# osqp/osqp-python

Measured on AMD Instinct MI355X. Metric: ADMM iterations/sec, n=100000 m=200000 nnz(A)=1000000 sparse QP (indirect PCG), higher is better.
Workload: dtype f64

## Files before the change

### osqp-python_amd/csrc/backend.h

```cpp
#pragma once
#include <cstddef>
#include <cstdint>
#include <stdexcept>

namespace osqp_hip {

struct DeviceError : std::runtime_error { using std::runtime_error::runtime_error; };

#ifndef OSQP_HIP_KBLOCK
#define OSQP_HIP_KBLOCK 256
#define OSQP_HIP_KGRID 1024
#endif
constexpr int kBlock = OSQP_HIP_KBLOCK;
constexpr int kGrid = OSQP_HIP_KGRID;
constexpr int kChunk = 8 * kBlock;
constexpr int kLongRow = 128;
constexpr int kMaxRowsPerBlock = 1024;
constexpr int kPartSlots = 40;
constexpr int kMaxCg = 1024;
constexpr int kWinCap = 1472;
constexpr int kF1Win = 512;
constexpr int kF1MaxD = 4;
constexpr int kF1PChunk = 256;
constexpr int kF1MaxOwn = 512;
constexpr int kF1MaxRows = 512;
constexpr int kF1Chunk = 1024;
constexpr int kF1StreamBytes = kF1Chunk * 12;

struct DevCsr {
  int nrows = 0, ncols = 0, nnz = 0, nblk = 0;
  int *rowptr = nullptr, *col = nullptr;
  int *blkdesc = nullptr;
  int *runinfo = nullptr;
  double *val = nullptr;
  int *blkwin = nullptr;
  unsigned short *lcol = nullptr;
  int split = 0;
  int nwin = 0;
  int single = 0;
};

struct DevF1 {
  int on = 0;
  int D = 0;
  int *blk = nullptr;
  unsigned char *stream = nullptr;
  unsigned short *cptr = nullptr;
  int *prp = nullptr, *pcol = nullptr, *psrc = nullptr;
  double *pval = nullptr;
  int pnnz = 0;
  double *va = nullptr; size_t ns = 0;
  unsigned vbytes = 0, o_rho = 0, o_pval = 0, o_pcol = 0, o_prp = 0, o_rowptr = 0, o_cptr = 0, nsb = 0;
  int mix = 0;
  int wt = 0;
  int *fcol = nullptr, *fq = nullptr;
  int *sp_ptr = nullptr;
  int *spk = nullptr;
  double *spill = nullptr; size_t nsp = 0;
};
constexpr int kF1MaxFar = 128;

constexpr int kKfMaxFill = 8;
struct DevKf {
  int on = 0;
  DevCsr K;
  int *tptr = nullptr;
  int *trow = nullptr, *ta = nullptr, *tb = nullptr;
  int nterm = 0;
  double *rec = nullptr;
};

constexpr int kWbMaxRows = 128;
constexpr int kWbLargeMax = 16384;
inline size_t wb_inverse_work(int n) { return (size_t)n * 64 * 3 + 2 * 64 * 64 + 8; }
constexpr int kWbxCols = 64;
constexpr int kWbxMaxN = 16384;
struct DevWbx {
  int on = 0, G = 0, nsc = 0;
  int slots = 0;
  double *tile2 = nullptr;
  double *tile = nullptr;
  double *partG = nullptr, *partZ = nullptr;
  double *ls0 = nullptr, *ls1 = nullptr;
  int one = 0;
  double *sinvp = nullptr;
  double *lz0 = nullptr, *lz1 = nullptr;
  int *sc_ptr = nullptr, *sc_row = nullptr, *sc_src = nullptr;
  double *sc_val = nullptr;
  double *bjj = nullptr;
};
struct DevWb {
  int on = 0, r = 0;
  int large = 0;
  int ct = 0;
  int probe = 0;
  double exact_tol = 1e-6;
  int log = 0;
  int *colmap = nullptr;
  double *W = nullptr;
  double *pv = nullptr;
  int *info = nullptr;
  int *dbg = nullptr;
  int exact = 0;
  DevWbx x;
  DevCsr AL, ALT;
  int *al_src = nullptr, *alt_src = nullptr;
  unsigned char *islong = nullptr;
  int *rows = nullptr;
  double *WT = nullptr;
  double *S = nullptr, *Sinv = nullptr;
  static constexpr int kCache = 4;
  double rho_key = 0.0;
  double *cache_buf[kCache] = {nullptr, nullptr, nullptr, nullptr}; double cache_rho[kCache] = {0, 0, 0, 0}; int cache_used = 0, cache_next = 0;
  int cache_hits = 0, cache_on = 1;
  double *g = nullptr, *h = nullptr;
  double *Dinv0 = nullptr;
  int vendor = 0;
  double *gjwork = nullptr;
  int dual = 0, cd = 0;
  int *kind = nullptr;
  int *dcol = nullptr;
  int *srow = nullptr, *ssrc = nullptr; double *sval = nullptr;
  int *sg_ptr = nullptr, *sg_col = nullptr;
  double *wv = nullptr, *den = nullptr, *beta = nullptr, *wbeta = nullptr, *rt = nullptr;
  double *uz = nullptr;
  int fused = 0;
  DevCsr Bd, Bn, As;
  double *cc = nullptr;
  int *lidx = nullptr;
  double *sig = nullptr;
  int dense = 0, grb = 0;
  int thin = 0;
  double *Ad = nullptr, *ud = nullptr, *ccd = nullptr, *gp = nullptr;
  int *bq_ptr = nullptr, *bq_idx = nullptr, *bq_col = nullptr;
};

enum ResId {
  R_PRI_U = 0, R_AX_U, R_Z_U, R_PRI_S, R_AX_S, R_Z_S, R_DY_U, R_DY_S, R_PINF_LHS, R_SUPP,
  R_DUA_U, R_PX_U, R_ATY_U, R_DUA_S, R_PX_S, R_ATY_S, R_DX_U, R_DX_S, R_XPX, R_QX, R_QDX,
  R_QN_S, R_QN_U,
  R_ATDY_U, R_ATDY_S, R_PDX_U, R_PDX_S, R_ADX_VIOL,
  R_COUNT
};
enum FlagId { F_DONE = 0, F_ITERS, F_STAT_SUM, F_STAT_MAX, F_STAT_UNCONV, F_STAT_SUMSQ, F_STAT_N, F_STAT_STAG, F_COUNT };
enum ScalId { S_TOL_REL = 0, S_TOL_ABS, S_TOL_NOW, S_RN0 , S_RN0H , S_HIST = 8  };

struct Ctl;
struct Dev {
  int n = 0, m = 0, device = 0;
  Ctl *ctl = nullptr;
  double sigma = 0, alpha = 0;
  double rho_eq_factor = 1e3;
  DevCsr A, B;
  int *Bdiag = nullptr;
  double *Praw = nullptr, *Araw = nullptr;
  int nzP = 0, nzA = 0;
  int *Pi = nullptr, *Pj = nullptr, *Pm1 = nullptr, *Pm2 = nullptr;
  int *Ai = nullptr, *Aj = nullptr, *AmA = nullptr, *AmB = nullptr;
  double *cs = nullptr;
  double *q = nullptr, *l = nullptr, *u = nullptr, *D = nullptr, *Dinv = nullptr, *E = nullptr, *Einv = nullptr;
  double *rho = nullptr, *rho_inv = nullptr;
  int *ctype = nullptr;
  double *qraw = nullptr, *lraw = nullptr, *uraw = nullptr;
  int *cnt = nullptr;
  int eq_from_cnt = 0;
  double rho_eq_mixed = 10.0;
  double *x = nullptr, *z = nullptr, *y = nullptr, *dx = nullptr, *dy = nullptr;
  double *xs = nullptr;
  double *xg = nullptr, *xsp = nullptr, *ztg = nullptr;
  int wt = 0;
  double theta = 0.9;
  double *zt = nullptr;
  double *t0 = nullptr;
  double *v = nullptr;
  double *r = nullptr, *uu = nullptr, *p = nullptr, *s = nullptr, *w = nullptr, *t = nullptr, *Minv = nullptr;
  double *uu2 = nullptr, *ms = nullptr;
  int fused = 0;
  int batch_wave_ran = -1;
  DevF1 f1;
  DevKf kf;
  DevWb wb;
  double *part = nullptr;
  double *res = nullptr;
  double *scal = nullptr;
  int *flags = nullptr;
  int *slot = nullptr;
  void *stream = nullptr;
  void *bside = nullptr, *bev0 = nullptr, *bev1 = nullptr;
  void *impl = nullptr;
};

constexpr int kBatchNB = 8;
constexpr int kBatchDirectMaxBw = 64 - kBatchNB;

constexpr int kBatchRec = 12;
struct BatchParams {
  int n, m, nbatch;
  DevCsr A, B;
  const double *D, *Dinv, *E, *Einv;
  double c, cinv, sigma, alpha, rho0, eq_factor, eps_abs, eps_rel, eps_pinf, eps_dinf, cg_frac, rho_tol;
  int max_iter, check, rho_interval, cg_max, unscaled, scaling, precond, rho_is_vec, warm;
  const double *q, *l, *u;
  const double *q0, *l0, *u0;
  double *x, *y;
  double *rec;
  int *iters_out = nullptr;
  const int *order = nullptr;
  double *zs = nullptr;
  int variant = 0;
  int polish = 0, refine = 0;
  double delta = 1e-6;
  int bw = -1;
// ... 152 lines not shown
```

### osqp-python_amd/csrc/engine.cpp

```cpp


#include "engine_internal.hpp"

#include <atomic>
#include <cstdarg>

namespace osqp_hip {

const BatchEnv &batch_env() {
  static const BatchEnv e = [] {
    auto num = [](const char *name, int dflt) { const char *v = std::getenv(name); return v ? std::atoi(v) : dflt; };
    return BatchEnv{num("OSQP_HIP_WAVE_SPLIT", -1), num("OSQP_HIP_WAVE_CUS", -1), num("OSQP_HIP_BATCH_WIDE_ROUNDS", 1 << 20)};
  }();
  return e;
}
namespace {
thread_local OSQPHipPolicy g_default_policy;
thread_local bool g_default_policy_set = false;

void policy_from_env(OSQPHipPolicy &p, bool runtime_only) {
  if (!runtime_only) { if (g_default_policy_set) p = g_default_policy; else Engine::default_policy(&p); }
  auto on = [](const char *name, OSQPInt &v) { if (const char *e = std::getenv(name)) v = e[0] != '0'; };
  auto num = [](const char *name, OSQPInt &v) { if (const char *e = std::getenv(name)) v = std::atoi(e); };
  auto real = [](const char *name, OSQPFloat &v) { if (const char *e = std::getenv(name)) v = std::atof(e); };
  on("OSQP_HIP_SMALL_DIRECT", p.small_direct); num("OSQP_HIP_DEVICE_DRIVEN", p.device_driven); on("OSQP_HIP_BATCH_REORDER", p.batch_reorder);
  num("OSQP_HIP_BATCH_WAVE", p.batch_wave);
  num("OSQP_HIP_RHO_WINDOW", p.rho_window); real("OSQP_HIP_RHO_WINDOW_TOL", p.rho_window_tol); on("OSQP_HIP_RHO_PERSIST", p.rho_persist);
  if (const char *e = std::getenv("OSQP_HIP_RHO_TOL_EXP")) { const double v = std::atof(e); p.rho_tol_exp = v > 0 && v <= 1 ? v : 0.5; }
  real("OSQP_HIP_BUDGET_TOLERATE", p.budget_tolerate); real("OSQP_HIP_BUDGET_SIGMA", p.budget_sigma); num("OSQP_HIP_BUDGET_SLACK", p.budget_slack);
  if (std::getenv("OSQP_HIP_BUDGET_FULL")) p.budget_full = 1;
  on("OSQP_HIP_CG_ESCALATE", p.cg_escalate); on("OSQP_HIP_STALL", p.stall);
  real("OSQP_HIP_POLISH_DELTA_FLOOR", p.polish_delta_floor); real("OSQP_HIP_POLISH_PCG_TOL", p.polish_pcg_tol);
  on("OSQP_HIP_SLOT_POLL", p.slot_poll); num("OSQP_HIP_POLL_LOW", p.poll_low); real("OSQP_HIP_POLL_FIRST", p.poll_first);
  real("OSQP_HIP_POLL_FRAC", p.poll_frac); real("OSQP_HIP_POLL_WAIT", p.poll_wait);
  num("OSQP_HIP_FINISH_PAIRS", p.finish_pairs); num("OSQP_HIP_POLL_SLEEP_US", p.poll_sleep_us);
  if (std::getenv("OSQP_HIP_SLOT_LOG")) p.slot_log = 1;
  if (std::getenv("OSQP_HIP_BATCH_TIMING")) p.batch_timing = 1;
  if (std::getenv("OSQP_HIP_WB_LOG")) p.woodbury_log = 1;
  if (const char *e = std::getenv("OSQP_HIP_BATCH_VARIANT")) {
    static const char *names[] = {"", "direct", "direct256", "w64", "w256", "generic"};
    p.batch_variant = 0;
    for (int k = 1; k <= 5; k++) if (!std::strcmp(e, names[k])) p.batch_variant = k;
  }
  if (runtime_only) return;
  num("OSQP_HIP_WOODBURY_FUSED", p.woodbury_fused); real("OSQP_HIP_WOODBURY_DIRECT_TOL", p.woodbury_direct_tol);
  on("OSQP_HIP_WOODBURY", p.woodbury); on("OSQP_HIP_WOODBURY_DIRECT", p.woodbury_direct); on("OSQP_HIP_WOODBURY_LARGE", p.woodbury_large);
  num("OSQP_HIP_REORDER", p.reorder); on("OSQP_HIP_WOODBURY_CACHE", p.woodbury_cache); on("OSQP_HIP_KFORM", p.kform); on("OSQP_HIP_WOODBURY_DUAL", p.woodbury_dual); on("OSQP_HIP_WOODBURY_VENDOR", p.woodbury_vendor);
  on("OSQP_HIP_GRAPH", p.graph); on("OSQP_HIP_SLOTS", p.slots); on("OSQP_HIP_PCG_FUSED", p.pcg_fused); num("OSQP_HIP_F1", p.f1); on("OSQP_HIP_WINDOW", p.window);
  real("OSQP_HIP_EXTRAP", p.extrap);
  if (const char *e = std::getenv("OSQP_HIP_RHO_EQ_FACTOR")) { const double v = std::atof(e); if (v >= 1.0) p.rho_eq_factor = v; }
  if (std::getenv("OSQP_HIP_SETUP_TIMING")) p.setup_timing = 1;
}
}

void Engine::default_policy(OSQPHipPolicy *p) {
  if (!p) return;
  *p = OSQPHipPolicy();
  p->graph = p->slots = p->pcg_fused = p->f1 = p->window = p->device_driven = p->small_direct = p->batch_reorder = 1; p->batch_variant = 0;
  p->extrap = 0.9; p->rho_eq_factor = 0.0;
  p->rho_window = 10; p->rho_window_tol = 0.1; p->rho_persist = 1; p->rho_tol_exp = 0.5;
  p->budget_tolerate = 0.0; p->budget_sigma = 3.0; p->budget_slack = 0; p->budget_full = 0; p->cg_escalate = 1; p->stall = 1;
  p->polish_delta_floor = 1e-3; p->polish_pcg_tol = 1e-15; p->woodbury = 1; p->woodbury_direct = 1; p->woodbury_large = 1; p->woodbury_cache = 1;
  p->slot_poll = 1; p->poll_low = 6; p->poll_first = 0.8; p->poll_frac = 0.75; p->poll_wait = 0.7;
  p->finish_pairs = 12; p->poll_sleep_us = 30;
  p->reorder = 1; p->kform = 0; p->woodbury_dual = 1; p->woodbury_vendor = 0; p->woodbury_fused = 1; p->woodbury_direct_tol = 1e-6; p->debug_fail_refactor = 0; p->batch_wave = 0;
}
void Engine::set_default_policy(const OSQPHipPolicy *p) {
  g_default_policy_set = p != nullptr;
  if (p) g_default_policy = *p;
}
int Engine::get_policy(OSQPHipPolicy *p) const { if (!p) return OSQP_DATA_VALIDATION_ERROR; *p = pol_; return OSQP_NO_ERROR; }
int Engine::set_policy(const OSQPHipPolicy *p) {
  if (!p) return OSQP_DATA_VALIDATION_ERROR;
  if (!(p->extrap >= 0 && p->extrap <= 2) || p->rho_window < 0 || !(p->rho_window_tol > 0) || !(p->rho_tol_exp > 0 && p->rho_tol_exp <= 1) ||
      !(p->budget_sigma >= 0) || p->finish_pairs < 1 || p->batch_variant < 0 || p->batch_variant > 5 || p->batch_wave < -1 || p->batch_wave > 1 ||
      !(p->rho_eq_factor == 0 || p->rho_eq_factor >= 1) || p->reorder < 0 || p->reorder > 2 || !(p->woodbury_direct_tol > 0 && p->woodbury_direct_tol < 1) || !(p->polish_delta_floor > 0) || !(p->polish_pcg_tol > 0 && p->polish_pcg_tol < 1))
    return OSQP_SETTINGS_VALIDATION_ERROR;
  const OSQPHipPolicy old = pol_;
  pol_ = *p; pol_explicit_ = true;
  pol_.slots = old.slots; pol_.pcg_fused = old.pcg_fused; pol_.f1 = old.f1; pol_.window = old.window; pol_.woodbury = old.woodbury; pol_.woodbury_direct = old.woodbury_direct; pol_.woodbury_large = old.woodbury_large; pol_.reorder = old.reorder; pol_.woodbury_cache = old.woodbury_cache; pol_.woodbury_fused = old.woodbury_fused; pol_.woodbury_direct_tol = old.woodbury_direct_tol; pol_.kform = old.kform; pol_.woodbury_dual = old.woodbury_dual; pol_.woodbury_vendor = old.woodbury_vendor;
  if (pol_.graph != old.graph) { use_graph_ = pol_.graph != 0; if (dev_ready_) { be::activate(d_); be::sync(d_); drop_graphs(); } }
  if (dev_ready_) d_.theta = pol_.extrap;
  if (dev_ready_ && d_.wb.dbg && pol_.debug_fail_refactor != old.debug_fail_refactor) { be::activate(d_); const int v = pol_.debug_fail_refactor; be::h2d(d_, d_.wb.dbg, &v, sizeof(int)); }
  if (dev_ready_ && pol_.rho_eq_factor >= 1.0 && pol_.rho_eq_factor != old.rho_eq_factor) return set_rho_eq_factor(pol_.rho_eq_factor);
  return OSQP_NO_ERROR;
}

namespace {
std::atomic<osqp_hip_print_fn> g_print_fn{nullptr};
std::atomic<void *> g_print_user{nullptr};
}
void Engine::set_default_print(osqp_hip_print_fn fn, void *user) { g_print_user.store(user); g_print_fn.store(fn); }
void Engine::say(const char *fmt, ...) const {
  char buf[1024];
  va_list ap;
  va_start(ap, fmt);
  std::vsnprintf(buf, sizeof(buf), fmt, ap);
  va_end(ap);
  if (print_fn_) print_fn_(buf, print_user_);
  else { std::fputs(buf, stdout); std::fflush(stdout); }
}
void Engine::print_summary_line(int iter, double obj, double pri, double dua, double rho, double t0) const {
  say("%4d  %11.4e   %8.2e   %8.2e   %8.2e  %8.2es\n", iter, obj, pri, dua, rho, (first_run_ ? info.setup_time : info.update_time) + (now_s() - t0));
}
void Engine::print_log(const Ctl &c, double t0) {
  if (!settings.verbose) return;
  if (c.nlog - log_printed_ > kCtlLog) log_printed_ = c.nlog - kCtlLog;
  for (; log_printed_ < c.nlog; log_printed_++) {
    const double *e = c.log[log_printed_ % kCtlLog];
    print_summary_line((int)e[0], e[1], e[2], e[3], e[4], t0);
  }
}

Engine::Engine() {
  print_fn_ = g_print_fn.load(); print_user_ = g_print_user.load();
  pub.settings = &settings; pub.solution = &solution; pub.info = &info; pub.work = reinterpret_cast<OSQPWorkspace *>(this);
  policy_from_env(pol_, false);
  use_graph_ = pol_.graph != 0; use_slots_ = pol_.slots != 0;
  if (pol_.rho_eq_factor >= 1.0) { eq_factor_mixed_ = pol_.rho_eq_factor; eq_factor_env_ = true; }
}
Engine::~Engine() { free_all(); }

void Engine::drop_graphs() {
  for (auto &kv : graphs_) be::graph_free(d_, kv.second);
  graphs_.clear();
  for (auto &kv : sgraphs_) be::graph_free(d_, kv.second);
  sgraphs_.clear();
}

void Engine::sync_graph_scalars() {
  const double sig[7] = {d_.theta, d_.alpha, d_.sigma, d_.rho_eq_factor, d_.rho_eq_mixed, (double)d_.eq_from_cnt, (double)reinterpret_cast<uintptr_t>(d_.wb.Sinv)};
  if (std::memcmp(sig, graph_sig_, sizeof(sig)) == 0) return;
  if (!graphs_.empty() || !sgraphs_.empty()) { be::sync(d_); drop_graphs(); }
  std::memcpy(graph_sig_, sig, sizeof(sig));
}

void Engine::free_all() {
  if (!dev_ready_) return;
  try { be::activate(d_); be::ext_wait(d_); be::sync(d_); } catch (const DeviceError &) {}
  drop_graphs();
  if (bbuf_) { be::dfree(d_, bbuf_); bbuf_ = nullptr; bbuf_cap_ = 0; }
  if (bmat_) { be::dfree(d_, bmat_); bmat_ = nullptr; bmat_cap_ = 0; }
  if (d_batch_order_) { be::dfree(d_, d_batch_order_); d_batch_order_ = nullptr; batch_order_cap_ = 0; }
  if (d_batch_iters_) { be::dfree(d_, d_batch_iters_); d_batch_iters_ = nullptr; d_batch_iters_n_ = 0; }
  batch_order_.clear();
  if (ckpt_) { be::dfree(d_, ckpt_); ckpt_ = nullptr; }
  free_batch_direct(); free_batch_spectral(); free_batch_wave();
  if (d_.f1.va) {
    d_.Minv = d_.xs = d_.p = d_.r = d_.s = d_.rho = d_.f1.pval = nullptr; d_.f1.pcol = d_.f1.prp = nullptr; d_.f1.cptr = nullptr;
  }
  if (d_.wb.cache_buf[0]) d_.wb.Sinv = d_.wb.cache_buf[0];
  void *ptrs[] = {d_.A.rowptr, d_.A.col, d_.A.blkdesc, d_.A.val, d_.B.rowptr, d_.B.col, d_.B.blkdesc, d_.B.val, d_.Bdiag, d_.A.runinfo, d_.B.runinfo, d_.A.blkwin, d_.B.blkwin, d_.A.lcol, d_.B.lcol, d_.qraw, d_.lraw, d_.uraw, d_.cnt,
                  d_.q, d_.l, d_.u, d_.D, d_.Dinv, d_.E, d_.Einv, d_.rho, d_.rho_inv, d_.ctype, d_.x, d_.z, d_.y, d_.dx,
                  d_.dy, d_.xs, d_.xg, d_.xsp, d_.ztg, d_.zt, d_.t0, d_.v, d_.r, d_.uu, d_.p, d_.s, d_.w, d_.t, d_.Minv, d_.uu2, d_.ms, d_.part, d_.res,
                  d_.scal, d_.flags, d_.slot, d_.Praw, d_.Araw, d_.cs, d_.Pi, d_.Pj, d_.Pm1, d_.Pm2, d_.Ai, d_.Aj, d_.AmA, d_.AmB,
                  d_.wb.AL.rowptr, d_.wb.AL.col, d_.wb.AL.blkdesc, d_.wb.AL.runinfo, d_.wb.AL.val, d_.wb.ALT.rowptr, d_.wb.ALT.col, d_.wb.ALT.blkdesc, d_.wb.ALT.runinfo, d_.wb.ALT.val,
                  d_.wb.al_src, d_.wb.alt_src, d_.wb.islong, d_.wb.rows, d_.wb.WT, d_.wb.S, d_.wb.Sinv, d_.wb.g, d_.wb.h, d_.wb.Dinv0, d_.wb.colmap, d_.wb.W, d_.wb.pv, d_.wb.info, d_.wb.dbg, d_.wb.x.tile, d_.wb.x.tile2, d_.wb.x.partG, d_.wb.x.partZ, d_.wb.x.ls0, d_.wb.x.ls1, d_.wb.x.lz0, d_.wb.x.lz1, d_.wb.x.sinvp, d_.wb.x.sc_ptr, d_.wb.x.sc_row, d_.wb.x.sc_src, d_.wb.x.sc_val, d_.wb.x.bjj,
                  d_.ctl, d_.f1.blk, d_.f1.stream, d_.f1.cptr, d_.f1.prp, d_.f1.pcol, d_.f1.psrc, d_.f1.pval, d_.f1.va, d_.f1.fcol, d_.f1.fq, d_.f1.sp_ptr, d_.f1.spk, d_.f1.spill, d_pc_, d_pr_,
                  d_.wb.gjwork, d_.wb.cc, d_.wb.sig, d_.wb.lidx, d_.wb.Ad, d_.wb.ud, d_.wb.ccd, d_.wb.gp, d_.wb.bq_ptr, d_.wb.bq_idx, d_.wb.bq_col, d_.wb.Bd.blkdesc, d_.wb.Bn.blkdesc, d_.wb.As.blkdesc, d_.wb.kind, d_.wb.dcol, d_.wb.srow, d_.wb.ssrc, d_.wb.sval, d_.wb.sg_ptr, d_.wb.sg_col, d_.wb.wv, d_.wb.den, d_.wb.beta, d_.wb.wbeta, d_.wb.rt, d_.wb.uz,
                  d_.kf.K.rowptr, d_.kf.K.col, d_.kf.K.blkdesc, d_.kf.K.runinfo, d_.kf.K.val, d_.kf.tptr, d_.kf.trow, d_.kf.ta, d_.kf.tb, d_.kf.rec};
  for (void *p : ptrs) if (p) be::dfree(d_, p);
  be::destroy(d_);
  d_ = Dev(); d_pc_ = d_pr_ = nullptr;
  dev_ready_ = false;
}

int Engine::validate_settings(const OSQPSettings *s, bool at_setup) {
  if (!s) return OSQP_SETTINGS_VALIDATION_ERROR;
  bool ok = s->device >= 0 && s->scaling >= 0 && s->rho > 0 && s->sigma > 0 && s->alpha > 0 && s->alpha < 2 &&
            s->cg_max_iter > 0 && s->cg_tol_reduction > 0 && s->cg_tol_fraction > 0 && s->cg_tol_fraction < 1 &&
            s->adaptive_rho_interval >= 0 && s->adaptive_rho_fraction > 0 && s->adaptive_rho_tolerance >= 1 &&
            s->max_iter > 0 && s->eps_abs >= 0 && s->eps_rel >= 0 && (s->eps_abs > 0 || s->eps_rel > 0) &&
            s->eps_prim_inf > 0 && s->eps_dual_inf > 0 && s->check_termination >= 0 && s->time_limit > 0 &&
            s->delta > 0 && s->polish_refine_iter >= 0 &&
            (s->cg_precond == OSQP_NO_PRECONDITIONER || s->cg_precond == OSQP_DIAGONAL_PRECONDITIONER);
  for (int flag : {s->verbose, s->warm_starting, s->polishing, s->rho_is_vec, s->adaptive_rho, s->scaled_termination, s->check_dualgap})
    ok = ok && (flag == 0 || flag == 1);
  if (!ok) return OSQP_SETTINGS_VALIDATION_ERROR;
  if (at_setup && s->linsys_solver != OSQP_INDIRECT_SOLVER) return OSQP_LINSYS_SOLVER_INIT_ERROR;
  return OSQP_NO_ERROR;
}

int Engine::auto_rho_interval() const {
  if (settings.adaptive_rho_interval > 0) return settings.adaptive_rho_interval;
  return settings.check_termination > 0 ? 2 * settings.check_termination : 50;
}

void Engine::compute_scaling(std::vector<double> &Px, std::vector<double> &Ax, std::vector<double> &qs) {
  D_.assign(n, 1.0); E_.assign(m, 1.0); c_ = 1.0;
  std::vector<double> dt(n), et(m), nP(n);
  auto p_col_norms = [&](std::vector<double> &out) {
    std::fill(out.begin(), out.end(), 0.0);
    for (int j = 0; j < n; j++)
      for (int k = P_.p[j]; k < P_.p[j + 1]; k++) {
        double a = std::fabs(Px[k]); int i = P_.i[k];
        out[j] = std::max(out[j], a); out[i] = std::max(out[i], a);
      }
  };
  for (int it = 0; it < settings.scaling; it++) {
    p_col_norms(dt);
    std::fill(et.begin(), et.end(), 0.0);
    for (int j = 0; j < n; j++)
      for (int k = A_.p[j]; k < A_.p[j + 1]; k++) {
        double a = std::fabs(Ax[k]);
        dt[j] = std::max(dt[j], a); et[A_.i[k]] = std::max(et[A_.i[k]], a);
      }
    for (int j = 0; j < n; j++) dt[j] = 1.0 / std::sqrt(limit_scaling(dt[j]));
    for (int i = 0; i < m; i++) et[i] = 1.0 / std::sqrt(limit_scaling(et[i]));
    for (int j = 0; j < n; j++) {
      for (int k = P_.p[j]; k < P_.p[j + 1]; k++) Px[k] *= dt[P_.i[k]] * dt[j];
      for (int k = A_.p[j]; k < A_.p[j + 1]; k++) Ax[k] *= et[A_.i[k]] * dt[j];
      qs[j] *= dt[j]; D_[j] *= dt[j];
    }
    for (int i = 0; i < m; i++) E_[i] *= et[i];
    p_col_norms(nP);
    double mean = 0; for (int j = 0; j < n; j++) mean += nP[j];
    mean /= std::max(n, 1);
    double nq = 0; for (int j = 0; j < n; j++) nq = std::max(nq, std::fabs(qs[j]));
    double ct = 1.0 / limit_scaling(std::max(limit_scaling(nq), mean));
    for (auto &v : Px) v *= ct;
    for (auto &v : qs) v *= ct;
    c_ *= ct;
  }
  Dinv_.resize(n); Einv_.resize(m);
  for (int j = 0; j < n; j++) Dinv_[j] = 1.0 / D_[j];
  for (int i = 0; i < m; i++) Einv_[i] = 1.0 / E_[i];
  cinv_ = 1.0 / c_;
}

void Engine::scale_matrix_values(std::vector<double> &Px, std::vector<double> &Ax) const {
  Px.resize(P_.nnz()); Ax.resize(A_.nnz());
  for (int j = 0; j < n; j++) {
    for (int k = P_.p[j]; k < P_.p[j + 1]; k++) Px[k] = c_ * D_[P_.i[k]] * D_[j] * P_.x[k];
    for (int k = A_.p[j]; k < A_.p[j + 1]; k++) Ax[k] = E_[A_.i[k]] * D_[j] * A_.x[k];
  }
}

void Engine::classify_constraints(const std::vector<double> &ls, const std::vector<double> &us) {
  const std::vector<int> before = ctype_;
  ctype_.resize(m);
  int n_ineq = 0;
  for (int i = 0; i < m; i++) {
    int t;
    if (ls[i] < -OSQP_INFTY * kMinScaling && us[i] > OSQP_INFTY * kMinScaling) t = -1;
    else if (us[i] - ls[i] < kRhoTol) t = 1;
    else t = 0;
    if (!settings.rho_is_vec) t = 0;
    ctype_[i] = t;
    n_ineq += (t == 0);
  }
  d_.rho_eq_factor = (n_ineq == 0) ? 1e3 : mixed_eq_factor();
  d_.eq_from_cnt = 0;
  if (before != ctype_) for (int k = 0; k < DevWb::kCache; k++) d_.wb.cache_rho[k] = -1.0;
}

void Engine::device_scale_vectors(bool q, bool bounds) {
  if (q) be::scale_q(d_, c_);
  if (bounds) {
    d_.rho_eq_mixed = mixed_eq_factor(); d_.eq_from_cnt = 1;
    be::scale_bounds(d_, settings.rho_is_vec);
    scaled_stale_ = true;
  }
}

void Engine::ensure_host_vectors() {
  if (raw_stale_) {
    be::d2h(d_, q0_.data(), d_.qraw, sizeof(double) * n);
    if (m > 0) { be::d2h(d_, l0_.data(), d_.lraw, sizeof(double) * m); be::d2h(d_, u0_.data(), d_.uraw, sizeof(double) * m); }
    raw_stale_ = false;
  }
  if (scaled_stale_) {
    ls_.resize(m); us_.resize(m);
    for (int i = 0; i < m; i++) { ls_[i] = E_[i] * l0_[i]; us_[i] = E_[i] * u0_[i]; }
    const int keep = d_.eq_from_cnt; const double keepf = d_.rho_eq_factor;
    classify_constraints(ls_, us_);
    d_.eq_from_cnt = keep; if (keep) d_.rho_eq_factor = keepf;
    scaled_stale_ = false;
  }
}

double Engine::mixed_eq_factor() const {
  constexpr int kSmallEqN = 256;
  return (!eq_factor_set_ && !eq_factor_env_ && n <= kSmallEqN) ? 1e3 : eq_factor_mixed_;
}

int Engine::set_rho_eq_factor(double f) {
  if (!dev_ready_) return OSQP_WORKSPACE_NOT_INIT_ERROR;
  if (!(f >= 1.0)) return OSQP_SETTINGS_VALIDATION_ERROR;
  be::activate(d_);
  eq_factor_mixed_ = f; eq_factor_set_ = true;
  ensure_host_vectors();
  upload_bounds_and_types();
  be::set_rho(d_, rho_bar_);
  be::precond(d_, settings.cg_precond == OSQP_DIAGONAL_PRECONDITIONER);
  return OSQP_NO_ERROR;
}

void Engine::upload_bounds_and_types() {
  std::vector<double> ls(m), us(m);
  for (int i = 0; i < m; i++) { ls[i] = E_[i] * l0_[i]; us[i] = E_[i] * u0_[i]; }
  apply_scaled_bounds(ls, us);
}
// ... 674 lines not shown
```

### osqp-python_amd/csrc/engine_setup.cpp

```cpp
#include "engine_internal.hpp"

namespace osqp_hip {

bool Engine::compute_reorder(const std::vector<int> &Arp, const std::vector<int> &Arj, const std::vector<int> &Brp, const std::vector<int> &Bj) {
  std::vector<int> cstamp(n, 0), rstamp(m, 0), comp_done(n, 0), order, sweep, best;
  order.reserve(n);
  int stamp = 0;
  size_t widest = 0;
  auto bfs = [&](int start, std::vector<int> &out) {
    out.clear(); stamp++;
    out.push_back(start); cstamp[start] = stamp;
    size_t level_end = 1;
    for (size_t h = 0; h < out.size(); h++) {
      if (h == level_end) { widest = std::max(widest, out.size() - level_end); level_end = out.size(); }
      const int j = out[h];
      for (int k = A_.p[j]; k < A_.p[j + 1]; k++) {
        const int i = A_.i[k];
        if (rstamp[i] == stamp) continue;
        rstamp[i] = stamp;
        for (int e = Arp[i]; e < Arp[i + 1]; e++) { const int c = Arj[e]; if (cstamp[c] != stamp) { cstamp[c] = stamp; out.push_back(c); } }
      }
      for (int k = Brp[j]; k < Brp[j + 1] && Bj[k] < n; k++) { const int c = Bj[k]; if (cstamp[c] != stamp) { cstamp[c] = stamp; out.push_back(c); } }
    }
  };
// ... 89 lines not shown
  if (!be::device_assembly() || m == 0 || nb < kGrid / 4) return fail("too few row blocks", nb);
  std::vector<int> a0(nb), wl(nb), lo0(nb), hi0(nb), nfar(nb, 0), cs(nb + 1);
  std::vector<int> sc, dcols;
  int D = 0;
  const int npass = allow_mix ? 3 : 1;
  for (int pass = 0; pass < npass; pass++) {
  bool pass_failed = false;
  const int far_cost = pass == 2 ? 1 : 4;
  pl.mix = 0; std::fill(nfar.begin(), nfar.end(), 0);
  for (int b = 0; b < nb; b++) {
    const int r0 = rb[b], r1 = rb[b + 1], k0 = Arp[r0], k1 = Arp[r1];
    if (k1 == k0 || r1 - r0 > kF1MaxRows || k1 - k0 > kF1Chunk || (r1 - r0 == 1 && k1 - k0 > kLongRow)) return fail("block shape", b);
    int lo = INT32_MAX, hi = -1;
    for (int k = k0; k < k1; k++) { lo = std::min(lo, Arj[k]); hi = std::max(hi, Arj[k]); }
    if (hi - lo + 1 > kF1Win || pass >= 1) {
      if (!allow_mix) return fail("no window (strict)", b);
      sc.assign(Arj.begin() + k0, Arj.begin() + k1);
      std::sort(sc.begin(), sc.end());
      bool found = false;
      {
        const int kFarCost = far_cost;
        std::vector<int> &dc = dcols; dc.assign(sc.begin(), sc.end());
        dc.erase(std::unique(dc.begin(), dc.end()), dc.end());
        const int U = (int)dc.size();
        int bi = 0, bj = 0, ci = 0; long cur = 0, best = 0;
        for (int t = 1; t < U; t++) {
          cur += kFarCost + 1 - (dc[t] - dc[t - 1]);
          if (cur < 0) { cur = 0; ci = t; }
          else if (cur > best) { best = cur; bi = ci; bj = t; }
        }
        const int far = U - (bj - bi + 1);
        const long inside = std::upper_bound(sc.begin(), sc.end(), dc[bj]) - std::lower_bound(sc.begin(), sc.end(), dc[bi]);
        if (far <= kF1MaxFar && 2 * inside >= (long)sc.size() && dc[bj] - dc[bi] + 1 <= (far ? kF1Win - kF1MaxFar : kF1Win)) { found = true; lo = dc[bi]; hi = dc[bj]; nfar[b] = far; }
      }
      if (!found && hi - lo + 1 <= kF1Win) found = true;
      if (!found) {
        const int width = kF1Win - kF1MaxFar;
        int best = -1, bi = 0, bj = 0;
        for (int i = 0, j = 0; i < (int)sc.size(); i++) {
          while (j < (int)sc.size() && sc[j] - sc[i] < width) j++;
          if (j - i > best) { best = j - i; bi = i; bj = j; }
        }
        int far = 0;
        for (int i = 0; i < (int)sc.size(); i++) if ((i < bi || i >= bj) && (i == 0 || sc[i] != sc[i - 1])) far++;
        if (far <= kF1MaxFar) { found = true; lo = sc[bi]; hi = sc[bj - 1]; nfar[b] = far; }
      }
      if (!found) { if (pass + 1 < npass) { pass_failed = true; break; } return fail("too many far columns", b); }
      if (nfar[b]) pl.mix = 1;
    }
    lo0[b] = lo; hi0[b] = hi;
  }
  if (pass_failed) continue;
  cs[0] = 0;
  for (int g = 1; g < nb; g++) {
    const int ideal = (int)((long)rb[g] * n / m);
    const int lo = std::max(cs[g - 1], std::min(lo0[g], n)), up = hi0[g - 1] + 1;
    cs[g] = lo <= up ? std::min(std::max(ideal, lo), up) : lo;
    cs[g] = std::min(std::max(cs[g], cs[g - 1]), n);
  }
  cs[nb] = n;
  for (int b = 0; b < nb; b++) {
    int lo = lo0[b], hi = hi0[b];
    if (cs[b + 1] > cs[b]) { lo = std::min(lo, cs[b]); hi = std::max(hi, cs[b + 1] - 1); }
    if (hi - lo + 1 > (nfar[b] ? kF1Win - kF1MaxFar : kF1Win)) { if (pass + 1 < npass) { pass_failed = true; break; } return fail("window + own columns too wide", b); }
    a0[b] = lo; wl[b] = hi - lo + 1;
  }
  if (pass_failed) continue;
  D = 0;
  for (int t = 1; t <= kF1MaxD && !D; t++) {
    bool ok = true;
    for (int g = 0; g + t < nb && ok; g++) ok = a0[g] + wl[g] <= a0[g + t];
    if (ok) D = t;
  }
  if (D) break;
  }
  if (!D) return fail("windows of blocks g and g + 4 overlap", -1);
  std::vector<int> &prp = pl.prp; prp.assign(n + 1, 0);
  for (int j = 0; j < n; j++) { int c = 0; for (int k = Brp[j]; k < Brp[j + 1] && Bj[k] < n; k++) c++; prp[j + 1] = prp[j] + c; }
  const int pnnz = prp[n];
  std::vector<int> &pcol = pl.pcol, &psrc = pl.psrc; pcol.assign(std::max(pnnz, 1), 0); psrc.assign(std::max(pnnz, 1), 0);
  for (int j = 0; j < n; j++) for (int k = Brp[j], o = prp[j]; k < Brp[j + 1] && Bj[k] < n; k++, o++) { pcol[o] = Bj[k]; psrc[o] = k; }
  std::vector<int> &blk = pl.blk; blk.assign(16 * (size_t)nb, 0);
  std::vector<unsigned int> &ent = pl.ent; ent.assign(Arj.size(), 0u);
  std::vector<unsigned short> &cptr = pl.cptr; cptr.clear();
  if (pl.mix) { pl.fcol.assign((size_t)nb * kF1MaxFar, -1); pl.fq.assign((size_t)nb * kF1MaxFar, 0); }
  size_t nsp = 0;
  std::vector<int> order, tpos, fc, slot;
  for (int b = 0; b < nb; b++) {
    if (cs[b + 1] - cs[b] > kF1MaxOwn || prp[cs[b + 1]] - prp[cs[b]] > kF1PChunk) return fail("own columns", b);
    const int r0 = rb[b], r1 = rb[b + 1], k0 = Arp[r0], k1 = Arp[r1], cnt = k1 - k0;
    int *w = &blk[16 * (size_t)b];
    w[0] = r0; w[1] = r1; w[2] = k0; w[3] = k1;
    w[4] = b < D ? 0 : a0[b]; w[5] = b + D < nb ? a0[b + D] : n; w[6] = cs[b]; w[7] = cs[b + 1];
    w[8] = (int)cptr.size(); w[9] = prp[cs[b]]; w[10] = prp[cs[b + 1]]; w[11] = 0;
    fc.clear();
    if (nfar[b]) {
      for (int k = k0; k < k1; k++) if (Arj[k] < a0[b] || Arj[k] >= a0[b] + wl[b]) fc.push_back(Arj[k]);
      std::sort(fc.begin(), fc.end()); fc.erase(std::unique(fc.begin(), fc.end()), fc.end());
    }
    const int nfc = (int)fc.size();
    w[11] = nfc;
    int g0 = a0[b], g1 = a0[b] + wl[b];
    for (int k = prp[cs[b]]; k < prp[cs[b + 1]]; k++) { g0 = std::min(g0, pcol[k]); g1 = std::max(g1, pcol[k] + 1); }
    if (g1 - g0 > (nfc ? kF1Win - kF1MaxFar : kF1Win) || 4 * (g1 - g0) > 5 * wl[b]) { g0 = a0[b]; g1 = a0[b] + wl[b]; }
    w[12] = g0; w[13] = g1 - g0; w[14] = a0[b]; w[15] = wl[b];
    slot.resize(cnt);
    for (int e = 0; e < cnt; e++) {
      const int c = Arj[k0 + e];
      if (c >= a0[b] && c < a0[b] + wl[b]) slot[e] = c - a0[b];
      else slot[e] = wl[b] + (int)(std::lower_bound(fc.begin(), fc.end(), c) - fc.begin());
    }
    order.resize(cnt);
    for (int e = 0; e < cnt; e++) order[e] = e;
    std::stable_sort(order.begin(), order.end(), [&](int x, int y) { return slot[x] < slot[y]; });
    tpos.resize(cnt);
    for (int t = 0; t < cnt; t++) tpos[order[t]] = t;
    for (int r = r0; r < r1; r++)
      for (int k = Arp[r]; k < Arp[r + 1]; k++) {
        const int sl = slot[k - k0];
        const unsigned gs = sl < wl[b] ? (unsigned)(Arj[k] - g0) : (unsigned)(kF1Win - kF1MaxFar + sl - wl[b]);
        ent[k] = gs | ((unsigned)(r - r0) << 9) | ((unsigned)tpos[k - k0] << 18);
      }
    const size_t base = cptr.size();
    cptr.resize(base + wl[b] + nfc + 1, 0);
    for (int e = 0; e < cnt; e++) cptr[base + slot[e] + 1]++;
    for (int c = 0; c < wl[b] + nfc; c++) cptr[base + c + 1] = (unsigned short)(cptr[base + c + 1] + cptr[base + c]);
    if (pl.mix) { std::copy(fc.begin(), fc.end(), pl.fcol.begin() + (size_t)b * kF1MaxFar); nsp += (size_t)nfc; }
  }
  if (pol_.f1 == 3 && !pl.mix) { pl.mix = 1; pl.fcol.assign((size_t)nb * kF1MaxFar, -1); pl.fq.assign((size_t)nb * kF1MaxFar, 0); }
  if (pl.mix && nsp >= (size_t)1 << 25) return fail("too many spill slots", -1);
  if (pl.mix) {
    pl.nsp = nsp;
    pl.sp_ptr.assign((size_t)n + 1, 0);
    for (int c : pl.fcol) if (c >= 0) pl.sp_ptr[c + 1]++;
    for (int j = 0; j < n; j++) pl.sp_ptr[j + 1] += pl.sp_ptr[j];
    std::vector<int> cur(pl.sp_ptr.begin(), pl.sp_ptr.end() - 1);
    for (size_t i = 0; i < pl.fcol.size(); i++) if (pl.fcol[i] >= 0) pl.fq[i] = cur[pl.fcol[i]]++;
    for (int j = 0; j < n; j++) if (pl.sp_ptr[j + 1] - pl.sp_ptr[j] > 63) return fail("a column is far for more than 63 row blocks", -1);
  }
  pl.D = D; pl.pnnz = pnnz; pl.ok = true;
  if (pol_.setup_timing) {
    double swl = 0, sgl = 0, sown = 0; int mwl = 0;
    for (int b = 0; b < nb; b++) { swl += wl[b]; sgl += blk[16 * (size_t)b + 13]; sown += cs[b + 1] - cs[b]; mwl = std::max(mwl, wl[b]); }
    std::fprintf(stderr, "[osqp_hip] F1 plan: %d row blocks, D = %d, scatter window %.1f columns on average (max %d), gather window %.1f, own columns %.1f, far columns %.2f per block\n",
                 nb, D, swl / nb, mwl, sgl / nb, sown / nb, (double)pl.nsp / nb);
  }
  return true;
}

void Engine::upload_f1(const F1Plan &pl, const std::vector<int> &Arp) {
  d_.f1 = DevF1();
  if (!pl.ok) return;
  const size_t ns = ((size_t)n + 31) / 32 * 32;
  size_t at = 8 * (7 + 3 * (size_t)pl.D) * ns;
  auto region = [&at](size_t bytes) { const size_t o = at; at += (std::max<size_t>(bytes, 1) + 255) / 256 * 256; return o; };
  const size_t o_rho = region(8 * (size_t)m), o_pval = region(8 * (size_t)pl.pnnz), o_pcol = region(sizeof(int) * pl.pcol.size()),
               o_prp = region(sizeof(int) * pl.prp.size()), o_rowptr = region(sizeof(int) * Arp.size()), o_cptr = region(sizeof(unsigned short) * pl.cptr.size());
  if (at >= ((size_t)1 << 31)) return;
  auto up_i = [&](const std::vector<int> &h) { int *p = dev_vec<int>(d_, h.size()); if (!h.empty()) be::h2d(d_, p, h.data(), sizeof(int) * h.size()); return p; };
  DevF1 &f = d_.f1;
  f.D = pl.D; f.pnnz = pl.pnnz;
  f.ns = ns; f.nsb = (unsigned)(8 * ns);
  f.va = dev_vec<double>(d_, at / 8); f.vbytes = (unsigned)at;
  unsigned char *ab = reinterpret_cast<unsigned char *>(f.va);
  f.o_rho = (unsigned)o_rho; f.o_pval = (unsigned)o_pval; f.o_pcol = (unsigned)o_pcol; f.o_prp = (unsigned)o_prp; f.o_rowptr = (unsigned)o_rowptr; f.o_cptr = (unsigned)o_cptr;
  f.pval = reinterpret_cast<double *>(ab + o_pval); f.pcol = reinterpret_cast<int *>(ab + o_pcol); f.prp = reinterpret_cast<int *>(ab + o_prp);
  f.cptr = reinterpret_cast<unsigned short *>(ab + o_cptr);
  auto put = [&](size_t o, const void *h, size_t bytes) { if (bytes) be::h2d(d_, ab + o, h, bytes); };
  put(o_pcol, pl.pcol.data(), sizeof(int) * pl.pcol.size()); put(o_prp, pl.prp.data(), sizeof(int) * pl.prp.size());
  put(o_rowptr, Arp.data(), sizeof(int) * Arp.size()); put(o_cptr, pl.cptr.data(), sizeof(unsigned short) * pl.cptr.size());
  f.blk = up_i(pl.blk); f.psrc = up_i(pl.psrc);
  {
    const size_t nb = pl.blk.size() / 16;
    std::vector<unsigned char> hs(nb * (size_t)kF1StreamBytes, 0);
    for (size_t b = 0; b < nb; b++) {
      const int k0 = pl.blk[16 * b + 2], cnt = pl.blk[16 * b + 3] - k0;
      std::memcpy(hs.data() + b * (size_t)kF1StreamBytes + sizeof(double) * kF1Chunk, pl.ent.data() + k0, sizeof(unsigned int) * (size_t)cnt);
    }
    f.stream = dev_vec<unsigned char>(d_, hs.size()); be::h2d(d_, f.stream, hs.data(), hs.size());
  }
  if (pl.mix) {
    std::vector<int> spk((size_t)n), fc2(2 * pl.fcol.size(), 0);
    for (int j = 0; j < n; j++) spk[j] = (pl.sp_ptr[j] << 6) | (pl.sp_ptr[j + 1] - pl.sp_ptr[j]);
    for (size_t i = 0; i < pl.fcol.size(); i++) if (pl.fcol[i] >= 0) { fc2[2 * i] = pl.fcol[i]; fc2[2 * i + 1] = spk[pl.fcol[i]]; }
    f.mix = 1; f.fcol = up_i(fc2); f.fq = up_i(pl.fq); f.sp_ptr = up_i(pl.sp_ptr); f.spk = up_i(spk);
    f.nsp = pl.nsp; f.spill = dev_vec<double>(d_, 3 * (f.nsp + 2));
  }
  {
    const double mb = ((double)(pl.blk.size() / 16) * kF1StreamBytes + 8.0 * (7 + 3 * (double)pl.D) * (double)f.ns + 8.0 * 10 * (double)m) / (1024.0 * 1024.0);
    const char *e = std::getenv("OSQP_HIP_F1_WT");
    f.wt = e ? (e[0] != '0') : (mb <= 380.0);
  }
  f.on = 1;
}

void Engine::prepare_kf(const std::vector<int> &Arp, const std::vector<int> &Arj, const std::vector<int> &Brp, const std::vector<int> &Bj) {
  d_.kf = DevKf();
  if (!pol_.kform || !be::kf_supported() || !be::device_assembly() || m == 0) return;
  const double t0 = now_s();
  const long nzA = Arp[m];
  long nprod = 0;
  for (int i = 0; i < m; i++) { const long len = Arp[i + 1] - Arp[i]; nprod += len * len; if (nprod > (long)kKfMaxFill * nzA + n) break; }
  long npt = 0;
  for (int j = 0; j < n; j++) for (int k = Brp[j]; k < Brp[j + 1] && Bj[k] < n; k++) npt++;
  if (nprod > (long)kKfMaxFill * nzA + n || nprod + npt >= (1L << 30)) {
    if (pol_.setup_timing) std::fprintf(stderr, "[osqp_hip] K form: fill too large (sum of squared row lengths > %d nnz(A))\n", kKfMaxFill);
    return;
  }
  std::vector<int> Krp(n + 1, 0), Kj, tptr, trow, ta, tb;
  Kj.reserve((size_t)(nprod + npt)); trow.reserve((size_t)(nprod + npt)); ta.reserve((size_t)(nprod + npt)); tb.reserve((size_t)(nprod + npt));
  tptr.reserve((size_t)(nprod + npt) + 1);
  std::vector<int> mark(n, -1), slot(n, 0), cols, cnt, order, newslot, start;
  struct Term { int s, row, a, b; };
  std::vector<Term> terms;
  for (int j = 0; j < n; j++) {
    cols.clear(); cnt.clear(); terms.clear();
    auto add = [&](int c, int row, int a, int b) {
      if (mark[c] != j) { mark[c] = j; slot[c] = (int)cols.size(); cols.push_back(c); cnt.push_back(0); }
      cnt[slot[c]]++; terms.push_back(Term{slot[c], row, a, b});
    };
    for (int k = Brp[j]; k < Brp[j + 1] && Bj[k] < n; k++) add(Bj[k], -1, k, 0);
    for (int k = A_.p[j]; k < A_.p[j + 1]; k++) {
      const int i = A_.i[k], pa = AmapA_[k];
      for (int e = Arp[i]; e < Arp[i + 1]; e++) add(Arj[e], i, pa, e);
    }
    const int nc = (int)cols.size();
    order.resize(nc);
    for (int q = 0; q < nc; q++) order[q] = q;
    std::sort(order.begin(), order.end(), [&](int x, int y) { return cols[x] < cols[y]; });
    newslot.resize(nc); start.resize(nc + 1);
    start[0] = 0;
    for (int q = 0; q < nc; q++) { newslot[order[q]] = q; start[q + 1] = start[q] + cnt[order[q]]; }
    const size_t tbase = trow.size();
    for (int q = 0; q < nc; q++) { Kj.push_back(cols[order[q]]); tptr.push_back((int)tbase + start[q]); }
    trow.resize(tbase + terms.size()); ta.resize(tbase + terms.size()); tb.resize(tbase + terms.size());
    for (const Term &t : terms) { const size_t o = tbase + (size_t)start[newslot[t.s]]++; trow[o] = t.row; ta[o] = t.a; tb[o] = t.b; }
    Krp[j + 1] = (int)Kj.size();
  }
  tptr.push_back((int)trow.size());
  const int nzK = (int)Kj.size();
  std::vector<int> rb = build_row_blocks(Krp, n), runs;
  auto up_i = [&](const std::vector<int> &h) { int *p = dev_vec<int>(d_, h.size()); if (!h.empty()) be::h2d(d_, p, h.data(), sizeof(int) * h.size()); return p; };
  DevKf &f = d_.kf;
  DevCsr &K = f.K;
  K.nrows = n; K.ncols = n; K.nnz = nzK; K.nblk = (int)rb.size() - 1; K.split = n; K.nwin = 0;
  K.single = (int)rb.size() - 1 <= kGrid;
  for (size_t b = 0; b + 1 < rb.size(); b++) if (rb[b + 1] - rb[b] > kBlock) K.single = 0;
  K.rowptr = up_i(Krp); K.col = up_i(Kj); K.blkdesc = up_i(block_descs(rb, Krp, Kj, runs)); K.runinfo = up_i(runs);
  K.val = dev_vec<double>(d_, nzK);
  f.tptr = up_i(tptr); f.trow = up_i(trow); f.ta = up_i(ta); f.tb = up_i(tb); f.nterm = (int)trow.size();
  f.rec = dev_vec<double>(d_, 8 * (size_t)n);
  f.on = 1;
  if (pol_.setup_timing) std::fprintf(stderr, "[osqp_hip] K form: nnz(K) = %d (%.1f per row), %d terms, %d row blocks, %.1f ms\n", nzK, (double)nzK / n, f.nterm, K.nblk, 1e3 * (now_s() - t0));
}

void Engine::prepare_wb(const std::vector<int> &Arp, const std::vector<int> &Arj) {
  d_.wb = DevWb();
  if (!pol_.woodbury || !be::wb_supported() || settings.cg_precond != OSQP_DIAGONAL_PRECONDITIONER || m == 0) return;
  std::vector<int> rows;
  for (int i = 0; i < m; i++) if (Arp[i + 1] - Arp[i] > kLongRow) rows.push_back(i);
  const int r = (int)rows.size();
  if (r < 1) return;
  bool large = false, dual = false;
  std::vector<int> colmap, cntL;
  int ct = 0, cd = 0;
  if (r > kWbMaxRows) {
    if (r > kWbLargeMax || !pol_.woodbury_large || !be::wb_large_supported()) return;
    size_t nz_long = 0;
    for (int i : rows) nz_long += (size_t)(Arp[i + 1] - Arp[i]);
    if (2 * nz_long < (size_t)Arp[m]) return;
    colmap.assign(n, -1);
    for (int i : rows) for (int k = Arp[i]; k < Arp[i + 1]; k++) colmap[Arj[k]] = 0;
    for (int j = 0; j < n; j++) if (colmap[j] == 0) colmap[j] = ct++;
    cntL.assign(n, 0);
    for (int i : rows) for (int k = Arp[i]; k < Arp[i + 1]; k++) cntL[Arj[k]]++;
    for (int j = 0; j < n; j++) cd += cntL[j] >= 2;
    dual = pol_.woodbury_dual != 0 && cd >= 1 && 4 * (long)cd <= 3 * (long)r;
    const double order = dual ? cd : r, width = dual ? cd : ct;
    if (8.0 * ((double)r * width + 2.0 * order * order) > 24.0 * 1024 * 1024 * 1024) return;
    large = true;
  }
  std::vector<unsigned char> islong(m, 0);
  std::vector<int> lrp(r + 1, 0), lcol, lsrc;
  for (int a = 0; a < r; a++) {
    const int i = rows[a]; islong[i] = 1;
    for (int k = Arp[i]; k < Arp[i + 1]; k++) { lcol.push_back(Arj[k]); lsrc.push_back(k); }
    lrp[a + 1] = (int)lcol.size();
  }
  std::vector<int> trp(n + 1, 0), tcol(lcol.size()), tsrc(lcol.size());
  for (int c : lcol) trp[c + 1]++;
  for (int j = 0; j < n; j++) trp[j + 1] += trp[j];
  { std::vector<int> cur(trp.begin(), trp.end() - 1);
    for (int a = 0; a < r; a++) for (int k = lrp[a]; k < lrp[a + 1]; k++) { const int pos = cur[lcol[k]]++; tcol[pos] = a; tsrc[pos] = lsrc[k]; } }
  auto up_i = [&](const std::vector<int> &h) { int *p = dev_vec<int>(d_, h.size()); if (!h.empty()) be::h2d(d_, p, h.data(), sizeof(int) * h.size()); return p; };
  auto up_csr = [&](DevCsr &M, int nr, int nc, const std::vector<int> &rp, const std::vector<int> &cj) {
    std::vector<int> rb;
    if (&M == &d_.wb.AL) { for (int a = 0; a <= nr; a++) rb.push_back(a); }
    else rb = build_row_blocks(rp, nr);
    std::vector<int> runs;
    M.nrows = nr; M.ncols = nc; M.nnz = (int)cj.size(); M.nblk = (int)rb.size() - 1; M.split = nc; M.single = 0; M.nwin = 0;
    M.rowptr = up_i(rp); M.col = up_i(cj); M.blkdesc = up_i(block_descs(rb, rp, cj, runs)); M.runinfo = up_i(runs);
    M.val = dev_vec<double>(d_, cj.size());
  };
  DevWb &w = d_.wb;
  w.r = r;
  up_csr(w.AL, r, n, lrp, lcol); up_csr(w.ALT, n, r, trp, tcol);
  w.al_src = up_i(lsrc); w.alt_src = up_i(tsrc); w.rows = up_i(rows);
  w.islong = dev_vec<unsigned char>(d_, m); be::h2d(d_, w.islong, islong.data(), m);
  const size_t ord = dual ? (size_t)cd : (size_t)r;
  w.S = dev_vec<double>(d_, ord * ord); w.Sinv = dev_vec<double>(d_, ord * ord);
  w.g = dev_vec<double>(d_, r); w.h = dev_vec<double>(d_, r); w.Dinv0 = dev_vec<double>(d_, n);
  if (large && dual) {
    std::vector<int> kind(n, 0), dcol, srow(n, 0), ssrc(n, 0), sg_ptr(r + 1, 0), sg_col;
    for (int j = 0; j < n; j++) { colmap[j] = -1; if (cntL[j] >= 2) { kind[j] = 1; colmap[j] = (int)dcol.size(); dcol.push_back(j); } else if (cntL[j] == 1) kind[j] = 2; }
    for (int a = 0; a < r; a++) {
      for (int k = lrp[a]; k < lrp[a + 1]; k++) if (kind[lcol[k]] == 2) { srow[lcol[k]] = a; ssrc[lcol[k]] = lsrc[k]; sg_col.push_back(lcol[k]); }
      sg_ptr[a + 1] = (int)sg_col.size();
    }
// ... 157 lines not shown
    for (int j = 0; j < n; j++) Brp[j + 1] += Brp[j];
    nzB = Brp[n];
    Bj.assign(nzB, 0); std::vector<int> &bdiag = bdiag_; bdiag.assign(n, 0);
    Pmap1_.assign(nzP, -1); Pmap2_.assign(nzP, -1); AmapB_.resize(nzA);
    {
      std::vector<int> cur(Brp.begin(), Brp.end() - 1);
      for (int j = 0; j < n; j++) {
        for (int k = P_.p[j]; k < P_.p[j + 1]; k++) {
          int i = P_.i[k];
          if (i == j) continue;
          int p1 = cur[j]++; Bj[p1] = i; Pmap1_[k] = p1;
        }
        bdiag[j] = cur[j]++; Bj[bdiag[j]] = j;
        for (int k = P_.p[j]; k < P_.p[j + 1]; k++)
          if (P_.i[k] == j) Pmap1_[k] = bdiag[j];
        for (int k = P_.p[j]; k < P_.p[j + 1]; k++) {
          int i = P_.i[k];
          if (i == j) continue;
          int p2 = cur[i]++; Bj[p2] = j; Pmap2_[k] = p2;
        }
      }
      for (int j = 0; j < n; j++)
        for (int k = A_.p[j]; k < A_.p[j + 1]; k++) { int pos = cur[j]++; Bj[pos] = n + A_.i[k]; AmapB_[k] = pos; }
    }
  };
  build_structure();
  lap("CSR(A), B structure, maps");
  std::vector<int> rbA = build_row_blocks(Arp, m), rbB = build_row_blocks(Brp, n);
  lap("row blocks");
  bool has_long = false;
  for (int i = 0; i < m && !has_long; i++) has_long = Arp[i + 1] - Arp[i] > kLongRow;
  const bool want_f1 = pol_.pcg_fused && use_slots_ && pol_.window != 0 && pol_.f1 && !has_long;
  F1Plan plan;
  auto try_plan = [&]() {
    if (!want_f1) return false;
    if (plan_f1(rbA, Arp, Arj, Brp, Bj, plan)) return true;
    if ((long)nzA > (long)kGrid * kF1Chunk) {
      std::vector<int> rbF = build_row_blocks(Arp, m, kF1Chunk);
      if (plan_f1(rbF, Arp, Arj, Brp, Bj, plan)) { rbA.swap(rbF); return true; }
    } else {
      std::vector<int> rbF = build_row_blocks_target(Arp, m, kF1Chunk - 24);
      if ((int)rbF.size() - 1 >= kGrid / 4 && plan_f1(rbF, Arp, Arj, Brp, Bj, plan)) { rbA.swap(rbF); return true; }
    }
    return false;
  };
  bool f1ok = try_plan();
  clear_reorder(); reorder_ms_ = 0;
  const int reorder = no_reorder_ ? 0 : pol_.reorder;
  if (m > 0 && (reorder == 2 || (reorder == 1 && want_f1 && !f1ok && be::device_assembly() && (int)rbA.size() - 1 >= kGrid / 4 && !be::batch_lds_bytes(n, m)))) {
    const double tr = now_s();
    if (compute_reorder(Arp, Arj, Brp, Bj) || reorder == 2) {
      if (pc_.empty()) {
        pc_.resize(n); ipc_.resize(n); pr_.resize(m); ipr_.resize(m);
        for (int j = 0; j < n; j++) pc_[j] = ipc_[j] = j;
        for (int i = 0; i < m; i++) pr_[i] = ipr_[i] = i;
      }
      HostCsc P0 = P_, A0 = A_; std::vector<double> q00 = q0_, l00 = l0_, u00 = u0_;
      apply_reorder();
      build_structure();
      rbA = build_row_blocks(Arp, m); rbB = build_row_blocks(Brp, n);
      f1ok = try_plan();
      if (!f1ok && reorder != 2) {
        P_ = std::move(P0); A_ = std::move(A0); q0_ = std::move(q00); l0_ = std::move(l00); u0_ = std::move(u00);
        clear_reorder();
        build_structure();
        rbA = build_row_blocks(Arp, m); rbB = build_row_blocks(Brp, n);
        f1ok = try_plan();
      }
    }
    reorder_ms_ = 1e3 * (now_s() - tr);
    lap("reordering");
  }
  if (!dev_asm) { Px = P_.x; Ax = A_.x; qs = q0_; compute_scaling(Px, Ax, qs); lap("Ruiz scaling (host)"); }
  Arp_ = Arp; Arj_ = Arj; Brp_ = Brp; Bj_ = Bj;
  d_.fused = pol_.pcg_fused ? 1 : 0;
  prepare_wb(Arp, Arj);
  if (d_.wb.on) d_.fused = 0;
  d_.f1 = DevF1();
  if (d_.fused && f1ok) upload_f1(plan, Arp);
  if (d_.fused && !d_.f1.on && use_slots_) prepare_kf(Arp, Arj, Brp, Bj);
  if (reordered_) {
    d_pc_ = dev_vec<int>(d_, n); d_pr_ = dev_vec<int>(d_, m);
    be::h2d(d_, d_pc_, pc_.data(), sizeof(int) * n); be::h2d(d_, d_pr_, pr_.data(), sizeof(int) * m);
  }
  lap("F1 / Woodbury plans");
  auto descs = [](const std::vector<int> &rb, const std::vector<int> &rp, const std::vector<int> &cj, std::vector<int> &runs) {
    std::vector<int> d; d.reserve(4 * rb.size());
    runs.clear();
    for (size_t b = 0; b + 1 < rb.size(); b++) {
      const int r0 = rb[b], r1 = rb[b + 1], k0 = rp[r0], k1 = rp[r1];
      int end_row = r1;
      if (r1 - r0 == 1 && k1 - k0 > kLongRow) {
        end_row = -(1 + (int)runs.size());
        for (int base = k0; base < k1; base += kChunk) {
          const int end = std::min(k1, base + kChunk);
          bool run = true;
          for (int k = base + 1; k < end && run; k++) run = cj[k] == cj[k - 1] + 1;
          runs.push_back(run ? cj[base] : -1);
        }
      }
      d.push_back(r0); d.push_back(end_row); d.push_back(k0); d.push_back(k1);
    }
    return d;
  };

  const bool win_on = pol_.window != 0;
  auto windows = [win_on](const std::vector<int> &rb, const std::vector<int> &rp, const std::vector<int> &cj, int split,
                    std::vector<int> &win, std::vector<unsigned short> &lcol) {
    const size_t nb = rb.size() - 1;
    win.assign(4 * nb, 0); lcol.assign(std::max<size_t>(cj.size(), 1), 0);
    int nwin = 0;
    for (size_t b = 0; b < nb; b++) {
      const int r0 = rb[b], r1 = rb[b + 1], k0 = rp[r0], k1 = rp[r1];
      win[4 * b + 1] = -1;
      if (!win_on || (r1 - r0 == 1 && k1 - k0 > kLongRow) || k1 == k0) continue;
      int lo0 = INT32_MAX, hi0 = -1, lo1 = INT32_MAX, hi1 = -1;
      for (int k = k0; k < k1; k++) {
        const int c = cj[k];
        if (c < split) { lo0 = std::min(lo0, c); hi0 = std::max(hi0, c); } else { lo1 = std::min(lo1, c - split); hi1 = std::max(hi1, c - split); }
      }
      const long len0 = hi0 >= 0 ? (long)hi0 - lo0 + 1 : 0, len1 = hi1 >= 0 ? (long)hi1 - lo1 + 1 : 0;
      if (len0 + len1 > kWinCap) continue;
      if (len0 == 0) lo0 = 0;
      if (len1 == 0) lo1 = 0;
      win[4 * b] = lo0; win[4 * b + 1] = (int)len0; win[4 * b + 2] = lo1; win[4 * b + 3] = (int)len1;
      for (int k = k0; k < k1; k++) {
        const int c = cj[k];
        lcol[k] = (unsigned short)(c < split ? c - lo0 : len0 + (c - split - lo1));
      }
      nwin++;
    }
    return nwin;
  };
  auto up_i = [&](const std::vector<int> &h) { int *p = dev_vec<int>(d_, h.size()); be::h2d(d_, p, h.data(), sizeof(int) * h.size()); return p; };
  auto up_win = [&](DevCsr &M, const std::vector<int> &rb, const std::vector<int> &rp, const std::vector<int> &cj, int split) {
    std::vector<int> win; std::vector<unsigned short> lcol;
    M.split = split;
    M.single = (int)rb.size() - 1 <= kGrid;
    for (size_t b = 0; b + 1 < rb.size(); b++) if (rb[b + 1] - rb[b] > kBlock) M.single = 0;
    M.nwin = windows(rb, rp, cj, split, win, lcol);
    M.blkwin = up_i(win);
    M.lcol = dev_vec<unsigned short>(d_, lcol.size());
    be::h2d(d_, M.lcol, lcol.data(), sizeof(unsigned short) * lcol.size());
  };
  d_.A.nrows = m; d_.A.ncols = n; d_.A.nnz = nzA; d_.A.nblk = (int)rbA.size() - 1;
  d_.A.rowptr = up_i(Arp); d_.A.col = up_i(Arj); { std::vector<int> runs; d_.A.blkdesc = up_i(descs(rbA, Arp, Arj, runs)); d_.A.runinfo = up_i(runs); } d_.A.val = dev_vec<double>(d_, nzA);
  d_.B.nrows = n; d_.B.ncols = n + m; d_.B.nnz = nzB; d_.B.nblk = (int)rbB.size() - 1;
  d_.B.rowptr = up_i(Brp); d_.B.col = up_i(Bj); { std::vector<int> runs; d_.B.blkdesc = up_i(descs(rbB, Brp, Bj, runs)); d_.B.runinfo = up_i(runs); } d_.B.val = dev_vec<double>(d_, nzB);
  d_.Bdiag = up_i(bdiag_);
  up_win(d_.A, rbA, Arp, Arj, n); up_win(d_.B, rbB, Brp, Bj, n);
  build_wbf_views(rbA, rbB, Arp, Arj, Brp, Bj);
  lap("upload structure");
  auto dv = [&](size_t cnt) { return dev_vec<double>(d_, cnt); };
  d_.q = dv(n); d_.l = dv(m); d_.u = dv(m); d_.D = dv(n); d_.Dinv = dv(n); d_.E = dv(m); d_.Einv = dv(m);
  d_.rho = d_.f1.on ? reinterpret_cast<double *>(reinterpret_cast<unsigned char *>(d_.f1.va) + d_.f1.o_rho) : dv(m); d_.rho_inv = dv(m); d_.ctype = dev_vec<int>(d_, m);
  d_.x = dv(n); d_.z = dv(m); d_.y = dv(m); d_.dx = dv(n); d_.dy = dv(m); d_.zt = dv(m); d_.t0 = dv(m); d_.v = dv(m);
  d_.xg = dv(n); d_.xsp = dv(n); d_.ztg = dv(m);
  d_.theta = pol_.extrap;
  {
    const double mb = (12.0 * ((double)d_.A.nnz + (double)d_.B.nnz) + 8.0 * (14.0 * n + 12.0 * m)) / (1024.0 * 1024.0);
    const char *ev = std::getenv("OSQP_HIP_WT");
    d_.wt = ev ? (ev[0] != '0') : (mb <= 160.0);
  }
  d_.uu = dv(n); d_.w = dv(n); d_.t = dv(m); d_.uu2 = dv(n); d_.ms = dv(2 * (size_t)n);
  if (d_.f1.on) { const size_t ns = d_.f1.ns; double *va = d_.f1.va; d_.Minv = va; d_.xs = va + ns; d_.p = va + 2 * ns; d_.r = va + 3 * ns; d_.s = va + 5 * ns; }
  else { d_.r = dv(n); d_.p = dv(n); d_.s = dv(n); d_.Minv = dv(n); d_.xs = dv(n); }
  d_.part = dv((size_t)kPartSlots * kGrid); d_.res = dv(R_COUNT); d_.scal = dv(S_HIST + 3 * (kMaxCg + 1)); d_.flags = dev_vec<int>(d_, F_COUNT); d_.slot = dev_vec<int>(d_, be::kSlotInts);
  d_.ctl = be::device_assembly() ? static_cast<Ctl *>(be::alloc(d_, sizeof(Ctl))) : nullptr;
  if (dev_asm) {
    std::vector<int> Pj(nzP), Aj(nzA);
    for (int j = 0; j < n; j++) { for (int k = P_.p[j]; k < P_.p[j + 1]; k++) Pj[k] = j; for (int k = A_.p[j]; k < A_.p[j + 1]; k++) Aj[k] = j; }
    d_.nzP = nzP; d_.nzA = nzA;
    d_.Praw = dv(nzP); d_.Araw = dv(nzA); d_.cs = dv(2);
    d_.Pi = up_i(P_.i); d_.Pj = up_i(Pj); d_.Pm1 = up_i(Pmap1_); d_.Pm2 = up_i(Pmap2_);
    d_.Ai = up_i(A_.i); d_.Aj = up_i(Aj); d_.AmA = up_i(AmapA_); d_.AmB = up_i(AmapB_);
    be::h2d(d_, d_.Praw, P_.x.data(), sizeof(double) * nzP); be::h2d(d_, d_.Araw, A_.x.data(), sizeof(double) * nzA);
    be::h2d(d_, d_.q, q0_.data(), sizeof(double) * n);
    be::assemble(d_, 0, 1.0, 0);
    c_ = be::ruiz(d_, settings.scaling);
    cinv_ = 1.0 / c_;
    be::f1_refresh(d_); be::wb_refresh(d_); be::wbx_refresh(d_);
    D_.resize(n); E_.resize(m); Dinv_.resize(n); Einv_.resize(m);
    be::d2h(d_, D_.data(), d_.D, sizeof(double) * n); be::d2h(d_, Dinv_.data(), d_.Dinv, sizeof(double) * n);
    if (m > 0) { be::d2h(d_, E_.data(), d_.E, sizeof(double) * m); be::d2h(d_, Einv_.data(), d_.Einv, sizeof(double) * m); }
    lap("assembly + Ruiz scaling (device)");
  } else {
    Aval_.assign(nzA, 0.0); Bval_.assign(nzB, 0.0);
    fill_matrix_values(Px, Ax);
    be::h2d(d_, d_.D, D_.data(), sizeof(double) * n); be::h2d(d_, d_.Dinv, Dinv_.data(), sizeof(double) * n);
    be::h2d(d_, d_.E, E_.data(), sizeof(double) * m); be::h2d(d_, d_.Einv, Einv_.data(), sizeof(double) * m);
    lap("matrix values (host-scaled)");
  }
  d_.qraw = dv(n); d_.lraw = dv(m); d_.uraw = dv(m); d_.cnt = dev_vec<int>(d_, 2);
  raw_stale_ = scaled_stale_ = false;
  if (be::device_vec_updates()) {
    be::copy_in(d_, d_.qraw, q0_.data(), sizeof(double) * n, 0);
    be::copy_in(d_, d_.lraw, l0_.data(), sizeof(double) * m, 0); be::copy_in(d_, d_.uraw, u0_.data(), sizeof(double) * m, 0);
    device_scale_vectors(true, true);
  } else {
    upload_q();
    upload_bounds_and_types();
  }
  be::set_rho(d_, rho_bar_);
  try { be::precond(d_, settings.cg_precond == OSQP_DIAGONAL_PRECONDITIONER); }
  catch (const DeviceError &err) {
    if (!(d_.wb.on && d_.wb.large)) throw;
    std::fprintf(stderr, "osqp_hip: large-rank Woodbury correction switched off for this handle (%s)\n", err.what());
    d_.wb.on = 0;
    be::precond(d_, settings.cg_precond == OSQP_DIAGONAL_PRECONDITIONER);
  }
  be::init_iterates(d_, 1);

  sol_x_.assign(n, kNaN); sol_y_.assign(m, kNaN); sol_pc_.assign(m, kNaN); sol_dc_.assign(n, kNaN);
  solution.x = sol_x_.data(); solution.y = sol_y_.data(); solution.prim_inf_cert = sol_pc_.data(); solution.dual_inf_cert = sol_dc_.data();
  std::memset(&info, 0, sizeof(info));
  set_status(OSQP_UNSOLVED);
  cg_budget_ = 0; have_tol_ = false; first_run_ = true; slot_pred_[0] = slot_pred_[1] = 6.0; slot_pred_[2] = 14.0;
  stats_ = OSQPHipStats(); stats_.nnzA = nzA; stats_.nnzB = nzB;
  be::sync(d_);
  lap("vectors, rho, preconditioner");
  info.setup_time = now_s() - t0;
  if (settings.verbose) print_setup_header();
  return OSQP_NO_ERROR;
}

void Engine::print_setup_header() const {
  say("-----------------------------------------------------------------\n");
  say("           OSQP v%s  -  Operator Splitting QP Solver\n", "1.0.0-hip");
  say("        ADMM engine for AMD MI355X (%s), C ABI of osqp v1\n", be::name());
  say("-----------------------------------------------------------------\n");
  say("problem:  variables n = %d, constraints m = %d\n", n, m);
  say("          nnz(P) + nnz(A) = %d\n", P_.nnz() + A_.nnz());
  say("settings: linear system solver = indirect (reduced-KKT PCG, %s),\n", settings.cg_precond == OSQP_DIAGONAL_PRECONDITIONER ? "diagonal preconditioner" : "no preconditioner");
  say("          eps_abs = %.2e, eps_rel = %.2e,\n", settings.eps_abs, settings.eps_rel);
  say("          eps_prim_inf = %.2e, eps_dual_inf = %.2e,\n", settings.eps_prim_inf, settings.eps_dual_inf);
  say("          rho = %.2e %s\n", settings.rho, settings.adaptive_rho ? "(adaptive)" : "");
  say("          sigma = %.2e, alpha = %.2f, max_iter = %d\n", settings.sigma, settings.alpha, settings.max_iter);
  say("          check_termination: %s (interval %d), cg_max_iter = %d\n", settings.check_termination ? "on" : "off", settings.check_termination, settings.cg_max_iter);
  say("          scaling: %s, scaled_termination: %s\n", settings.scaling ? "on" : "off", settings.scaled_termination ? "on" : "off");
  say("          warm_start: %s, polish: %s\n\n", settings.warm_starting ? "on" : "off", settings.polishing ? "on" : "off");
}

}
```

### osqp-python_amd/csrc/pcg_hip.hip

```cpp
#include "hip_common.h"

namespace osqp_hip {
namespace be {

namespace {

struct GKb {
  const double *xg, *v, *t0; int n;
  __device__ __forceinline__ void operator()(int c, double a, double (&pr)[2]) const {
    if (c < n) { pr[0] = 0.0; pr[1] = a * xg[c]; }
    else { pr[0] = a * v[c - n]; pr[1] = a * t0[c - n]; }
  }
};
struct EKb {
  const double *x, *q, *Minv; double *r, *uu; double sigma; const double *xg; double *xs; double g = 0, rn = 0, bn = 0; double px = 0, pq = 0, pm = 0, pg = 0; int wt = 0;
  __device__ __forceinline__ void prefetch(int j) { px = x[j]; pq = q[j]; pm = Minv[j]; pg = xg[j]; }
  __device__ __forceinline__ void operator()(int j, const double (&s)[2]) {
    const double rhs = sigma * px - pq + s[0];
    const double rr = rhs - s[1], u = pm * rr;
    stw(wt, r + j, rr); stw(wt, uu + j, u); stw(wt, xs + j, pg);
    g += rr * u; rn = nanmax(rn, fabs(rr)); bn = nanmax(bn, fabs(rhs));
  }
};
__global__ __launch_bounds__(kBlock) void k_kb(Dev d) {
// ... 384 lines not shown
    double DL = dl_first;
    if (!d.B.single) { __syncthreads(); DL += block_sum(e.dl, lds.k2f.red); }
    put_partial(d.part, SL_DELTA, DL);
    st.ph = P_K1F;
  }
  slot_write(W, st);
}

template <class L>
__device__ __forceinline__ void slot_ka(const Dev &d, L &lds, int used, int conv, const FirstDesc &fd, int admm, int target, int seq, int rn_slot = -1) {
  double theta = d.theta, rn_last = 0.0, bn_last = 0.0;
  if (!conv) { theta = cutoff_theta(d, rn_slot >= 0 ? rn_slot : (used & 1), lds.red, rn_last, bn_last, admm); __syncthreads(); }
  GVec g{d.xs};
  EKa e{d.l, d.u, d.rho, d.rho_inv, d.z, d.y, d.zt, d.t0, d.v, d.dy, d.alpha, d.ztg, theta}; e.wt = d.wt;
  process_rows_fd<1>(d.A, g, e, lds, NoPre(), fd);
  const int stride = gridDim.x * kBlock;
  for (int j = blockIdx.x * kBlock + threadIdx.x; j < d.n; j += stride) {
    const double xt = d.xs[j], xo = d.x[j], xn = d.alpha * xt + (1.0 - d.alpha) * xo;
    stw(d.wt, d.dx + j, xn - xo); stw(d.wt, d.x + j, xn);
    stw(d.wt, d.xg + j, xt + theta * (xt - d.xsp[j])); stw(d.wt, d.xsp + j, xt);
  }
  if (blockIdx.x == 0) {
    if (!conv) {
      const double rn = rn_last, bn = bn_last;
      conv = !(rn > fmax(d.scal[S_TOL_REL] * bn, d.scal[S_TOL_ABS])) ? 2 : 0;
      if (!conv && threadIdx.x == 0 && rn > 0.1 * d.scal[S_RN0]) d.flags[F_STAT_STAG] += 1;
    }
    if (threadIdx.x == 0) {
      d.flags[F_STAT_SUM] += used; d.flags[F_STAT_SUMSQ] += used * used; d.flags[F_STAT_N] += 1;
      if (used > d.flags[F_STAT_MAX]) d.flags[F_STAT_MAX] = used;
      if (!conv) d.flags[F_STAT_UNCONV] += 1;
      if (d.ctl && admm + 1 >= target) { d.ctl->seq_end = seq + 1; d.ctl->chunk_done = 1; }
    }
  }
}

__global__ __launch_bounds__(kBlock) void k_slot_a(Dev d) {
  __shared__ union { StreamLdsW<1, double> k1; StreamLdsW<1, double> k1f; } lds;
  const FirstDesc fd = first_desc<true>(d.A);
  SlotState st = slot_read(d.slot + SR_WORDS);
  int *W = d.slot;
  if (st.ph == P_K1) {
    GVec g{d.uu};
    EK1 e{d.rho, d.t};
    if (process_rows_fd<1>(d.A, g, e, lds.k1, PreK1{d, 0, 0, lds.k1.red, st.admm & 1}, fd)) { st.ph = P_K2F; st.k = 0; }
    else {
      __syncthreads();
      slot_ka(d, lds.k1, 0, 1, fd, st.admm, st.target, st.seq);
      st.ph = P_KB; st.admm += 1;
    }
  } else if (st.ph == P_K1F) {
    const int k = st.k, i = k + 1;
    const int nchunk = (d.n + kBlock - 1) / kBlock, per = (nchunk + 7) >> 3;
    const int xcd = blockIdx.x & 7, slot0 = blockIdx.x >> 3;
    const bool has_vec = slot0 < per && xcd * per + slot0 < nchunk;
    if (!wg_has_rows(d.A) && !has_vec && blockIdx.x != 0) {
      put_partial(d.part, SL_GAMMA0 + (i & 1), 0.0); put_partial(d.part, SL_RN0 + (i & 1), 0.0);
    } else {
      double g = 0, rn = 0;
      GMs gr{d.ms};
      EK1F e{d.rho, d.t}; e.wt = d.wt;
      process_rows_fd<1>(d.A, gr, e, lds.k1f, PreK1F{d, k, has_vec, &e, lds.k1f.red, &g, &rn}, fd);
      __syncthreads();
      block_sum_max(g, rn, lds.k1f.red);
      put_partial(d.part, SL_GAMMA0 + (i & 1), g); put_partial(d.part, SL_RN0 + (i & 1), rn);
    }
    if (i >= st.cap) { st.ph = P_KA; st.used = i; st.conv = 0; }
    else { st.ph = P_K2F; st.k = i; }
  } else if (st.ph == P_KA) {
    slot_ka(d, lds.k1, st.used, st.conv, fd, st.admm, st.target, st.seq);
    st.ph = P_KB; st.admm += 1;
  }
  slot_write(W, st);
}


struct F1Lds {
  double win[kF1Win];
  double prod[kF1Chunk];
  double tvec[kF1MaxRows];
  double uown[kF1MaxOwn];
  double puown[kF1MaxOwn];
  double pprod[kF1PChunk];
  double red[3 * kWaves];
};
struct F1Stream { double val[kF1Chunk]; unsigned int ent[kF1Chunk]; };
static_assert(sizeof(F1Stream) == kF1StreamBytes, "LDS image and global layout of a block's stream must agree");
static_assert(kF1StreamBytes % (kWaves * 1024) == 0, "every wave issues whole 1 KB pieces");
template <bool NT>
__device__ __forceinline__ void lds_dma16(const void *gsrc, unsigned lds_base) {
#if defined(__HIP_DEVICE_COMPILE__)
  unsigned keep;
  if constexpr (NT) asm volatile("s_mov_b32 %0, m0\n\ts_mov_b32 m0, %2\n\ts_nop 0\n\tglobal_load_lds_dwordx4 %1, off nt\n\ts_mov_b32 m0, %0" : "=&s"(keep) : "v"(gsrc), "s"(lds_base) : "memory");
  else asm volatile("s_mov_b32 %0, m0\n\ts_mov_b32 m0, %2\n\ts_nop 0\n\tglobal_load_lds_dwordx4 %1, off\n\ts_mov_b32 m0, %0" : "=&s"(keep) : "v"(gsrc), "s"(lds_base) : "memory");
#else
  (void)gsrc; (void)lds_base;
#endif
}
__device__ __forceinline__ unsigned lds_offset_of(const void *p) {
#if defined(__HIP_DEVICE_COMPILE__)
  return (unsigned)(unsigned long long)(__attribute__((address_space(3))) const void *)p;
#else
  (void)p; return 0u;
#endif
}
template <bool NT>
__device__ __forceinline__ void f1_stream_issue(const unsigned char *stream, int b, F1Stream &S) {
  constexpr int kPieces = kF1StreamBytes / (kWaves * 1024);
  const int wave = __builtin_amdgcn_readfirstlane((int)(threadIdx.x >> 6));
  const unsigned char *g = stream + (size_t)b * kF1StreamBytes + (size_t)wave * (kPieces * 1024) + (threadIdx.x & 63) * 16;
  const unsigned l0 = lds_offset_of(&S) + (unsigned)wave * (kPieces * 1024);
#pragma unroll
  for (int q = 0; q < kPieces; q++) lds_dma16<NT>(g + q * 1024, __builtin_amdgcn_readfirstlane(l0 + q * 1024));
}
__device__ __forceinline__ void f1_stream_wait() {
#if defined(__HIP_DEVICE_COMPILE__)
  asm volatile("s_waitcnt vmcnt(0)" ::: "memory");
#endif
}
struct F1Scal { double alpha, beta; int general; };
template <int D>
__device__ __forceinline__ double f1_w(const double (&rp)[D]) {
  double w = rp[0];
#pragma unroll
  for (int q = 1; q < D; q++) w += rp[q];
  return w;
}
__device__ __forceinline__ void f1_upd(const F1Scal &sc, double minv, double r, double w, double sp, double &sn, double &rn, double &un) {
  sn = fma(sc.beta, sc.general ? sp : 0.0, w);
  rn = fma(-sc.alpha, sn, r);
  un = minv * rn;
}
template <int kB>
__device__ __forceinline__ double f1_segsum(const double *seg, int a, int z) {
  double v[kB];
#pragma unroll
  for (int q = 0; q < kB; q++) v[q] = a + q < z ? seg[a + q] : 0.0;
  double acc = 0.0;
#pragma unroll
  for (int q = 0; q < kB; q++) acc += v[q];
  for (int k = a + kB; k < z; k++) acc += seg[k];
  return acc;
}
struct F1Fold { PartRegs a, b, c; };
__device__ __forceinline__ F1Fold f1_fold_issue(const double *part, const int par, const int probe) {
  F1Fold f;
#pragma unroll
  for (int q = 0; q < kPart; q++) { f.a.v[q] = 0.0; f.b.v[q] = 0.0; f.c.v[q] = 0.0; }
  if (probe == 1) return f;
  const int prev = par ^ 1;
  f.a = partial_load(part + (SL_GAMMA0 + prev) * kGrid); f.b = partial_load(part + (SL_DELTA + prev) * kGrid); f.c = partial_load(part + (SL_RN0 + prev) * kGrid);
  return f;
}
__device__ __forceinline__ bool f1_fold_finish(const Dev &d, const int k, const int admm_par, const int probe, const F1Fold &f, double *red, F1Scal &sc) {
  double *gam = gptr(d.scal) + S_HIST, *alp = gptr(d.scal) + S_HIST + kMaxCg + 1;
  const int tid = threadIdx.x;
  sc = F1Scal{0.0, 0.0, k >= 2};
  if (probe == 1) { sc.alpha = 1e-3; sc.beta = k >= 2 ? 0.5 : 0.0; return true; }
  if (k == 0) return true;
  double tol = gptr(d.scal)[S_TOL_NOW];
  const double glast = k >= 2 ? gam[k - 2] : 1.0, alast = k >= 2 ? alp[k - 2] : 1.0;
  double gamma = partial_fold_sum(f.a), rn = partial_fold_max(f.c), delta = partial_fold_sum(f.b);
  block_sum_max_sum(gamma, rn, delta, red);
  if (k == 1 && probe == 0) {
    const double bn = block_max(partial_fold_max(partial_load(gptr(d.part) + SL_BN * kGrid)), red);
    tol = fmax(gptr(d.scal)[S_TOL_REL] * bn, gptr(d.scal)[S_TOL_ABS]);
    if (blockIdx.x == 0 && tid == 0) { gptr(d.scal)[S_TOL_NOW] = tol; gptr(d.scal)[S_RN0] = rn; gptr(d.scal)[S_RN0H + admm_par] = rn; }
    if (!(rn > tol)) return false;
  }
  if (probe) {
    if (rn < -1.0) gptr(d.res)[R_COUNT - 1] = gamma + delta + tol + glast + alast;
    sc.alpha = 1e-3; sc.beta = k >= 2 ? 0.5 : 0.0;
    return true;
  }
  if (k >= 2 && !(rn > tol)) return false;
  sc.beta = k >= 2 ? gamma / glast : 0.0;
  sc.alpha = k >= 2 ? gamma / (delta - sc.beta * gamma / alast) : gamma / delta;
  if (blockIdx.x == 0 && tid == 0) { gam[k - 1] = gamma; alp[k - 1] = sc.alpha; }
  return true;
}
__device__ __forceinline__ int4 sload_int4(const int *base, size_t idx) {
#if defined(__HIP_DEVICE_COMPILE__)
  typedef int __attribute__((ext_vector_type(4))) v4i;
  typedef const v4i __attribute__((address_space(4))) *cptr;
  const v4i v = ((cptr)(unsigned long long)base)[idx];
  return make_int4(v.x, v.y, v.z, v.w);
#else
  return reinterpret_cast<const int4 *>(base)[idx];
#endif
}
struct F1Rec { int4 ds, fa, fb, fc; };
__device__ __forceinline__ F1Rec f1_record(const DevF1 &f, int b) {
  return F1Rec{sload_int4(f.blk, 4 * (size_t)b), sload_int4(f.blk, 4 * (size_t)b + 1), sload_int4(f.blk, 4 * (size_t)b + 2), sload_int4(f.blk, 4 * (size_t)b + 3)};
}
struct F1Spill { double v0, v1; };
__device__ __forceinline__ F1Spill f1_spill_take(const double *sp, int word) {
  const int q0 = word >> 6, cnt = word & 63;
  F1Spill t{0.0, 0.0};
  if (cnt > 0) t.v0 = sp[q0];
  if (cnt > 1) t.v1 = sp[q0 + 1];
  return t;
}
__device__ __forceinline__ double f1_spill_sum(const double *sp, int word, const F1Spill &t) {
  const int q0 = word >> 6, cnt = word & 63;
  double a = 0.0;
  if (cnt > 0) a += t.v0;
  if (cnt > 1) a += t.v1;
  for (int q = q0 + 2; q < q0 + cnt; q++) a += sp[q];
  return a;
}
__device__ __forceinline__ double f1_spill_sum(const double *sp, const int *spk, int c) {
  const int word = spk[c];
  return f1_spill_sum(sp, word, f1_spill_take(sp, word));
}
template <bool WT>
__device__ __forceinline__ void gst_(double *p, double v) {
  if constexpr (WT) __hip_atomic_store(p, v, __ATOMIC_RELAXED, __HIP_MEMORY_SCOPE_AGENT); else *p = v;
}
#define gst gst_<WT>
struct F1Arena {
#if defined(__HIP_DEVICE_COMPILE__)
  __amdgpu_buffer_rsrc_t r;
  __device__ __forceinline__ F1Arena(const double *va, unsigned bytes) : r(__builtin_amdgcn_make_buffer_rsrc(const_cast<double *>(va), 0, (int)bytes, 0x00020000)) {}
  __device__ __forceinline__ double d(unsigned vo, unsigned so) const { return __builtin_bit_cast(double, __builtin_amdgcn_raw_buffer_load_b64(r, vo, so, 0)); }
  __device__ __forceinline__ int i(unsigned vo, unsigned so) const { return (int)__builtin_amdgcn_raw_buffer_load_b32(r, vo, so, 0); }
  __device__ __forceinline__ int h(unsigned vo, unsigned so) const { return (int)__builtin_amdgcn_raw_buffer_load_b16(r, vo, so, 0); }
#else
  const unsigned char *b;
  __device__ F1Arena(const double *va, unsigned) : b(reinterpret_cast<const unsigned char *>(va)) {}
  __device__ double d(unsigned vo, unsigned so) const { return *reinterpret_cast<const double *>(b + vo + so); }
  __device__ int i(unsigned vo, unsigned so) const { return *reinterpret_cast<const int *>(b + vo + so); }
  __device__ int h(unsigned vo, unsigned so) const { return *reinterpret_cast<const unsigned short *>(b + vo + so); }
#endif
};
template <int D, bool FIRST, bool MIX, bool WT>
__device__ __forceinline__ void f1_body(const Dev &d, const int k, const bool vec_only, const F1Scal sc, F1Lds &L, F1Stream &S, const F1Rec &rec0, const int par) {
  const DevF1 &f = d.f1;
  const int n = d.n, tid = threadIdx.x;
  const int cur = (k + 1) & 1, nxt = k & 1;
  KT(1);
  const size_t ns = f.ns;
  const F1Arena ar(f.va, f.vbytes);
  const unsigned nsb = f.nsb;
  const unsigned oxs = nsb, op = 2 * nsb;
  const unsigned orr = (3 + cur) * nsb;
  const unsigned osp = (5 + cur) * nsb;
  const unsigned orep = (7 + cur * D) * nsb;
  [[maybe_unused]] const unsigned orepV = (7 + 2 * D) * nsb;
  double *xs_w = gptr(f.va) + ns, *p_w = gptr(f.va) + 2 * ns;
  double *rnxt = gptr(f.va) + (3 + nxt) * ns;
  double *snew = gptr(f.va) + (5 + nxt) * ns;
  double *repnxt = gptr(f.va) + (7 + (size_t)nxt * D) * ns;
  [[maybe_unused]] const double *spcur = MIX ? gptr(f.spill) + (size_t)cur * (f.nsp + 2) : nullptr, *spV = MIX ? gptr(f.spill) + 2 * (f.nsp + 2) : nullptr;
  [[maybe_unused]] double *spnxt = MIX ? gptr(f.spill) + (size_t)nxt * (f.nsp + 2) : nullptr;
  [[maybe_unused]] const int *spk = MIX ? gptr(f.spk) : nullptr;
  double g_acc = 0.0, rn_acc = 0.0, dl_acc = 0.0, bn_acc = 0.0;
  auto own_update = [&](int j, double mi, double r, double w, double sp, double pp, double x) -> double {
    double sn, rn, un;
    f1_upd(sc, mi, r, w, sp, sn, rn, un);
    const double pn = fma(sc.beta, sc.general ? pp : 0.0, mi * r);
    gst(xs_w + j, fma(sc.alpha, pn, x)); gst(p_w + j, pn); gst(snew + j, sn); gst(rnxt + j, rn);
    g_acc += rn * un; rn_acc = nanmax(rn_acc, fabs(rn));
    return un;
  };
  const int xcd = blockIdx.x & 7, slot0 = blockIdx.x >> 3, slots = gridDim.x >> 3;
  const int per = (d.A.nblk + 7) >> 3;
  constexpr int CW = kF1Win / kBlock, CE = kF1Chunk / kBlock;
  constexpr int kFB = kF1Win - kF1MaxFar;
  static_assert(kFB >= (CW - 1) * kBlock, "the far slots belong to the lanes' last window element");
  static_assert(kF1PChunk == kBlock, "one (P + sigma I) entry per lane");
  for (int sl = slot0; sl < per; sl += slots) {
    const int b = __builtin_amdgcn_readfirstlane(xcd * per + sl);
    if (b >= d.A.nblk) break;
    [[maybe_unused]] int2 fcl = make_int2(0, 0); [[maybe_unused]] int fql = 0;
    if constexpr (MIX) { if (tid >= kFB - (CW - 1) * kBlock) { const size_t i = (size_t)b * kF1MaxFar + (tid - (kFB - (CW - 1) * kBlock)); fcl = reinterpret_cast<const int2 *>(gptr(f.fcol))[i]; fql = gptr(f.fq)[i]; } }
    const F1Rec rec = sl == slot0 ? rec0 : f1_record(f, b);
    const int4 ds = rec.ds, fa = rec.fa, fb = rec.fb, fc = rec.fc;
    const int r0 = ds.x, nrows = ds.y - ds.x, k0 = ds.z, cnt = ds.w - ds.z;
    const int cov0 = fa.x, cov1 = fa.y, cs0 = fa.z, nown = fa.w - fa.z;
    const int cpo = fb.x, pk0 = fb.y, pcnt = fb.z - fb.y;
    const int g0 = fc.x, gl = vec_only ? 0 : fc.y, a0 = fc.z, wl = fc.w;
    const int nfc = MIX && !vec_only ? fb.w : 0;
    const int nw = nfc ? CW : (gl + kBlock - 1) / kBlock, nu = (cnt + kBlock - 1) / kBlock, ns2 = nfc ? CW : (wl + kBlock - 1) / kBlock;
    KT(2);
    const bool hasp = !vec_only && tid < pcnt;
    const int pe = min(pk0 + max(0, min(tid, pcnt - 1)), f.pnnz - 1);
    const double pv = ar.d(8u * pe, f.o_pval); const int pc = ar.i(4u * pe, f.o_pcol);
    double wm[CW], wr[CW], wsv[CW], wq[CW][D], wpp[CW], wx[CW];
    bool wown[CW];
    [[maybe_unused]] int wsw[CW]; [[maybe_unused]] F1Spill wst[CW];
#pragma unroll
    for (int u = 0; u < CW; u++) {
      wown[u] = false;
      if (u < nw) {
        const int e = tid + u * kBlock;
        int c = g0 + min(e, gl - 1);
        if constexpr (MIX) { const bool isfar = u == CW - 1 && e >= kFB && e - kFB < nfc; if (isfar) c = fcl.x; wsw[u] = isfar ? fcl.y : spk[c]; }
        wown[u] = e < gl && c >= cs0 && c - cs0 < nown;
        wm[u] = ar.d(8u * c, 0);
#pragma unroll
        for (int q = 0; q < D; q++) wq[u][q] = ar.d(8u * c, orep + q * nsb);
        const int co = wown[u] ? c : g0;
        if (!FIRST) {
          wr[u] = ar.d(8u * c, orr);
          wsv[u] = ar.d(8u * c, osp);
          wx[u] = ar.d(8u * co, oxs); wpp[u] = ar.d(8u * co, op);
        } else { wx[u] = ar.d(8u * co, oxs); wpp[u] = gptr(d.xg)[co]; }
      }
    }
    if constexpr (MIX) {
#pragma unroll
      for (int u = 0; u < CW; u++) { if (u < nw) wst[u] = f1_spill_take(spcur, wsw[u]); }
    }
    int cp0[CW], cp1[CW];
    const int prow = r0 + min(tid, nrows - 1);
    const int rp0 = ar.i(4u * prow, f.o_rowptr), rp1 = ar.i(4u * prow, f.o_rowptr + 4); const double rrho = ar.d(8u * prow, f.o_rho);
#pragma unroll
    for (int u = 0; u < CW; u++) {
      if (u < ns2) {
        int c = min(tid + u * kBlock, wl - 1);
        if constexpr (MIX) { const int cf = tid + u * kBlock - kFB; if (u == CW - 1 && cf >= 0 && cf < nfc) c = wl + cf; }
        cp0[u] = ar.h(2u * (cpo + c), f.o_cptr); cp1[u] = ar.h(2u * (cpo + c), f.o_cptr + 2);
      }
    }
    const int pj = min(cs0 + max(0, min(tid, nown - 1)), n - 1);
    const int pp0 = ar.i(4u * pj, f.o_prp), pp1 = ar.i(4u * pj, f.o_prp + 4);
    const int pcl = pc - g0;
    const bool esc = hasp && !(pcl >= 0 && pcl < gl);
    KT(3);
#pragma unroll
    for (int u = 0; u < CW; u++) {
      if (u < nw) {
        int e = min(tid + u * kBlock, gl - 1);
        if constexpr (MIX) { const int ef = tid + u * kBlock; if (u == CW - 1 && ef >= kFB && ef - kFB < nfc) e = ef; }
        double un;
        double w = f1_w<D>(wq[u]);
        if constexpr (MIX) w += f1_spill_sum(spcur, wsw[u], wst[u]);
        if constexpr (FIRST) {
          const double r0 = w;
          un = wm[u] * r0;
          if (wown[u]) {
            const int j = g0 + e;
            gst(rnxt + j, r0); gst(gptr(d.xsp) + j, wx[u]); gst(xs_w + j, wpp[u]);
            g_acc += r0 * un; rn_acc = nanmax(rn_acc, fabs(r0));
          }
        } else {
          if (wown[u]) un = own_update(g0 + e, wm[u], wr[u], w, wsv[u], wpp[u], wx[u]);
          else { double sn, rn; f1_upd(sc, wm[u], wr[u], w, wsv[u], sn, rn, un); }
        }
        if (wown[u]) L.uown[g0 + e - cs0] = un;
        L.win[e] = un;
      }
    }
    for (int jj = tid; jj < nown; jj += kBlock) {
      const int j = cs0 + jj;
      if (j >= g0 && j - g0 < gl) continue;
      const double mi = ar.d(8u * j, 0);
      double rp[D];
#pragma unroll
      for (int q = 0; q < D; q++) rp[q] = ar.d(8u * j, orep + q * nsb);
      double un;
      double wj = f1_w<D>(rp);
      if constexpr (MIX) wj += f1_spill_sum(spcur, spk, j);
      if constexpr (FIRST) {
        const double r0 = wj;
        un = mi * r0;
        gst(rnxt + j, r0); gst(gptr(d.xsp) + j, ar.d(8u * j, oxs)); gst(xs_w + j, gptr(d.xg)[j]);
        g_acc += r0 * un; rn_acc = nanmax(rn_acc, fabs(r0));
      } else un = own_update(j, mi, ar.d(8u * j, orr), wj, ar.d(8u * j, osp), ar.d(8u * j, op), ar.d(8u * j, oxs));
      if (!vec_only) L.uown[jj] = un;
    }
    if (vec_only) continue;
    KT(4);
    f1_stream_wait();
#if defined(__HIP_DEVICE_COMPILE__)
    asm volatile("" :: "v"(rp0), "v"(rp1), "v"(rrho), "v"(pp0), "v"(pp1), "v"(pv), "v"(pc));
#pragma unroll
    for (int u = 0; u < CW; u++) { if (u < ns2) asm volatile("" :: "v"(cp0[u]), "v"(cp1[u])); }
    if constexpr (MIX) asm volatile("" :: "v"(fql));
#endif
    __syncthreads();
    [[maybe_unused]] double bv[D];
    [[maybe_unused]] int bsw = 0; [[maybe_unused]] F1Spill bst{0.0, 0.0};
    if constexpr (FIRST) {
      const int j = cs0 + max(0, min(tid, nown - 1));
#pragma unroll
      for (int q = 0; q < D; q++) bv[q] = ar.d(8u * j, orepV + q * nsb);
      if constexpr (MIX) bsw = spk[j];
    }
    double vw[CE]; unsigned int en[CE];
#pragma unroll
    for (int u = 0; u < CE; u++) { if (u < nu) { const int e = min(tid + u * kBlock, cnt - 1); vw[u] = S.val[e]; en[u] = S.ent[e]; } }
#pragma unroll
    for (int u = 0; u < CE; u++) { if (u < nu) L.prod[tid + u * kBlock] = vw[u] * L.win[en[u] & 0x1ffu]; }
    if (hasp) {
      double uv;
      if (!esc) uv = L.win[pcl];
      else {
        double eq[D];
#pragma unroll
        for (int q = 0; q < D; q++) eq[q] = ar.d(8u * pc, orep + q * nsb);
        const double em = ar.d(8u * pc, 0);
        double ew = f1_w<D>(eq);
        if constexpr (MIX) ew += f1_spill_sum(spcur, spk, pc);
        if constexpr (FIRST) uv = em * ew;
        else { double sn, rn; f1_upd(sc, em, ar.d(8u * pc, orr), ew, ar.d(8u * pc, osp), sn, rn, uv); }
      }
      L.pprod[tid] = pv * uv;
    }
    KT(5);
    __syncthreads();
    if (sl + slots < per) {
      const int bn = __builtin_amdgcn_readfirstlane(xcd * per + sl + slots);
      if (bn < d.A.nblk) f1_stream_issue<!WT>(f.stream, bn, S);
    }
    if (tid < nrows) {
      const double au = f1_segsum<6>(L.prod, rp0 - k0, rp1 - k0), t = rrho * au;
      L.tvec[tid] = t; dl_acc += t * au;
    }
    for (int row = tid + kBlock; row < nrows; row += kBlock) {
      const int q0 = ar.i(4u * (r0 + row), f.o_rowptr), q1 = ar.i(4u * (r0 + row), f.o_rowptr + 4);
      const double au = f1_segsum<6>(L.prod, q0 - k0, q1 - k0), t = ar.d(8u * (r0 + row), f.o_rho) * au;
      L.tvec[row] = t; dl_acc += t * au;
    }
    KT(6);
    __syncthreads();
#pragma unroll
    for (int u = 0; u < CE; u++) { if (u < nu) L.prod[en[u] >> 18] = vw[u] * L.tvec[(en[u] >> 9) & 0x1ffu]; }
    if (tid < nown) {
      const double pu = f1_segsum<4>(L.pprod, pp0 - pk0, pp1 - pk0);
      L.puown[tid] = pu; dl_acc += L.uown[tid] * pu;
    }
    for (int jj = tid + kBlock; jj < nown; jj += kBlock) {
      const int q0 = ar.i(4u * (cs0 + jj), f.o_prp), q1 = ar.i(4u * (cs0 + jj), f.o_prp + 4);
      const double pu = f1_segsum<4>(L.pprod, q0 - pk0, q1 - pk0);
      L.puown[jj] = pu; dl_acc += L.uown[jj] * pu;
    }
    KT(7);
    __syncthreads();
    double *rout = repnxt + (size_t)(b % D) * ns;
#pragma unroll
    for (int u = 0; u < CW; u++) {
      if (u < ns2) {
        const int c = tid + u * kBlock;
        if (c < wl) {
          double v = f1_segsum<8>(L.prod, cp0[u], cp1[u]);
          const int jo = a0 + c - cs0;
          if (jo >= 0 && jo < nown) v += L.puown[jo];
          gst(rout + a0 + c, v);
        } else if constexpr (MIX) {
          if (u == CW - 1 && c >= kFB && c - kFB < nfc) gst(spnxt + fql, f1_segsum<8>(L.prod, cp0[u], cp1[u]));
        }
      }
    }
    for (int j = cov0 + tid; j < a0; j += kBlock) gst(rout + j, 0.0);
    for (int j = a0 + wl + tid; j < cov1; j += kBlock) gst(rout + j, 0.0);
    if constexpr (FIRST) {
      if (tid < nown) bn_acc = nanmax(bn_acc, fabs(MIX ? f1_w<D>(bv) + f1_spill_sum(spV, bsw, f1_spill_take(spV, bsw)) : f1_w<D>(bv)));
      for (int jj = tid + kBlock; jj < nown; jj += kBlock) {
        double rv[D];
#pragma unroll
        for (int q = 0; q < D; q++) rv[q] = ar.d(8u * (cs0 + jj), orepV + q * nsb);
        bn_acc = nanmax(bn_acc, fabs(MIX ? f1_w<D>(rv) + f1_spill_sum(spV, spk, cs0 + jj) : f1_w<D>(rv)));
      }
    }
    KT(8);
    if (sl + slots < per) __syncthreads();
  }
  if (vec_only) f1_stream_wait();
  __syncthreads();
  block_sum_max_sum(g_acc, rn_acc, dl_acc, L.red);
  put_partial(gptr(d.part), SL_GAMMA0 + par, g_acc); put_partial(gptr(d.part), SL_RN0 + par, rn_acc);
  if constexpr (FIRST) {
    bn_acc = block_max(bn_acc, L.red);
    put_partial(gptr(d.part), SL_BN, bn_acc);
  }
  if (!vec_only) put_partial(gptr(d.part), SL_DELTA + par, dl_acc);
  KT(9);
}
__device__ __forceinline__ F1Rec f1_first_record(const int *blk, int nblk) {
  const int b0 = __builtin_amdgcn_readfirstlane((int)(blockIdx.x & 7) * ((nblk + 7) >> 3) + (int)(blockIdx.x >> 3));
  const size_t b = (size_t)min(b0, nblk - 1);
  return F1Rec{sload_int4(blk, 4 * b), sload_int4(blk, 4 * b + 1), sload_int4(blk, 4 * b + 2), sload_int4(blk, 4 * b + 3)};
}
template <int D, bool MIX, bool WT>
__device__ __forceinline__ bool f1_iteration(const Dev &d, const int k, const int cap, const int admm_par, const int probe, F1Lds &L, F1Stream &S, const F1Rec &rec0, const F1Fold &fold, const int par) {
  KT(0);
  F1Scal sc;
  if (!f1_fold_finish(d, k, admm_par, probe, fold, L.red, sc)) return false;
  const bool vec_only = !probe && k >= cap;
  if (k == 0) f1_body<D, true, MIX, WT>(d, k, vec_only, sc, L, S, rec0, par);
  else f1_body<D, false, MIX, WT>(d, k, vec_only, sc, L, S, rec0, par);
  return true;
}
template <bool NT>
__device__ __forceinline__ void f1_stream_first(const unsigned char *stream, int nblk, F1Stream &S) {
  const int per = (nblk + 7) >> 3, slot0 = (int)(blockIdx.x >> 3);
  const int b0 = __builtin_amdgcn_readfirstlane((int)(blockIdx.x & 7) * per + slot0);
  if (slot0 < per && b0 < nblk) f1_stream_issue<NT>(stream, b0, S);
}

template <int D, bool SCATTER_ONLY, bool MIX, bool WT>
__device__ __forceinline__ void f1_ka_body(const Dev &d, F1Lds &L, F1Stream &S, const F1Rec &rec0, const double theta) {
  const DevF1 &f = d.f1;
  const int tid = threadIdx.x;
  const double *va = gptr(f.va); const size_t ns = f.ns;
  const double *xs_r = va + ns;
  double *repR = gptr(f.va) + (7 + (size_t)1 * D) * ns, *repV = gptr(f.va) + (7 + (size_t)2 * D) * ns;
  [[maybe_unused]] double *spR = MIX ? gptr(f.spill) + (f.nsp + 2) : nullptr, *spVw = MIX ? gptr(f.spill) + 2 * (f.nsp + 2) : nullptr;
  const double alpha = d.alpha, sigma = d.sigma;
  const int xcd = blockIdx.x & 7, slot0 = blockIdx.x >> 3, slots = gridDim.x >> 3;
  const int per = (d.A.nblk + 7) >> 3;
  constexpr int CW = kF1Win / kBlock, CE = kF1Chunk / kBlock;
  constexpr int kFB = kF1Win - kF1MaxFar;
  for (int sl = slot0; sl < per; sl += slots) {
    const int b = __builtin_amdgcn_readfirstlane(xcd * per + sl);
    if (b >= d.A.nblk) break;
    [[maybe_unused]] int fcl = 0, fql = 0;
    if constexpr (MIX) { if (tid >= kFB - (CW - 1) * kBlock) { const size_t i = (size_t)b * kF1MaxFar + (tid - (kFB - (CW - 1) * kBlock)); fcl = gptr(f.fcol)[2 * i]; fql = gptr(f.fq)[i]; } }
    const F1Rec rec = sl == slot0 ? rec0 : f1_record(f, b);
    const int4 ds = rec.ds, fa = rec.fa, fb = rec.fb, fc = rec.fc;
    const int r0 = ds.x, nrows = ds.y - ds.x, k0 = ds.z, cnt = ds.w - ds.z;
    const int cov0 = fa.x, cov1 = fa.y, cs0 = fa.z, nown = fa.w - fa.z;
    const int cpo = fb.x, pk0 = fb.y, pcnt = fb.z - fb.y;
    const int g0 = fc.x, gl = fc.y, a0 = fc.z, wl = fc.w;
    const int nfc = MIX ? fb.w : 0;
    const int nw = nfc ? CW : (gl + kBlock - 1) / kBlock, nu = (cnt + kBlock - 1) / kBlock, ns2 = nfc ? CW : (wl + kBlock - 1) / kBlock;
    double pv = 0.0; int pc = g0;
    const bool hasp = tid < pcnt;
    { const int e = pk0 + max(0, min(tid, pcnt - 1)); pv = gptr(f.pval)[e]; pc = gptr(f.pcol)[e]; }
    const int pcl = pc - g0;
    const bool pin = pcl >= 0 && pcl < gl;
    double pxs = 0.0, pxp = 0.0;
    if (SCATTER_ONLY) pxs = gptr(d.xg)[pc];
    else { pxp = gptr(d.xsp)[pc]; if (!pin) pxs = xs_r[pc]; }
    double wx[CW], wxo[CW], wxp[CW], wq[CW];
    bool wown[CW];
#pragma unroll
    for (int u = 0; u < CW; u++) {
      wown[u] = false;
      if (u < nw) {
        const int e = tid + u * kBlock;
        int c = g0 + min(e, gl - 1);
        if constexpr (MIX) { if (u == CW - 1 && e >= kFB && e - kFB < nfc) c = fcl; }
        wown[u] = e < gl && c >= cs0 && c - cs0 < nown;
        const int co = wown[u] ? c : g0;
        if (!SCATTER_ONLY) { wx[u] = xs_r[c]; wxp[u] = gptr(d.xsp)[co]; }
        wxo[u] = gptr(d.x)[co]; wq[u] = gptr(d.q)[co];
      }
    }
    int rp0 = 0, rp1 = 0;
    double el = 0, eu = 0, erho = 0, erinv = 0, ez = 0, ey = 0, ezt = 0;
    { const int row = r0 + min(tid, nrows - 1);
      if (SCATTER_ONLY) { ez = gptr(d.v)[row]; ey = gptr(d.t0)[row]; }
      else { rp0 = gptr(d.A.rowptr)[row]; rp1 = gptr(d.A.rowptr)[row + 1]; el = gptr(d.l)[row]; eu = gptr(d.u)[row]; erho = gptr(d.rho)[row]; erinv = gptr(d.rho_inv)[row]; ez = gptr(d.z)[row]; ey = gptr(d.y)[row]; ezt = gptr(d.zt)[row]; } }
    int cp0[CW], cp1[CW];
#pragma unroll
    for (int u = 0; u < CW; u++) {
      if (u < ns2) {
        int c = min(tid + u * kBlock, wl - 1);
        if constexpr (MIX) { const int cf = tid + u * kBlock - kFB; if (u == CW - 1 && cf >= 0 && cf < nfc) c = wl + cf; }
        cp0[u] = gptr(f.cptr)[cpo + c]; cp1[u] = gptr(f.cptr)[cpo + c + 1];
      }
    }
    int pp0 = 0, pp1 = 0;
    { const int j = min(cs0 + max(0, min(tid, nown - 1)), d.n - 1); pp0 = gptr(f.prp)[j]; pp1 = gptr(f.prp)[j + 1]; }
#pragma unroll
    for (int u = 0; u < CW; u++) {
      if (u < nw) {
        int e = min(tid + u * kBlock, gl - 1);
        if constexpr (MIX) { const int ef = tid + u * kBlock; if (u == CW - 1 && ef >= kFB && ef - kFB < nfc) e = ef; }
        if (!SCATTER_ONLY) L.win[e] = wx[u];
        if (wown[u]) {
          const int j = g0 + e;
          double xn = wxo[u];
          if (!SCATTER_ONLY) {
            const double xt = wx[u];
            xn = alpha * xt + (1.0 - alpha) * wxo[u];
            gst(gptr(d.dx) + j, xn - wxo[u]); gst(gptr(d.x) + j, xn);
            gst(gptr(d.xg) + j, xt + theta * (xt - wxp[u]));
          }
          L.uown[j - cs0] = sigma * xn - wq[u];
        }
      }
    }
    f1_stream_wait();
#if defined(__HIP_DEVICE_COMPILE__)
    asm volatile("" :: "v"(rp0), "v"(rp1), "v"(el), "v"(eu), "v"(erho), "v"(erinv), "v"(ez), "v"(ey), "v"(ezt), "v"(pp0), "v"(pp1), "v"(pv), "v"(pc), "v"(pxs), "v"(pxp));
#pragma unroll
    for (int u = 0; u < CW; u++) { if (u < ns2) asm volatile("" :: "v"(cp0[u]), "v"(cp1[u])); }
    if constexpr (MIX) asm volatile("" :: "v"(fql));
#endif
    __syncthreads();
    double vw[CE]; unsigned int en[CE];
#pragma unroll
    for (int u = 0; u < CE; u++) { if (u < nu) { const int e = min(tid + u * kBlock, cnt - 1); vw[u] = S.val[e]; en[u] = S.ent[e]; } }
    if (!SCATTER_ONLY) {
#pragma unroll
      for (int u = 0; u < CE; u++) { if (u < nu) L.prod[tid + u * kBlock] = vw[u] * L.win[en[u] & 0x1ffu]; }
    }
    if (hasp) {
      double xg;
      if (SCATTER_ONLY) xg = pxs;
      else { const double xt = pin ? L.win[pcl] : pxs; xg = xt + theta * (xt - pxp); }
      L.pprod[tid] = pv * xg;
    }
    __syncthreads();
    if (sl + slots < per) {
      const int bn = __builtin_amdgcn_readfirstlane(xcd * per + sl + slots);
      if (bn < d.A.nblk) f1_stream_issue<!WT>(f.stream, bn, S);
    }
    double t0r = 0.0;
    if (tid < nrows) {
      double vi;
      if (SCATTER_ONLY) { vi = ez; t0r = ey; }
      else {
        const int i = r0 + tid;
        const double ztil = f1_segsum<6>(L.prod, rp0 - k0, rp1 - k0);
        const double zr = alpha * ztil + (1.0 - alpha) * ez;
        const double zn = fmin(fmax(zr + erinv * ey, el), eu);
        const double dyi = erho * (zr - zn), yn = ey + dyi;
        const double zg = ztil + theta * (ztil - ezt);
        vi = erho * zn - yn; t0r = erho * zg;
        gst(gptr(d.y) + i, yn); gst(gptr(d.dy) + i, dyi); gst(gptr(d.z) + i, zn); gst(gptr(d.zt) + i, ztil); gst(gptr(d.v) + i, vi); gst(gptr(d.ztg) + i, zg); gst(gptr(d.t0) + i, t0r);
      }
      L.tvec[tid] = vi;
    }
    for (int row = tid + kBlock; row < nrows; row += kBlock) {
      const int i = r0 + row;
      double vi;
      if (SCATTER_ONLY) vi = gptr(d.v)[i];
      else {
        const int q0 = gptr(d.A.rowptr)[i], q1 = gptr(d.A.rowptr)[i + 1];
        const double rho = gptr(d.rho)[i], zo = gptr(d.z)[i], yo = gptr(d.y)[i];
        const double ztil = f1_segsum<6>(L.prod, q0 - k0, q1 - k0);
        const double zr = alpha * ztil + (1.0 - alpha) * zo;
        const double zn = fmin(fmax(zr + gptr(d.rho_inv)[i] * yo, gptr(d.l)[i]), gptr(d.u)[i]);
        const double dyi = rho * (zr - zn), yn = yo + dyi;
        const double zg = ztil + theta * (ztil - gptr(d.zt)[i]);
        vi = rho * zn - yn;
        gst(gptr(d.y) + i, yn); gst(gptr(d.dy) + i, dyi); gst(gptr(d.z) + i, zn); gst(gptr(d.zt) + i, ztil); gst(gptr(d.v) + i, vi); gst(gptr(d.ztg) + i, zg); gst(gptr(d.t0) + i, rho * zg);
      }
      L.tvec[row] = vi;
    }
    if (tid < nown) L.puown[tid] = f1_segsum<4>(L.pprod, pp0 - pk0, pp1 - pk0);
    for (int jj = tid + kBlock; jj < nown; jj += kBlock) { const int q0 = gptr(f.prp)[cs0 + jj], q1 = gptr(f.prp)[cs0 + jj + 1]; L.puown[jj] = f1_segsum<4>(L.pprod, q0 - pk0, q1 - pk0); }
    __syncthreads();
#pragma unroll
    for (int u = 0; u < CE; u++) { if (u < nu) L.prod[en[u] >> 18] = vw[u] * L.tvec[(en[u] >> 9) & 0x1ffu]; }
    __syncthreads();
    double cv[CW];
#pragma unroll
    for (int u = 0; u < CW; u++) {
      cv[u] = 0.0;
      if (u < ns2) { const int c = tid + u * kBlock; if (c < wl || (MIX && u == CW - 1 && c >= kFB && c - kFB < nfc)) cv[u] = f1_segsum<8>(L.prod, cp0[u], cp1[u]); }
    }
    __syncthreads();
    if (tid < nrows) L.tvec[tid] = t0r;
    for (int row = tid + kBlock; row < nrows; row += kBlock) L.tvec[row] = gptr(d.t0)[r0 + row];
    __syncthreads();
#pragma unroll
    for (int u = 0; u < CE; u++) { if (u < nu) L.prod[en[u] >> 18] = vw[u] * L.tvec[(en[u] >> 9) & 0x1ffu]; }
    __syncthreads();
    double *routR = repR + (size_t)(b % D) * ns, *routV = repV + (size_t)(b % D) * ns;
#pragma unroll
    for (int u = 0; u < CW; u++) {
      if (u < ns2) {
        const int c = tid + u * kBlock;
        if (c < wl) {
          double tv = cv[u], tt = f1_segsum<8>(L.prod, cp0[u], cp1[u]);
          const int jo = a0 + c - cs0;
          if (jo >= 0 && jo < nown) { tv += L.uown[jo]; tt += L.puown[jo]; }
          gst(routV + a0 + c, tv); gst(routR + a0 + c, tv - tt);
        } else if constexpr (MIX) {
          if (u == CW - 1 && c >= kFB && c - kFB < nfc) { const double tv = cv[u], tt = f1_segsum<8>(L.prod, cp0[u], cp1[u]); gst(spVw + fql, tv); gst(spR + fql, tv - tt); }
        }
      }
    }
    for (int j = cov0 + tid; j < a0; j += kBlock) { gst(routV + j, 0.0); gst(routR + j, 0.0); }
    for (int j = a0 + wl + tid; j < cov1; j += kBlock) { gst(routV + j, 0.0); gst(routR + j, 0.0); }
    if (sl + slots < per) __syncthreads();
  }
}
template <int D, bool MIX, bool WT>
__device__ __forceinline__ void f1_slot_ka(const Dev &d, F1Lds &L, F1Stream &S, const F1Rec &rec0, int used, int conv, int admm, int target, int rn_slot, int seq) {
  double theta = d.theta, rn_last = 0.0, bn_last = 0.0;
  if (!conv) { theta = cutoff_theta(d, rn_slot, L.red, rn_last, bn_last, admm); __syncthreads(); }
  f1_ka_body<D, false, MIX, WT>(d, L, S, rec0, theta);
  if (blockIdx.x == 0) {
    if (!conv) {
      const double rn = rn_last, bn = bn_last;
      conv = !(rn > fmax(gptr(d.scal)[S_TOL_REL] * bn, gptr(d.scal)[S_TOL_ABS])) ? 2 : 0;
      if (!conv && threadIdx.x == 0 && rn > 0.1 * gptr(d.scal)[S_RN0]) gptr(d.flags)[F_STAT_STAG] += 1;
    }
    if (threadIdx.x == 0) {
      gptr(d.flags)[F_STAT_SUM] += used; gptr(d.flags)[F_STAT_SUMSQ] += used * used; gptr(d.flags)[F_STAT_N] += 1;
      if (used > gptr(d.flags)[F_STAT_MAX]) gptr(d.flags)[F_STAT_MAX] = used;
      if (!conv) gptr(d.flags)[F_STAT_UNCONV] += 1;
      if (d.ctl && admm + 1 >= target) { gptr(d.ctl)->seq_end = seq + 1; gptr(d.ctl)->chunk_done = 1; }
    }
  }
}
__global__ __launch_bounds__(kBlock) void k_f1_refresh(Dev d) {
  for (int k = blockIdx.x * kBlock + threadIdx.x; k < d.f1.pnnz; k += gridDim.x * kBlock) d.f1.pval[k] = d.B.val[d.f1.psrc[k]];
  for (int b = blockIdx.x; b < d.A.nblk; b += gridDim.x) {
    const int k0 = d.f1.blk[16 * (size_t)b + 2], cnt = d.f1.blk[16 * (size_t)b + 3] - k0;
    double *dst = reinterpret_cast<double *>(d.f1.stream + (size_t)b * kF1StreamBytes);
    for (int e = threadIdx.x; e < cnt; e += kBlock) dst[e] = d.A.val[k0 + e];
  }
}
template <int D, bool MIX, bool WT>
__global__ __launch_bounds__(kBlock) __attribute__((amdgpu_waves_per_eu(4, 4))) void k_f1_probe(Dev d, int k, int mode) {
  __shared__ F1Lds lds;
  __shared__ F1Stream sbuf;
  const int par = k & 1;
  f1_stream_first<!WT>(d.f1.stream, d.A.nblk, sbuf);
  const F1Fold fold = f1_fold_issue(gptr(d.part), par, mode);
  f1_iteration<D, MIX, WT>(d, k, 1 << 30, 0, mode, lds, sbuf, f1_first_record(d.f1.blk, d.A.nblk), fold, par);
}

template <int D, bool MIX, bool WT>
__global__ __launch_bounds__(kBlock) __attribute__((amdgpu_waves_per_eu(4, 4))) void k_f1_ka_probe(Dev d, int scatter_only) {
  __shared__ F1Lds lds;
  __shared__ F1Stream sbuf;
  f1_stream_first<!WT>(d.f1.stream, d.A.nblk, sbuf);
  const F1Rec rec0 = f1_first_record(d.f1.blk, d.A.nblk);
  if (scatter_only) f1_ka_body<D, true, MIX, WT>(d, lds, sbuf, rec0, d.theta); else f1_ka_body<D, false, MIX, WT>(d, lds, sbuf, rec0, d.theta);
}

struct F1DevBlock { Dev d; };
template <int D, bool MIX, bool WT>
__global__ __launch_bounds__(kBlock) __attribute__((amdgpu_waves_per_eu(4, 4))) void k_slot1(const unsigned char *__restrict__ stream, const int *__restrict__ fblk, int nblk, int par,
                                                                                             const double *__restrict__ part, const int *__restrict__ slot, const F1DevBlock *__restrict__ blk) {
  __shared__ F1Lds lds;
  __shared__ F1Stream sbuf;
  static_assert(sizeof(F1Lds) + sizeof(F1Stream) <= 160 * 1024 / 4, "four workgroups per CU");
  const Dev &d = blk->d;
  const int *R = slot + (par ? SR_WORDS : 0);
  int *W = const_cast<int *>(R) + (par ? -SR_WORDS : SR_WORDS);
  f1_stream_first<!WT>(stream, nblk, sbuf);
  const F1Fold fold = f1_fold_issue(gptr(part), par, 0);
  const F1Rec rec0 = f1_first_record(fblk, nblk);
  SlotState st = slot_read_scalar(R);
  if (st.ph == P_KB) {
    if (st.admm >= st.target) { st.ph = P_IDLE; f1_stream_wait(); slot_write(W, st); return; }
    f1_ka_body<D, true, MIX, WT>(d, lds, sbuf, rec0, 0.0);
    if (blockIdx.x == 0 && threadIdx.x == 0) { gptr(d.flags)[F_DONE] = 0; gptr(d.flags)[F_ITERS] = 0; }
    st.ph = P_F; st.k = 0;
  } else if (st.ph == P_F) {
    if (f1_iteration<D, MIX, WT>(d, st.k, st.cap, st.admm & 1, 0, lds, sbuf, rec0, fold, par)) {
      if (st.k >= st.cap) { st.ph = P_KA; st.used = st.k; st.conv = 0; }
      else st.k += 1;
    } else {
      __syncthreads();
      f1_slot_ka<D, MIX, WT>(d, lds, sbuf, rec0, st.k - 1, 1, st.admm, st.target, 0, st.seq);
      st.admm += 1; st.k = 0; st.ph = st.admm >= st.target ? P_IDLE : P_F;
    }
  } else if (st.ph == P_KA) {
    f1_slot_ka<D, MIX, WT>(d, lds, sbuf, rec0, st.used, st.conv, st.admm, st.target, par ^ 1, st.seq);
    st.admm += 1; st.k = 0; st.ph = st.admm >= st.target ? P_IDLE : P_F;
  } else f1_stream_wait();
  slot_write(W, st);
}


#undef gst
struct KfOps { double2 a, b; };
struct GKf {
  const double *rec; const F1Scal *sc;
  using Ops = KfOps;
  __device__ __forceinline__ Ops fetch(int c) const { const double2 *p = reinterpret_cast<const double2 *>(rec + 4 * (size_t)c); Ops o; o.a = p[0]; o.b = p[1]; return o; }
  __device__ __forceinline__ void prod(const Ops &o, double a, double (&pr)[1]) const { double sn, rn, un; f1_upd(*sc, o.a.x, o.a.y, o.b.x, o.b.y, sn, rn, un); pr[0] = a * un; }
  __device__ __forceinline__ void operator()(int c, double a, double (&pr)[1]) const { prod(fetch(c), a, pr); }
};
struct EKf {
  const double *recr; double *recw, *p, *xs; const F1Scal *sc;
  double g = 0, rn = 0, dl = 0;
  double2 oa = make_double2(0, 0), ob = make_double2(0, 0); double pp = 0, px = 0;
  __device__ __forceinline__ void prefetch(int j) { const double2 *q = reinterpret_cast<const double2 *>(recr + 4 * (size_t)j); oa = q[0]; ob = q[1]; pp = p[j]; px = xs[j]; }
  __device__ __forceinline__ void update(int j, double w, bool with_w) {
    double sn, rnew, un;
    f1_upd(*sc, oa.x, oa.y, ob.x, ob.y, sn, rnew, un);
    const double pn = fma(sc->beta, sc->general ? pp : 0.0, oa.x * oa.y);
    xs[j] = fma(sc->alpha, pn, px); p[j] = pn;
    double2 *o = reinterpret_cast<double2 *>(recw + 4 * (size_t)j);
    o[0] = make_double2(oa.x, rnew); o[1] = make_double2(w, sn);
    g += rnew * un; rn = nanmax(rn, fabs(rnew)); if (with_w) dl += un * w;
  }
  __device__ __forceinline__ void operator()(int j, const double (&s)[1]) { update(j, s[0], true); }
};
struct PreKf {
  [[maybe_unused]] static constexpr int kTraceBase = 0;
  const Dev &d; int k, admm_par, probe, par; double *red; F1Scal *sc;
  using Tok = F1Fold;
  __device__ __forceinline__ Tok begin() const { return f1_fold_issue(d.part, par, probe); }
  __device__ __forceinline__ bool finish(const Tok &t) const { return f1_fold_finish(d, k, admm_par, probe, t, red, *sc); }
};
template <class L>
__device__ __forceinline__ bool kf_iteration(const Dev &d, const int k, const int cap, const int admm_par, const int probe, L &lds, const int par) {
  F1Scal sc{0.0, 0.0, 0};
  const int cur = (k + 1) & 1, nxt = k & 1;
  const double *recr = d.kf.rec + (size_t)cur * 4 * (size_t)d.n;
  double *recw = d.kf.rec + (size_t)nxt * 4 * (size_t)d.n;
  const bool vec_only = !probe && k >= cap;
  EKf e{recr, recw, d.p, d.xs, &sc};
  if (vec_only) {
    const F1Fold fold = f1_fold_issue(d.part, par, probe);
    if (!f1_fold_finish(d, k, admm_par, probe, fold, lds.red, sc)) return false;
    const DevCsr &M = d.kf.K;
    const int4 *desc = reinterpret_cast<const int4 *>(M.blkdesc);
    const int xcd = blockIdx.x & 7, slot0 = blockIdx.x >> 3, slots = gridDim.x >> 3, per = (M.nblk + 7) >> 3;
    for (int sl = slot0; sl < per; sl += slots) {
      const int b = xcd * per + sl;
      if (b >= M.nblk) break;
      const int4 ds = desc[b];
      const int r1 = ds.y < 0 ? ds.x + 1 : ds.y;
      for (int j = ds.x + (int)threadIdx.x; j < r1; j += kBlock) { e.prefetch(j); e.update(j, 0.0, false); }
    }
  } else {
    GKf g{recr, &sc};
    if (!process_rows<1>(d.kf.K, g, e, lds, PreKf{d, k, admm_par, probe, par, lds.red, &sc})) return false;
  }
  __syncthreads();
  block_sum_max_sum(e.g, e.rn, e.dl, lds.red);
  put_partial(d.part, SL_GAMMA0 + par, e.g); put_partial(d.part, SL_RN0 + par, e.rn);
  if (!vec_only) put_partial(d.part, SL_DELTA + par, e.dl);
  return true;
}
struct EKbK {
  const double *x, *q, *Minv; double *rec1; double sigma; const double *xg; double *xs; double bn = 0; double px = 0, pq = 0, pm = 0, pg = 0;
  __device__ __forceinline__ void prefetch(int j) { px = x[j]; pq = q[j]; pm = Minv[j]; pg = xg[j]; }
  __device__ __forceinline__ void operator()(int j, const double (&s)[2]) {
    const double rhs = sigma * px - pq + s[0];
    const double rr = rhs - s[1];
    double2 *o = reinterpret_cast<double2 *>(rec1 + 4 * (size_t)j);
    o[0] = make_double2(pm, rr); o[1] = make_double2(0.0, 0.0);
    xs[j] = pg;
    bn = nanmax(bn, fabs(rhs));
  }
};
__global__ __launch_bounds__(kBlock) void k_kf_values(Dev d, int cond) {
  if (cond && !d.ctl->rho_flag) return;
  const DevKf &f = d.kf;
  const int stride = gridDim.x * kBlock;
  for (int e = blockIdx.x * kBlock + threadIdx.x; e < f.K.nnz; e += stride) {
    const int t0 = f.tptr[e], t1 = f.tptr[e + 1];
    double v = 0.0;
    for (int t = t0; t < t1; t++) { const int i = f.trow[t]; v += i < 0 ? d.B.val[f.ta[t]] : d.rho[i] * (d.A.val[f.ta[t]] * d.A.val[f.tb[t]]); }
    f.K.val[e] = v;
  }
}
__global__ __launch_bounds__(kBlock) void k_slotk(Dev d, int par) {
  __shared__ union { StreamLds<2> kb; StreamLds<1> f; StreamLdsW<1, double> ka; } lds;
  const int *R = d.slot + (par ? SR_WORDS : 0);
  int *W = d.slot + (par ? 0 : SR_WORDS);
  const FirstDesc fdA = first_desc<true>(d.A);
  SlotState st = slot_read(R);
  if (st.ph == P_KB) {
    if (st.admm >= st.target) { st.ph = P_IDLE; slot_write(W, st); return; }
    GKb g{d.xg, d.v, d.t0, d.n};
    EKbK e{d.x, d.q, d.Minv, d.kf.rec + 4 * (size_t)d.n, d.sigma, d.xg, d.xs};
    process_rows<2>(d.B, g, e, lds.kb);
    __syncthreads();
    const double BN = block_max(e.bn, lds.kb.red);
    put_partial(d.part, SL_BN, BN);
    if (blockIdx.x == 0 && threadIdx.x == 0) { d.flags[F_DONE] = 0; d.flags[F_ITERS] = 0; }
    st.ph = P_F; st.k = 0;
  } else if (st.ph == P_F) {
    if (kf_iteration(d, st.k, st.cap, st.admm & 1, st.conv == 2 ? 2 : 0, lds.f, par)) {
      if (st.k >= st.cap) { st.ph = P_KA; st.used = st.k; st.conv = 0; }
      else st.k += 1;
    } else {
      __syncthreads();
      slot_ka(d, lds.ka, st.k - 1, 1, fdA, st.admm, st.target, st.seq);
      st.admm += 1; st.k = 0; st.ph = P_KB;
    }
  } else if (st.ph == P_KA) {
    slot_ka(d, lds.ka, st.used, st.conv, fdA, st.admm, st.target, st.seq, par ^ 1);
    st.admm += 1; st.k = 0; st.ph = P_KB;
  }
  slot_write(W, st);
}


}

void kb_rhs(Dev &d) { LAUNCH(k_kb, d, d); }
bool pcg_fused(const Dev &d) { return d.fused != 0; }
void k1(Dev &d, int i) { if (d.fused && i > 0) LAUNCH(k_k1f, d, d, i); else LAUNCH(k_k1, d, d, i, 0); }
void k2(Dev &d, int i) { if (d.fused) LAUNCH(k_k2f, d, d, i); else LAUNCH(k_k2, d, d, 0); }
void kv(Dev &d, int i) { if (d.n >= 2 * kGrid * kBlock) LAUNCH(k_kv<2>, d, d, i, 0); else LAUNCH(k_kv<1>, d, d, i, 0); }
void ka(Dev &d, int budget) { LAUNCH(k_ka, d, d, budget); }
bool slots_supported(const Dev &d) { return (d.fused != 0 || wbx_slots(d)) && d.slot != nullptr; }
void dev_publish(Dev &d) {
  if (!d.f1.on) return;
  Impl &p = im(d);
  if (!p.dev_block) {
    HIP_CHECK(hipMalloc(&p.dev_block, sizeof(F1DevBlock)));
    HIP_CHECK(hipHostMalloc(reinterpret_cast<void **>(&p.pin_block), sizeof(F1DevBlock), hipHostMallocDefault));
    p.shadow_block = static_cast<unsigned char *>(std::calloc(1, sizeof(F1DevBlock)));
    std::memset(p.pin_block, 0, sizeof(F1DevBlock));
    p.shadow_block[0] = 1;
  }
  F1DevBlock nb;
  std::memset(static_cast<void *>(&nb), 0, sizeof(nb));
  std::memcpy(static_cast<void *>(&nb.d), static_cast<const void *>(&d), sizeof(Dev));
  if (std::memcmp(&nb, p.shadow_block, sizeof(nb)) == 0) return;
  HIP_CHECK(hipStreamSynchronize(st(d)));
  std::memcpy(p.shadow_block, &nb, sizeof(nb));
  std::memcpy(p.pin_block, &nb, sizeof(nb));
  HIP_CHECK(hipMemcpyAsync(p.dev_block, p.pin_block, sizeof(nb), hipMemcpyHostToDevice, st(d)));
}
void dev_release(Dev &d) {
  Impl &p = im(d);
  if (p.dev_block) { (void)hipFree(p.dev_block); p.dev_block = nullptr; }
  if (p.pin_block) { (void)hipHostFree(p.pin_block); p.pin_block = nullptr; }
  if (p.shadow_block) { std::free(p.shadow_block); p.shadow_block = nullptr; }
}
template <class F>
static void f1_dispatch(const Dev &d, F &&f) {
  auto with_m = [&](auto Dc, auto Mc) { if (d.f1.wt) f(Dc, Mc, std::true_type{}); else f(Dc, Mc, std::false_type{}); };
  auto with_d = [&](auto Dc) { if (d.f1.mix) with_m(Dc, std::true_type{}); else with_m(Dc, std::false_type{}); };
  switch (d.f1.D) {
    case 1: with_d(std::integral_constant<int, 1>{}); break;
    case 2: with_d(std::integral_constant<int, 2>{}); break;
    case 3: with_d(std::integral_constant<int, 3>{}); break;
    default: with_d(std::integral_constant<int, 4>{}); break;
  }
}
void slot_begin(Dev &d, int target, int cap) { HIP_CHECK(hipSetDevice(d.device)); dev_publish(d); hipLaunchKernelGGL(k_slot_init, dim3(1), dim3(1), 0, st(d), d.slot, target, cap, ++im(d).epoch); }
void slot_pair(Dev &d) {
  if (wbx_slots(d)) { wbx_slot_pair(d); return; }
  if (d.f1.on) {
    const F1DevBlock *db = static_cast<const F1DevBlock *>(im(d).dev_block);
    f1_dispatch(d, [&](auto Dc, auto Mc, auto Wc) {
      constexpr int DD = decltype(Dc)::value; constexpr bool MM = decltype(Mc)::value, WW = decltype(Wc)::value;
      hipLaunchKernelGGL((k_slot1<DD, MM, WW>), dim3(kGrid), dim3(kBlock), 0, st(d), static_cast<const unsigned char *>(d.f1.stream), static_cast<const int *>(d.f1.blk), d.A.nblk, 0, static_cast<const double *>(d.part), static_cast<const int *>(d.slot), db);
      hipLaunchKernelGGL((k_slot1<DD, MM, WW>), dim3(kGrid), dim3(kBlock), 0, st(d), static_cast<const unsigned char *>(d.f1.stream), static_cast<const int *>(d.f1.blk), d.A.nblk, 1, static_cast<const double *>(d.part), static_cast<const int *>(d.slot), db);
    });
  }
  else if (d.kf.on) { LAUNCH(k_slotk, d, d, 0); LAUNCH(k_slotk, d, d, 1); }
  else { LAUNCH(k_slot_b, d, d); LAUNCH(k_slot_a, d, d); }
}
bool kf_supported() { return true; }
void kf_values(Dev &d, int cond) { if (d.kf.on) { HIP_CHECK(hipSetDevice(d.device)); LAUNCH(k_kf_values, d, d, cond); } }
void f1_refresh(Dev &d) { if (d.f1.on) { HIP_CHECK(hipSetDevice(d.device)); LAUNCH(k_f1_refresh, d, d); } }
int slot_seq(Dev &d) { return (im(d).pin_flags + F_COUNT)[SR_SEQ]; }
int slot_done(Dev &d) {
  const int *rec = im(d).pin_flags + F_COUNT;
  return rec[SR_ADMM];
}

void slot_poll(Dev &d, int *seq, int *done) {
  HIP_CHECK(hipSetDevice(d.device));
  Impl &p = im(d);
  HIP_CHECK(hipMemcpyAsync(p.pin_poll, d.slot, sizeof(int) * kSlotInts, hipMemcpyDeviceToHost, p.side));
  HIP_CHECK(hipStreamSynchronize(p.side));
  if (p.pin_poll[2 * SR_WORDS] != p.epoch) { *seq = 0; *done = 0; return; }
  const int *ra = p.pin_poll, *rb = p.pin_poll + SR_WORDS;
  const int *nw = ra[SR_SEQ] >= rb[SR_SEQ] ? ra : rb;
  *seq = nw[SR_SEQ]; *done = nw[SR_ADMM];
}

__global__ void k_slot_probe_f(int *slot, double *scal, int k0, int conv) {
  for (int rec = 0; rec < 2; rec++) {
    int *r = slot + rec * SR_WORDS;
    r[SR_PHASE] = P_F; r[SR_K] = k0; r[SR_ADMM] = 0; r[SR_TARGET] = 1; r[SR_USED] = 0; r[SR_CONV] = conv; r[SR_CAP] = 1 << 20; r[SR_SEQ] = rec ? -1 : 0;
  }
  scal[S_TOL_NOW] = -1.0;
}
static void f1_probe_pair(Dev &d, int mode) {
  f1_dispatch(d, [&](auto Dc, auto Mc, auto Wc) {
    constexpr int DD = decltype(Dc)::value; constexpr bool MM = decltype(Mc)::value, WW = decltype(Wc)::value;
    hipLaunchKernelGGL((k_f1_probe<DD, MM, WW>), dim3(kGrid), dim3(kBlock), 0, st(d), d, 2, mode);
    hipLaunchKernelGGL((k_f1_probe<DD, MM, WW>), dim3(kGrid), dim3(kBlock), 0, st(d), d, 3, mode);
  });
}
float time_kernel(Dev &d, int which, int reps) {
  HIP_CHECK(hipSetDevice(d.device));
  Impl &p = im(d);
  struct Save { double *ptr; size_t cnt; double *bak; };
  const size_t n = d.n, m = d.m;
  if (which >= 14 && which <= 18 && !d.f1.on && !(which == 16 && d.kf.on)) return 0.f;
  if (which == 20 && !wbx_active(d)) return 0.f;
  if (which == 21 && !(d.wb.on && d.wb.exact)) return 0.f;
  if (which == 23 && !wbf_active(d)) return 0.f;
  const bool wbx = which == 20;
  const size_t r3 = wbx ? 3 * (size_t)d.wb.r : 0, gp_ = wbx ? (size_t)d.wb.x.G * kWbMaxRows : 0;
  Save sv[] = {{d.x, n, nullptr}, {d.z, m, nullptr}, {d.y, m, nullptr}, {d.xs, n, nullptr}, {d.zt, m, nullptr}, {d.t0, m, nullptr},
               {d.v, m, nullptr}, {d.dx, n, nullptr}, {d.dy, m, nullptr}, {d.r, n, nullptr}, {d.uu, n, nullptr}, {d.p, n, nullptr},
               {d.s, n, nullptr}, {d.w, n, nullptr}, {d.t, m, nullptr}, {d.uu2, n, nullptr}, {d.ms, 2 * n, nullptr},
               {d.xg, n, nullptr}, {d.xsp, n, nullptr}, {d.ztg, m, nullptr}, {d.kf.rec, d.kf.on ? 8 * n : 0, nullptr},
               {d.wb.x.ls0, r3, nullptr}, {d.wb.x.ls1, r3, nullptr}, {d.wb.x.partG, gp_, nullptr}, {d.wb.x.partZ, gp_, nullptr}};
  int flags_bak[F_COUNT];
  HIP_CHECK(hipStreamSynchronize(st(d)));
  HIP_CHECK(hipMemcpy(flags_bak, d.flags, sizeof(flags_bak), hipMemcpyDeviceToHost));
  for (auto &s : sv) {
    if (!s.cnt) continue;
    HIP_CHECK(hipMalloc(reinterpret_cast<void **>(&s.bak), s.cnt * sizeof(double)));
    HIP_CHECK(hipMemcpy(s.bak, s.ptr, s.cnt * sizeof(double), hipMemcpyDeviceToDevice));
  }
  auto K1 = [&](int pr) { LAUNCH(k_k1, d, d, 1, pr); };
  auto K2 = [&]() { LAUNCH(k_k2, d, d, 1); };
  auto KV = [&](int pr) { if (d.n >= 2 * kGrid * kBlock) LAUNCH(k_kv<2>, d, d, 1, pr); else LAUNCH(k_kv<1>, d, d, 1, pr); };
  auto launch = [&]() {
    switch (which) {
      case 0: LAUNCH(k_k1, d, d, 1, 1); break;
      case 1: LAUNCH(k_k2, d, d, 1); break;
      case 2: if (d.n >= 2 * kGrid * kBlock) LAUNCH(k_kv<2>, d, d, 1, 1); else LAUNCH(k_kv<1>, d, d, 1, 1); break;
      case 3: LAUNCH(k_kb, d, d); break;
      case 4: LAUNCH(k_ka, d, d, 0); break;
      case 5: K1(1); K2(); KV(1); break;
      case 6: K1(2); K2(); KV(2); break;
      case 7: K1(2); KV(2); break;
      case 8: K2(); KV(2); break;
      case 9: K1(2); K2(); break;
      case 11: LAUNCH(k_k1f, d, d, 1); break;
      case 12: LAUNCH(k_k2f, d, d, 0); break;
      case 13: LAUNCH(k_k2f, d, d, 2); LAUNCH(k_k1f, d, d, 3); break;
      case 14: f1_probe_pair(d, 1); break;
      case 16: slot_pair(d); break;
      case 17: case 18:
        f1_dispatch(d, [&](auto Dc, auto Mc, auto Wc) {
          constexpr int DD = decltype(Dc)::value; constexpr bool MM = decltype(Mc)::value, WW = decltype(Wc)::value;
          hipLaunchKernelGGL((k_f1_ka_probe<DD, MM, WW>), dim3(kGrid), dim3(kBlock), 0, st(d), d, (int)(which == 18));
        });
        break;
      case 21: HIP_CHECK(hipMemsetAsync(d.flags + F_DONE, 0, sizeof(int), st(d))); wb_apply(d, 0, 1); break;
      case 23: wbf_iteration(d); break;
      case 15: f1_probe_pair(d, 2); break;
      default: LAUNCH(k_k2f, d, d, 0); LAUNCH(k_k1f, d, d, 1); break;
    }
  };
  if (which == 20) {
    wbx_chunk(d, 3);
    HIP_CHECK(hipEventRecord(p.ev0, st(d)));
    wbx_chunk(d, reps);
    HIP_CHECK(hipEventRecord(p.ev1, st(d)));
    HIP_CHECK(hipEventSynchronize(p.ev1));
    float msx = 0.f;
    HIP_CHECK(hipEventElapsedTime(&msx, p.ev0, p.ev1));
    for (auto &sx : sv) { if (!sx.cnt) continue; HIP_CHECK(hipMemcpy(sx.ptr, sx.bak, sx.cnt * sizeof(double), hipMemcpyDeviceToDevice)); HIP_CHECK(hipFree(sx.bak)); }
    HIP_CHECK(hipMemcpy(d.flags, flags_bak, sizeof(flags_bak), hipMemcpyHostToDevice));
    return msx / reps;
  }
  if (which == 16) {
    dev_publish(d);
    if (reps > 400) reps = 400;
    hipLaunchKernelGGL(k_slot_probe_f, dim3(1), dim3(1), 0, st(d), d.slot, d.scal, 2, d.kf.on ? 2 : 0);
  }
  if (which >= 10) HIP_CHECK(hipMemsetAsync(d.flags + F_DONE, which == 13 ? 1 : 0, sizeof(int), st(d)));
  for (int w = 0; w < 5; w++) launch();
  HIP_CHECK(hipEventRecord(p.ev0, st(d)));
  for (int r = 0; r < reps; r++) launch();
  HIP_CHECK(hipEventRecord(p.ev1, st(d)));
  HIP_CHECK(hipEventSynchronize(p.ev1));
  float ms = 0.f;
  HIP_CHECK(hipEventElapsedTime(&ms, p.ev0, p.ev1));
  for (auto &s : sv) {
// ... 25 lines not shown
```

Before: 11160.

## Place ADMM vectors in the F1 arena and read a compact scalar header

When the fused F1 path is active, the primal and dual vectors (q, x, dx, xg, xsp, y, dy, z, zt, v, ztg, t0, l, u, rho_inv) are now carved out of the single F1 arena. Kernels then access them through buffer-resource loads and stores with fixed offsets instead of through generic global pointers taken from the large Dev struct. A compact 88-byte F1Head is added at the front of the device parameter block and loaded with a few wide scalar loads, so the hot loop no longer reads many scattered fields of Dev. The aim is fewer address computations, fewer scalar loads and better-behaved memory instructions. The cost is a larger arena and more complex offset bookkeeping, and the free path now has to null out the aliased pointers.

```diff
diff --git a/osqp-python_amd/csrc/backend.h b/osqp-python_amd/csrc/backend.h
--- a/osqp-python_amd/csrc/backend.h
+++ b/osqp-python_amd/csrc/backend.h
@@ -51,6 +51,7 @@
   int pnnz = 0;
   double *va = nullptr; size_t ns = 0;
   unsigned vbytes = 0, o_rho = 0, o_pval = 0, o_pcol = 0, o_prp = 0, o_rowptr = 0, o_cptr = 0, nsb = 0;
+  unsigned o_mv = 0, msb = 0;
   int mix = 0;
   int wt = 0;
   int *fcol = nullptr, *fq = nullptr;
@@ -58,6 +59,8 @@
   int *spk = nullptr;
   double *spill = nullptr; size_t nsp = 0;
 };
+enum { kF1Vq = 0, kF1Vx, kF1Vdx, kF1Vxg, kF1Vxsp, kF1NVec };
+enum { kF1My = 0, kF1Mdy, kF1Mz, kF1Mzt, kF1Mv, kF1Mztg, kF1Mt0, kF1Ml, kF1Mu, kF1Mrinv, kF1MVec };
 constexpr int kF1MaxFar = 128;
 
 constexpr int kKfMaxFill = 8;
diff --git a/osqp-python_amd/csrc/engine.cpp b/osqp-python_amd/csrc/engine.cpp
--- a/osqp-python_amd/csrc/engine.cpp
+++ b/osqp-python_amd/csrc/engine.cpp
@@ -148,6 +148,7 @@
   free_batch_direct(); free_batch_spectral(); free_batch_wave();
   if (d_.f1.va) {
     d_.Minv = d_.xs = d_.p = d_.r = d_.s = d_.rho = d_.f1.pval = nullptr; d_.f1.pcol = d_.f1.prp = nullptr; d_.f1.cptr = nullptr;
+    d_.q = d_.x = d_.dx = d_.xg = d_.xsp = d_.y = d_.dy = d_.z = d_.zt = d_.v = d_.ztg = d_.t0 = d_.l = d_.u = d_.rho_inv = nullptr;
   }
   if (d_.wb.cache_buf[0]) d_.wb.Sinv = d_.wb.cache_buf[0];
   void *ptrs[] = {d_.A.rowptr, d_.A.col, d_.A.blkdesc, d_.A.val, d_.B.rowptr, d_.B.col, d_.B.blkdesc, d_.B.val, d_.Bdiag, d_.A.runinfo, d_.B.runinfo, d_.A.blkwin, d_.B.blkwin, d_.A.lcol, d_.B.lcol, d_.qraw, d_.lraw, d_.uraw, d_.cnt,
diff --git a/osqp-python_amd/csrc/engine_setup.cpp b/osqp-python_amd/csrc/engine_setup.cpp
--- a/osqp-python_amd/csrc/engine_setup.cpp
+++ b/osqp-python_amd/csrc/engine_setup.cpp
@@ -265,10 +265,12 @@
   d_.f1 = DevF1();
   if (!pl.ok) return;
   const size_t ns = ((size_t)n + 31) / 32 * 32;
-  size_t at = 8 * (7 + 3 * (size_t)pl.D) * ns;
+  const size_t ms = ((size_t)std::max(m, 1) + 31) / 32 * 32;
+  size_t at = 8 * (7 + 3 * (size_t)pl.D + kF1NVec) * ns;
   auto region = [&at](size_t bytes) { const size_t o = at; at += (std::max<size_t>(bytes, 1) + 255) / 256 * 256; return o; };
   const size_t o_rho = region(8 * (size_t)m), o_pval = region(8 * (size_t)pl.pnnz), o_pcol = region(sizeof(int) * pl.pcol.size()),
-               o_prp = region(sizeof(int) * pl.prp.size()), o_rowptr = region(sizeof(int) * Arp.size()), o_cptr = region(sizeof(unsigned short) * pl.cptr.size());
+               o_prp = region(sizeof(int) * pl.prp.size()), o_rowptr = region(sizeof(int) * Arp.size()), o_cptr = region(sizeof(unsigned short) * pl.cptr.size()),
+               o_mv = region(8 * (size_t)kF1MVec * ms);
   if (at >= ((size_t)1 << 31)) return;
   auto up_i = [&](const std::vector<int> &h) { int *p = dev_vec<int>(d_, h.size()); if (!h.empty()) be::h2d(d_, p, h.data(), sizeof(int) * h.size()); return p; };
   DevF1 &f = d_.f1;
@@ -276,7 +278,7 @@
   f.ns = ns; f.nsb = (unsigned)(8 * ns);
   f.va = dev_vec<double>(d_, at / 8); f.vbytes = (unsigned)at;
   unsigned char *ab = reinterpret_cast<unsigned char *>(f.va);
-  f.o_rho = (unsigned)o_rho; f.o_pval = (unsigned)o_pval; f.o_pcol = (unsigned)o_pcol; f.o_prp = (unsigned)o_prp; f.o_rowptr = (unsigned)o_rowptr; f.o_cptr = (unsigned)o_cptr;
+  f.o_rho = (unsigned)o_rho; f.o_pval = (unsigned)o_pval; f.o_pcol = (unsigned)o_pcol; f.o_prp = (unsigned)o_prp; f.o_rowptr = (unsigned)o_rowptr; f.o_cptr = (unsigned)o_cptr; f.o_mv = (unsigned)o_mv; f.msb = (unsigned)(8 * ms);
   f.pval = reinterpret_cast<double *>(ab + o_pval); f.pcol = reinterpret_cast<int *>(ab + o_pcol); f.prp = reinterpret_cast<int *>(ab + o_prp);
   f.cptr = reinterpret_cast<unsigned short *>(ab + o_cptr);
   auto put = [&](size_t o, const void *h, size_t bytes) { if (bytes) be::h2d(d_, ab + o, h, bytes); };
@@ -740,10 +742,18 @@
   build_wbf_views(rbA, rbB, Arp, Arj, Brp, Bj);
   lap("upload structure");
   auto dv = [&](size_t cnt) { return dev_vec<double>(d_, cnt); };
-  d_.q = dv(n); d_.l = dv(m); d_.u = dv(m); d_.D = dv(n); d_.Dinv = dv(n); d_.E = dv(m); d_.Einv = dv(m);
-  d_.rho = d_.f1.on ? reinterpret_cast<double *>(reinterpret_cast<unsigned char *>(d_.f1.va) + d_.f1.o_rho) : dv(m); d_.rho_inv = dv(m); d_.ctype = dev_vec<int>(d_, m);
-  d_.x = dv(n); d_.z = dv(m); d_.y = dv(m); d_.dx = dv(n); d_.dy = dv(m); d_.zt = dv(m); d_.t0 = dv(m); d_.v = dv(m);
-  d_.xg = dv(n); d_.xsp = dv(n); d_.ztg = dv(m);
+  const bool f1a = d_.f1.on != 0;
+  auto f1n = [&](int k) { return d_.f1.va + (7 + 3 * (size_t)d_.f1.D + k) * d_.f1.ns; };
+  auto f1m = [&](int k) { return reinterpret_cast<double *>(reinterpret_cast<unsigned char *>(d_.f1.va) + d_.f1.o_mv + (size_t)k * d_.f1.msb); };
+  d_.q = f1a ? f1n(kF1Vq) : dv(n); d_.l = f1a ? f1m(kF1Ml) : dv(m); d_.u = f1a ? f1m(kF1Mu) : dv(m); d_.D = dv(n); d_.Dinv = dv(n); d_.E = dv(m); d_.Einv = dv(m);
+  d_.rho = d_.f1.on ? reinterpret_cast<double *>(reinterpret_cast<unsigned char *>(d_.f1.va) + d_.f1.o_rho) : dv(m); d_.rho_inv = f1a ? f1m(kF1Mrinv) : dv(m); d_.ctype = dev_vec<int>(d_, m);
+  if (f1a) {
+    d_.x = f1n(kF1Vx); d_.dx = f1n(kF1Vdx); d_.xg = f1n(kF1Vxg); d_.xsp = f1n(kF1Vxsp);
+    d_.y = f1m(kF1My); d_.dy = f1m(kF1Mdy); d_.z = f1m(kF1Mz); d_.zt = f1m(kF1Mzt); d_.v = f1m(kF1Mv); d_.ztg = f1m(kF1Mztg); d_.t0 = f1m(kF1Mt0);
+  } else {
+    d_.x = dv(n); d_.z = dv(m); d_.y = dv(m); d_.dx = dv(n); d_.dy = dv(m); d_.zt = dv(m); d_.t0 = dv(m); d_.v = dv(m);
+    d_.xg = dv(n); d_.xsp = dv(n); d_.ztg = dv(m);
+  }
   d_.theta = pol_.extrap;
   {
     const double mb = (12.0 * ((double)d_.A.nnz + (double)d_.B.nnz) + 8.0 * (14.0 * n + 12.0 * m)) / (1024.0 * 1024.0);
diff --git a/osqp-python_amd/csrc/pcg_hip.hip b/osqp-python_amd/csrc/pcg_hip.hip
--- a/osqp-python_amd/csrc/pcg_hip.hip
+++ b/osqp-python_amd/csrc/pcg_hip.hip
@@ -560,24 +560,24 @@
   f.a = partial_load(part + (SL_GAMMA0 + prev) * kGrid); f.b = partial_load(part + (SL_DELTA + prev) * kGrid); f.c = partial_load(part + (SL_RN0 + prev) * kGrid);
   return f;
 }
-__device__ __forceinline__ bool f1_fold_finish(const Dev &d, const int k, const int admm_par, const int probe, const F1Fold &f, double *red, F1Scal &sc) {
-  double *gam = gptr(d.scal) + S_HIST, *alp = gptr(d.scal) + S_HIST + kMaxCg + 1;
+__device__ __forceinline__ bool f1_fold_finish(double *scal, const double *part, double *res, const int k, const int admm_par, const int probe, const F1Fold &f, double *red, F1Scal &sc) {
+  double *gam = scal + S_HIST, *alp = scal + S_HIST + kMaxCg + 1;
   const int tid = threadIdx.x;
   sc = F1Scal{0.0, 0.0, k >= 2};
   if (probe == 1) { sc.alpha = 1e-3; sc.beta = k >= 2 ? 0.5 : 0.0; return true; }
   if (k == 0) return true;
-  double tol = gptr(d.scal)[S_TOL_NOW];
+  double tol = scal[S_TOL_NOW];
   const double glast = k >= 2 ? gam[k - 2] : 1.0, alast = k >= 2 ? alp[k - 2] : 1.0;
   double gamma = partial_fold_sum(f.a), rn = partial_fold_max(f.c), delta = partial_fold_sum(f.b);
   block_sum_max_sum(gamma, rn, delta, red);
   if (k == 1 && probe == 0) {
-    const double bn = block_max(partial_fold_max(partial_load(gptr(d.part) + SL_BN * kGrid)), red);
-    tol = fmax(gptr(d.scal)[S_TOL_REL] * bn, gptr(d.scal)[S_TOL_ABS]);
-    if (blockIdx.x == 0 && tid == 0) { gptr(d.scal)[S_TOL_NOW] = tol; gptr(d.scal)[S_RN0] = rn; gptr(d.scal)[S_RN0H + admm_par] = rn; }
+    const double bn = block_max(partial_fold_max(partial_load(part + SL_BN * kGrid)), red);
+    tol = fmax(scal[S_TOL_REL] * bn, scal[S_TOL_ABS]);
+    if (blockIdx.x == 0 && tid == 0) { scal[S_TOL_NOW] = tol; scal[S_RN0] = rn; scal[S_RN0H + admm_par] = rn; }
     if (!(rn > tol)) return false;
   }
   if (probe) {
-    if (rn < -1.0) gptr(d.res)[R_COUNT - 1] = gamma + delta + tol + glast + alast;
+    if (rn < -1.0) res[R_COUNT - 1] = gamma + delta + tol + glast + alast;
     sc.alpha = 1e-3; sc.beta = k >= 2 ? 0.5 : 0.0;
     return true;
   }
@@ -598,8 +598,8 @@
 #endif
 }
 struct F1Rec { int4 ds, fa, fb, fc; };
-__device__ __forceinline__ F1Rec f1_record(const DevF1 &f, int b) {
-  return F1Rec{sload_int4(f.blk, 4 * (size_t)b), sload_int4(f.blk, 4 * (size_t)b + 1), sload_int4(f.blk, 4 * (size_t)b + 2), sload_int4(f.blk, 4 * (size_t)b + 3)};
+__device__ __forceinline__ F1Rec f1_record(const int *blk, int b) {
+  return F1Rec{sload_int4(blk, 4 * (size_t)b), sload_int4(blk, 4 * (size_t)b + 1), sload_int4(blk, 4 * (size_t)b + 2), sload_int4(blk, 4 * (size_t)b + 3)};
 }
 struct F1Spill { double v0, v1; };
 __device__ __forceinline__ F1Spill f1_spill_take(const double *sp, int word) {
@@ -633,32 +633,70 @@
   __device__ __forceinline__ double d(unsigned vo, unsigned so) const { return __builtin_bit_cast(double, __builtin_amdgcn_raw_buffer_load_b64(r, vo, so, 0)); }
   __device__ __forceinline__ int i(unsigned vo, unsigned so) const { return (int)__builtin_amdgcn_raw_buffer_load_b32(r, vo, so, 0); }
   __device__ __forceinline__ int h(unsigned vo, unsigned so) const { return (int)__builtin_amdgcn_raw_buffer_load_b16(r, vo, so, 0); }
+  template <bool WT> __device__ __forceinline__ void st(unsigned vo, unsigned so, double v) const { typedef unsigned __attribute__((ext_vector_type(2))) v2u; __builtin_amdgcn_raw_buffer_store_b64(__builtin_bit_cast(v2u, v), r, vo, so, WT ? 16 : 0); }
 #else
   const unsigned char *b;
   __device__ F1Arena(const double *va, unsigned) : b(reinterpret_cast<const unsigned char *>(va)) {}
   __device__ double d(unsigned vo, unsigned so) const { return *reinterpret_cast<const double *>(b + vo + so); }
   __device__ int i(unsigned vo, unsigned so) const { return *reinterpret_cast<const int *>(b + vo + so); }
   __device__ int h(unsigned vo, unsigned so) const { return *reinterpret_cast<const unsigned short *>(b + vo + so); }
+  template <bool WT> __device__ void st(unsigned vo, unsigned so, double v) const { *reinterpret_cast<double *>(const_cast<unsigned char *>(b) + vo + so) = v; }
 #endif
 };
+struct F1Head {
+  double *va, *scal;
+  double sigma, alpha, theta;
+  unsigned vbytes, nsb;
+  int pnnz, n;
+  unsigned o_rho, o_pval, o_pcol, o_prp, o_rowptr, o_cptr, o_mv, msb;
+};
+static_assert(sizeof(F1Head) == 88, "scalar loads of 8, 4, 2 and 8 words");
+inline __host__ __device__ F1Head f1_head_of(const Dev &d) {
+  const DevF1 &f = d.f1;
+  return F1Head{f.va, d.scal, d.sigma, d.alpha, d.theta, f.vbytes, f.nsb, f.pnnz, d.n, f.o_rho, f.o_pval, f.o_pcol, f.o_prp, f.o_rowptr, f.o_cptr, f.o_mv, f.msb};
+}
+struct F1Ctx { F1Head h; const unsigned char *stream; const int *blk; int nblk; double *part; };
+inline __host__ __device__ F1Ctx f1_ctx_of(const Dev &d) { return F1Ctx{f1_head_of(d), d.f1.stream, d.f1.blk, d.A.nblk, d.part}; }
+__device__ __forceinline__ F1Head f1_head_load(const void *blk) {
+#if defined(__HIP_DEVICE_COMPILE__)
+  typedef int __attribute__((ext_vector_type(8))) v8i;
+  typedef int __attribute__((ext_vector_type(4))) v4i;
+  typedef int __attribute__((ext_vector_type(2))) v2i;
+  typedef const unsigned char __attribute__((address_space(4))) *cptr;
+  const cptr p = (cptr)(unsigned long long)blk;
+  const v8i a = *(const v8i __attribute__((address_space(4))) *)p;
+  const v4i b = *(const v4i __attribute__((address_space(4))) *)(p + 32);
+  const v2i c = *(const v2i __attribute__((address_space(4))) *)(p + 48);
+  const v8i e = *(const v8i __attribute__((address_space(4))) *)(p + 56);
+  F1Head h;
+  unsigned char *hb = reinterpret_cast<unsigned char *>(&h);
+  __builtin_memcpy(hb, &a, 32); __builtin_memcpy(hb + 32, &b, 16); __builtin_memcpy(hb + 48, &c, 8); __builtin_memcpy(hb + 56, &e, 32);
+  return h;
+#else
+  return *static_cast<const F1Head *>(blk);
+#endif
+}
 template <int D, bool FIRST, bool MIX, bool WT>
-__device__ __forceinline__ void f1_body(const Dev &d, const int k, const bool vec_only, const F1Scal sc, F1Lds &L, F1Stream &S, const F1Rec &rec0, const int par) {
-  const DevF1 &f = d.f1;
-  const int n = d.n, tid = threadIdx.x;
+__device__ __forceinline__ void f1_body(const Dev &d, const F1Ctx &c, const int k, const bool vec_only, const F1Scal sc, F1Lds &L, F1Stream &S, const F1Rec &rec0, const int par) {
+  [[maybe_unused]] const DevF1 &f = d.f1;
+  const F1Head &h = c.h;
+  const int n = h.n, tid = threadIdx.x;
   const int cur = (k + 1) & 1, nxt = k & 1;
   KT(1);
-  const size_t ns = f.ns;
-  const F1Arena ar(f.va, f.vbytes);
-  const unsigned nsb = f.nsb;
+  const unsigned nsb = h.nsb;
+  const size_t ns = nsb >> 3;
+  const F1Arena ar(h.va, h.vbytes);
   const unsigned oxs = nsb, op = 2 * nsb;
   const unsigned orr = (3 + cur) * nsb;
   const unsigned osp = (5 + cur) * nsb;
   const unsigned orep = (7 + cur * D) * nsb;
   [[maybe_unused]] const unsigned orepV = (7 + 2 * D) * nsb;
-  double *xs_w = gptr(f.va) + ns, *p_w = gptr(f.va) + 2 * ns;
-  double *rnxt = gptr(f.va) + (3 + nxt) * ns;
-  double *snew = gptr(f.va) + (5 + nxt) * ns;
-  double *repnxt = gptr(f.va) + (7 + (size_t)nxt * D) * ns;
+  double *xs_w = gptr(h.va) + ns, *p_w = gptr(h.va) + 2 * ns;
+  double *rnxt = gptr(h.va) + (3 + nxt) * ns;
+  double *snew = gptr(h.va) + (5 + nxt) * ns;
+  double *repnxt = gptr(h.va) + (7 + (size_t)nxt * D) * ns;
+  [[maybe_unused]] const unsigned oxg = (7 + 3 * D + kF1Vxg) * nsb;
+  [[maybe_unused]] double *xsp_w = gptr(h.va) + (7 + 3 * D + kF1Vxsp) * ns;
   [[maybe_unused]] const double *spcur = MIX ? gptr(f.spill) + (size_t)cur * (f.nsp + 2) : nullptr, *spV = MIX ? gptr(f.spill) + 2 * (f.nsp + 2) : nullptr;
   [[maybe_unused]] double *spnxt = MIX ? gptr(f.spill) + (size_t)nxt * (f.nsp + 2) : nullptr;
   [[maybe_unused]] const int *spk = MIX ? gptr(f.spk) : nullptr;
@@ -672,17 +710,17 @@
     return un;
   };
   const int xcd = blockIdx.x & 7, slot0 = blockIdx.x >> 3, slots = gridDim.x >> 3;
-  const int per = (d.A.nblk + 7) >> 3;
+  const int per = (c.nblk + 7) >> 3;
   constexpr int CW = kF1Win / kBlock, CE = kF1Chunk / kBlock;
   constexpr int kFB = kF1Win - kF1MaxFar;
   static_assert(kFB >= (CW - 1) * kBlock, "the far slots belong to the lanes' last window element");
   static_assert(kF1PChunk == kBlock, "one (P + sigma I) entry per lane");
   for (int sl = slot0; sl < per; sl += slots) {
     const int b = __builtin_amdgcn_readfirstlane(xcd * per + sl);
-    if (b >= d.A.nblk) break;
+    if (b >= c.nblk) break;
     [[maybe_unused]] int2 fcl = make_int2(0, 0); [[maybe_unused]] int fql = 0;
     if constexpr (MIX) { if (tid >= kFB - (CW - 1) * kBlock) { const size_t i = (size_t)b * kF1MaxFar + (tid - (kFB - (CW - 1) * kBlock)); fcl = reinterpret_cast<const int2 *>(gptr(f.fcol))[i]; fql = gptr(f.fq)[i]; } }
-    const F1Rec rec = sl == slot0 ? rec0 : f1_record(f, b);
+    const F1Rec rec = sl == slot0 ? rec0 : f1_record(c.blk, b);
     const int4 ds = rec.ds, fa = rec.fa, fb = rec.fb, fc = rec.fc;
     const int r0 = ds.x, nrows = ds.y - ds.x, k0 = ds.z, cnt = ds.w - ds.z;
     const int cov0 = fa.x, cov1 = fa.y, cs0 = fa.z, nown = fa.w - fa.z;
@@ -692,8 +730,8 @@
     const int nw = nfc ? CW : (gl + kBlock - 1) / kBlock, nu = (cnt + kBlock - 1) / kBlock, ns2 = nfc ? CW : (wl + kBlock - 1) / kBlock;
     KT(2);
     const bool hasp = !vec_only && tid < pcnt;
-    const int pe = min(pk0 + max(0, min(tid, pcnt - 1)), f.pnnz - 1);
-    const double pv = ar.d(8u * pe, f.o_pval); const int pc = ar.i(4u * pe, f.o_pcol);
+    const int pe = min(pk0 + max(0, min(tid, pcnt - 1)), h.pnnz - 1);
+    const double pv = ar.d(8u * pe, h.o_pval); const int pc = ar.i(4u * pe, h.o_pcol);
     double wm[CW], wr[CW], wsv[CW], wq[CW][D], wpp[CW], wx[CW];
     bool wown[CW];
     [[maybe_unused]] int wsw[CW]; [[maybe_unused]] F1Spill wst[CW];
@@ -713,7 +751,7 @@
           wr[u] = ar.d(8u * c, orr);
           wsv[u] = ar.d(8u * c, osp);
           wx[u] = ar.d(8u * co, oxs); wpp[u] = ar.d(8u * co, op);
-        } else { wx[u] = ar.d(8u * co, oxs); wpp[u] = gptr(d.xg)[co]; }
+        } else { wx[u] = ar.d(8u * co, oxs); wpp[u] = ar.d(8u * co, oxg); }
       }
     }
     if constexpr (MIX) {
@@ -722,17 +760,17 @@
     }
     int cp0[CW], cp1[CW];
     const int prow = r0 + min(tid, nrows - 1);
-    const int rp0 = ar.i(4u * prow, f.o_rowptr), rp1 = ar.i(4u * prow, f.o_rowptr + 4); const double rrho = ar.d(8u * prow, f.o_rho);
+    const int rp0 = ar.i(4u * prow, h.o_rowptr), rp1 = ar.i(4u * prow, h.o_rowptr + 4); const double rrho = ar.d(8u * prow, h.o_rho);
 #pragma unroll
     for (int u = 0; u < CW; u++) {
       if (u < ns2) {
         int c = min(tid + u * kBlock, wl - 1);
         if constexpr (MIX) { const int cf = tid + u * kBlock - kFB; if (u == CW - 1 && cf >= 0 && cf < nfc) c = wl + cf; }
-        cp0[u] = ar.h(2u * (cpo + c), f.o_cptr); cp1[u] = ar.h(2u * (cpo + c), f.o_cptr + 2);
+        cp0[u] = ar.h(2u * (cpo + c), h.o_cptr); cp1[u] = ar.h(2u * (cpo + c), h.o_cptr + 2);
       }
     }
     const int pj = min(cs0 + max(0, min(tid, nown - 1)), n - 1);
-    const int pp0 = ar.i(4u * pj, f.o_prp), pp1 = ar.i(4u * pj, f.o_prp + 4);
+    const int pp0 = ar.i(4u * pj, h.o_prp), pp1 = ar.i(4u * pj, h.o_prp + 4);
     const int pcl = pc - g0;
     const bool esc = hasp && !(pcl >= 0 && pcl < gl);
     KT(3);
@@ -749,7 +787,7 @@
           un = wm[u] * r0;
           if (wown[u]) {
             const int j = g0 + e;
-            gst(rnxt + j, r0); gst(gptr(d.xsp) + j, wx[u]); gst(xs_w + j, wpp[u]);
+            gst(rnxt + j, r0); gst(xsp_w + j, wx[u]); gst(xs_w + j, wpp[u]);
             g_acc += r0 * un; rn_acc = nanmax(rn_acc, fabs(r0));
           }
         } else {
@@ -773,7 +811,7 @@
       if constexpr (FIRST) {
         const double r0 = wj;
         un = mi * r0;
-        gst(rnxt + j, r0); gst(gptr(d.xsp) + j, ar.d(8u * j, oxs)); gst(xs_w + j, gptr(d.xg)[j]);
+        gst(rnxt + j, r0); gst(xsp_w + j, ar.d(8u * j, oxs)); gst(xs_w + j, ar.d(8u * j, oxg));
         g_acc += r0 * un; rn_acc = nanmax(rn_acc, fabs(r0));
       } else un = own_update(j, mi, ar.d(8u * j, orr), wj, ar.d(8u * j, osp), ar.d(8u * j, op), ar.d(8u * j, oxs));
       if (!vec_only) L.uown[jj] = un;
@@ -820,15 +858,15 @@
     __syncthreads();
     if (sl + slots < per) {
       const int bn = __builtin_amdgcn_readfirstlane(xcd * per + sl + slots);
-      if (bn < d.A.nblk) f1_stream_issue<!WT>(f.stream, bn, S);
+      if (bn < c.nblk) f1_stream_issue<!WT>(c.stream, bn, S);
     }
     if (tid < nrows) {
       const double au = f1_segsum<6>(L.prod, rp0 - k0, rp1 - k0), t = rrho * au;
       L.tvec[tid] = t; dl_acc += t * au;
     }
     for (int row = tid + kBlock; row < nrows; row += kBlock) {
-      const int q0 = ar.i(4u * (r0 + row), f.o_rowptr), q1 = ar.i(4u * (r0 + row), f.o_rowptr + 4);
-      const double au = f1_segsum<6>(L.prod, q0 - k0, q1 - k0), t = ar.d(8u * (r0 + row), f.o_rho) * au;
+      const int q0 = ar.i(4u * (r0 + row), h.o_rowptr), q1 = ar.i(4u * (r0 + row), h.o_rowptr + 4);
+      const double au = f1_segsum<6>(L.prod, q0 - k0, q1 - k0), t = ar.d(8u * (r0 + row), h.o_rho) * au;
       L.tvec[row] = t; dl_acc += t * au;
     }
     KT(6);
@@ -840,7 +878,7 @@
       L.puown[tid] = pu; dl_acc += L.uown[tid] * pu;
     }
     for (int jj = tid + kBlock; jj < nown; jj += kBlock) {
-      const int q0 = ar.i(4u * (cs0 + jj), f.o_prp), q1 = ar.i(4u * (cs0 + jj), f.o_prp + 4);
+      const int q0 = ar.i(4u * (cs0 + jj), h.o_prp), q1 = ar.i(4u * (cs0 + jj), h.o_prp + 4);
       const double pu = f1_segsum<4>(L.pprod, q0 - pk0, q1 - pk0);
       L.puown[jj] = pu; dl_acc += L.uown[jj] * pu;
     }
@@ -878,12 +916,12 @@
   if (vec_only) f1_stream_wait();
   __syncthreads();
   block_sum_max_sum(g_acc, rn_acc, dl_acc, L.red);
-  put_partial(gptr(d.part), SL_GAMMA0 + par, g_acc); put_partial(gptr(d.part), SL_RN0 + par, rn_acc);
+  put_partial(c.part, SL_GAMMA0 + par, g_acc); put_partial(c.part, SL_RN0 + par, rn_acc);
   if constexpr (FIRST) {
     bn_acc = block_max(bn_acc, L.red);
-    put_partial(gptr(d.part), SL_BN, bn_acc);
-  }
-  if (!vec_only) put_partial(gptr(d.part), SL_DELTA + par, dl_acc);
+    put_partial(c.part, SL_BN, bn_acc);
+  }
+  if (!vec_only) put_partial(c.part, SL_DELTA + par, dl_acc);
   KT(9);
 }
 __device__ __forceinline__ F1Rec f1_first_record(const int *blk, int nblk) {
@@ -892,13 +930,13 @@
   return F1Rec{sload_int4(blk, 4 * b), sload_int4(blk, 4 * b + 1), sload_int4(blk, 4 * b + 2), sload_int4(blk, 4 * b + 3)};
 }
 template <int D, bool MIX, bool WT>
-__device__ __forceinline__ bool f1_iteration(const Dev &d, const int k, const int cap, const int admm_par, const int probe, F1Lds &L, F1Stream &S, const F1Rec &rec0, const F1Fold &fold, const int par) {
+__device__ __forceinline__ bool f1_iteration(const Dev &d, const F1Ctx &c, const int k, const int cap, const int admm_par, const int probe, F1Lds &L, F1Stream &S, const F1Rec &rec0, const F1Fold &fold, const int par) {
   KT(0);
   F1Scal sc;
-  if (!f1_fold_finish(d, k, admm_par, probe, fold, L.red, sc)) return false;
+  if (!f1_fold_finish(gptr(c.h.scal), c.part, probe ? gptr(d.res) : nullptr, k, admm_par, probe, fold, L.red, sc)) return false;
   const bool vec_only = !probe && k >= cap;
-  if (k == 0) f1_body<D, true, MIX, WT>(d, k, vec_only, sc, L, S, rec0, par);
-  else f1_body<D, false, MIX, WT>(d, k, vec_only, sc, L, S, rec0, par);
+  if (k == 0) f1_body<D, true, MIX, WT>(d, c, k, vec_only, sc, L, S, rec0, par);
+  else f1_body<D, false, MIX, WT>(d, c, k, vec_only, sc, L, S, rec0, par);
   return true;
 }
 template <bool NT>
@@ -909,24 +947,30 @@
 }
 
 template <int D, bool SCATTER_ONLY, bool MIX, bool WT>
-__device__ __forceinline__ void f1_ka_body(const Dev &d, F1Lds &L, F1Stream &S, const F1Rec &rec0, const double theta) {
-  const DevF1 &f = d.f1;
+__device__ __forceinline__ void f1_ka_body(const Dev &d, const F1Ctx &c, F1Lds &L, F1Stream &S, const F1Rec &rec0, const double theta) {
+  [[maybe_unused]] const DevF1 &f = d.f1;
+  const F1Head &h = c.h;
   const int tid = threadIdx.x;
-  const double *va = gptr(f.va); const size_t ns = f.ns;
-  const double *xs_r = va + ns;
-  double *repR = gptr(f.va) + (7 + (size_t)1 * D) * ns, *repV = gptr(f.va) + (7 + (size_t)2 * D) * ns;
+  const F1Arena ar(h.va, h.vbytes);
+  const unsigned nsb = h.nsb, msb = h.msb, omv = h.o_mv;
+  const unsigned oxs = nsb;
+  const unsigned orepR = (7 + 1 * D) * nsb, orepV = (7 + 2 * D) * nsb;
+  const unsigned oq = (7 + 3 * D + kF1Vq) * nsb, ox = (7 + 3 * D + kF1Vx) * nsb, odx = (7 + 3 * D + kF1Vdx) * nsb, oxg = (7 + 3 * D + kF1Vxg) * nsb, oxsp = (7 + 3 * D + kF1Vxsp) * nsb;
+  const unsigned oy = omv + kF1My * msb, ody = omv + kF1Mdy * msb, oz = omv + kF1Mz * msb, ozt = omv + kF1Mzt * msb, ov = omv + kF1Mv * msb, oztg = omv + kF1Mztg * msb,
+                 ot0 = omv + kF1Mt0 * msb, ol = omv + kF1Ml * msb, ou = omv + kF1Mu * msb, orinv = omv + kF1Mrinv * msb;
+  auto ast = [&](unsigned vo, unsigned so, double v) { ar.template st<WT>(vo, so, v); };
   [[maybe_unused]] double *spR = MIX ? gptr(f.spill) + (f.nsp + 2) : nullptr, *spVw = MIX ? gptr(f.spill) + 2 * (f.nsp + 2) : nullptr;
-  const double alpha = d.alpha, sigma = d.sigma;
+  const double alpha = h.alpha, sigma = h.sigma;
   const int xcd = blockIdx.x & 7, slot0 = blockIdx.x >> 3, slots = gridDim.x >> 3;
-  const int per = (d.A.nblk + 7) >> 3;
+  const int per = (c.nblk + 7) >> 3;
   constexpr int CW = kF1Win / kBlock, CE = kF1Chunk / kBlock;
   constexpr int kFB = kF1Win - kF1MaxFar;
   for (int sl = slot0; sl < per; sl += slots) {
     const int b = __builtin_amdgcn_readfirstlane(xcd * per + sl);
-    if (b >= d.A.nblk) break;
+    if (b >= c.nblk) break;
     [[maybe_unused]] int fcl = 0, fql = 0;
     if constexpr (MIX) { if (tid >= kFB - (CW - 1) * kBlock) { const size_t i = (size_t)b * kF1MaxFar + (tid - (kFB - (CW - 1) * kBlock)); fcl = gptr(f.fcol)[2 * i]; fql = gptr(f.fq)[i]; } }
-    const F1Rec rec = sl == slot0 ? rec0 : f1_record(f, b);
+    const F1Rec rec = sl == slot0 ? rec0 : f1_record(c.blk, b);
     const int4 ds = rec.ds, fa = rec.fa, fb = rec.fb, fc = rec.fc;
     const int r0 = ds.x, nrows = ds.y - ds.x, k0 = ds.z, cnt = ds.w - ds.z;
     const int cov0 = fa.x, cov1 = fa.y, cs0 = fa.z, nown = fa.w - fa.z;
@@ -936,12 +980,12 @@
     const int nw = nfc ? CW : (gl + kBlock - 1) / kBlock, nu = (cnt + kBlock - 1) / kBlock, ns2 = nfc ? CW : (wl + kBlock - 1) / kBlock;
     double pv = 0.0; int pc = g0;
     const bool hasp = tid < pcnt;
-    { const int e = pk0 + max(0, min(tid, pcnt - 1)); pv = gptr(f.pval)[e]; pc = gptr(f.pcol)[e]; }
+    { const int e = pk0 + max(0, min(tid, pcnt - 1)); pv = ar.d(8u * e, h.o_pval); pc = ar.i(4u * e, h.o_pcol); }
     const int pcl = pc - g0;
     const bool pin = pcl >= 0 && pcl < gl;
     double pxs = 0.0, pxp = 0.0;
-    if (SCATTER_ONLY) pxs = gptr(d.xg)[pc];
-    else { pxp = gptr(d.xsp)[pc]; if (!pin) pxs = xs_r[pc]; }
+    if (SCATTER_ONLY) pxs = ar.d(8u * pc, oxg);
+    else { pxp = ar.d(8u * pc, oxsp); if (!pin) pxs = ar.d(8u * pc, oxs); }
     double wx[CW], wxo[CW], wxp[CW], wq[CW];
     bool wown[CW];
 #pragma unroll
@@ -953,26 +997,27 @@
         if constexpr (MIX) { if (u == CW - 1 && e >= kFB && e - kFB < nfc) c = fcl; }
         wown[u] = e < gl && c >= cs0 && c - cs0 < nown;
         const int co = wown[u] ? c : g0;
-        if (!SCATTER_ONLY) { wx[u] = xs_r[c]; wxp[u] = gptr(d.xsp)[co]; }
-        wxo[u] = gptr(d.x)[co]; wq[u] = gptr(d.q)[co];
+        if (!SCATTER_ONLY) { wx[u] = ar.d(8u * c, oxs); wxp[u] = ar.d(8u * co, oxsp); }
+        wxo[u] = ar.d(8u * co, ox); wq[u] = ar.d(8u * co, oq);
       }
     }
     int rp0 = 0, rp1 = 0;
     double el = 0, eu = 0, erho = 0, erinv = 0, ez = 0, ey = 0, ezt = 0;
     { const int row = r0 + min(tid, nrows - 1);
-      if (SCATTER_ONLY) { ez = gptr(d.v)[row]; ey = gptr(d.t0)[row]; }
-      else { rp0 = gptr(d.A.rowptr)[row]; rp1 = gptr(d.A.rowptr)[row + 1]; el = gptr(d.l)[row]; eu = gptr(d.u)[row]; erho = gptr(d.rho)[row]; erinv = gptr(d.rho_inv)[row]; ez = gptr(d.z)[row]; ey = gptr(d.y)[row]; ezt = gptr(d.zt)[row]; } }
+      if (SCATTER_ONLY) { ez = ar.d(8u * row, ov); ey = ar.d(8u * row, ot0); }
+      else { rp0 = ar.i(4u * row, h.o_rowptr); rp1 = ar.i(4u * row, h.o_rowptr + 4); el = ar.d(8u * row, ol); eu = ar.d(8u * row, ou); erho = ar.d(8u * row, h.o_rho); erinv = ar.d(8u * row, orinv);
+             ez = ar.d(8u * row, oz); ey = ar.d(8u * row, oy); ezt = ar.d(8u * row, ozt); } }
     int cp0[CW], cp1[CW];
 #pragma unroll
     for (int u = 0; u < CW; u++) {
       if (u < ns2) {
         int c = min(tid + u * kBlock, wl - 1);
         if constexpr (MIX) { const int cf = tid + u * kBlock - kFB; if (u == CW - 1 && cf >= 0 && cf < nfc) c = wl + cf; }
-        cp0[u] = gptr(f.cptr)[cpo + c]; cp1[u] = gptr(f.cptr)[cpo + c + 1];
+        cp0[u] = ar.h(2u * (cpo + c), h.o_cptr); cp1[u] = ar.h(2u * (cpo + c), h.o_cptr + 2);
       }
     }
     int pp0 = 0, pp1 = 0;
-    { const int j = min(cs0 + max(0, min(tid, nown - 1)), d.n - 1); pp0 = gptr(f.prp)[j]; pp1 = gptr(f.prp)[j + 1]; }
+    { const int j = min(cs0 + max(0, min(tid, nown - 1)), h.n - 1); pp0 = ar.i(4u * j, h.o_prp); pp1 = ar.i(4u * j, h.o_prp + 4); }
 #pragma unroll
     for (int u = 0; u < CW; u++) {
       if (u < nw) {
@@ -985,8 +1030,8 @@
           if (!SCATTER_ONLY) {
             const double xt = wx[u];
             xn = alpha * xt + (1.0 - alpha) * wxo[u];
-            gst(gptr(d.dx) + j, xn - wxo[u]); gst(gptr(d.x) + j, xn);
-            gst(gptr(d.xg) + j, xt + theta * (xt - wxp[u]));
+            ast(8u * j, odx, xn - wxo[u]); ast(8u * j, ox, xn);
+            ast(8u * j, oxg, xt + theta * (xt - wxp[u]));
           }
           L.uown[j - cs0] = sigma * xn - wq[u];
         }
@@ -1016,7 +1061,7 @@
     __syncthreads();
     if (sl + slots < per) {
       const int bn = __builtin_amdgcn_readfirstlane(xcd * per + sl + slots);
-      if (bn < d.A.nblk) f1_stream_issue<!WT>(f.stream, bn, S);
+      if (bn < c.nblk) f1_stream_issue<!WT>(c.stream, bn, S);
     }
     double t0r = 0.0;
     if (tid < nrows) {
@@ -1030,29 +1075,29 @@
         const double dyi = erho * (zr - zn), yn = ey + dyi;
         const double zg = ztil + theta * (ztil - ezt);
         vi = erho * zn - yn; t0r = erho * zg;
-        gst(gptr(d.y) + i, yn); gst(gptr(d.dy) + i, dyi); gst(gptr(d.z) + i, zn); gst(gptr(d.zt) + i, ztil); gst(gptr(d.v) + i, vi); gst(gptr(d.ztg) + i, zg); gst(gptr(d.t0) + i, t0r);
+        ast(8u * i, oy, yn); ast(8u * i, ody, dyi); ast(8u * i, oz, zn); ast(8u * i, ozt, ztil); ast(8u * i, ov, vi); ast(8u * i, oztg, zg); ast(8u * i, ot0, t0r);
       }
       L.tvec[tid] = vi;
     }
     for (int row = tid + kBlock; row < nrows; row += kBlock) {
       const int i = r0 + row;
       double vi;
-      if (SCATTER_ONLY) vi = gptr(d.v)[i];
+      if (SCATTER_ONLY) vi = ar.d(8u * i, ov);
       else {
-        const int q0 = gptr(d.A.rowptr)[i], q1 = gptr(d.A.rowptr)[i + 1];
-        const double rho = gptr(d.rho)[i], zo = gptr(d.z)[i], yo = gptr(d.y)[i];
+        const int q0 = ar.i(4u * i, h.o_rowptr), q1 = ar.i(4u * i, h.o_rowptr + 4);
+        const double rho = ar.d(8u * i, h.o_rho), zo = ar.d(8u * i, oz), yo = ar.d(8u * i, oy);
         const double ztil = f1_segsum<6>(L.prod, q0 - k0, q1 - k0);
         const double zr = alpha * ztil + (1.0 - alpha) * zo;
-        const double zn = fmin(fmax(zr + gptr(d.rho_inv)[i] * yo, gptr(d.l)[i]), gptr(d.u)[i]);
+        const double zn = fmin(fmax(zr + ar.d(8u * i, orinv) * yo, ar.d(8u * i, ol)), ar.d(8u * i, ou));
         const double dyi = rho * (zr - zn), yn = yo + dyi;
-        const double zg = ztil + theta * (ztil - gptr(d.zt)[i]);
+        const double zg = ztil + theta * (ztil - ar.d(8u * i, ozt));
         vi = rho * zn - yn;
-        gst(gptr(d.y) + i, yn); gst(gptr(d.dy) + i, dyi); gst(gptr(d.z) + i, zn); gst(gptr(d.zt) + i, ztil); gst(gptr(d.v) + i, vi); gst(gptr(d.ztg) + i, zg); gst(gptr(d.t0) + i, rho * zg);
+        ast(8u * i, oy, yn); ast(8u * i, ody, dyi); ast(8u * i, oz, zn); ast(8u * i, ozt, ztil); ast(8u * i, ov, vi); ast(8u * i, oztg, zg); ast(8u * i, ot0, rho * zg);
       }
       L.tvec[row] = vi;
     }
     if (tid < nown) L.puown[tid] = f1_segsum<4>(L.pprod, pp0 - pk0, pp1 - pk0);
-    for (int jj = tid + kBlock; jj < nown; jj += kBlock) { const int q0 = gptr(f.prp)[cs0 + jj], q1 = gptr(f.prp)[cs0 + jj + 1]; L.puown[jj] = f1_segsum<4>(L.pprod, q0 - pk0, q1 - pk0); }
+    for (int jj = tid + kBlock; jj < nown; jj += kBlock) { const int q0 = ar.i(4u * (cs0 + jj), h.o_prp), q1 = ar.i(4u * (cs0 + jj), h.o_prp + 4); L.puown[jj] = f1_segsum<4>(L.pprod, q0 - pk0, q1 - pk0); }
     __syncthreads();
 #pragma unroll
     for (int u = 0; u < CE; u++) { if (u < nu) L.prod[en[u] >> 18] = vw[u] * L.tvec[(en[u] >> 9) & 0x1ffu]; }
@@ -1065,12 +1110,12 @@
     }
     __syncthreads();
     if (tid < nrows) L.tvec[tid] = t0r;
-    for (int row = tid + kBlock; row < nrows; row += kBlock) L.tvec[row] = gptr(d.t0)[r0 + row];
+    for (int row = tid + kBlock; row < nrows; row += kBlock) L.tvec[row] = ar.d(8u * (r0 + row), ot0);
     __syncthreads();
 #pragma unroll
     for (int u = 0; u < CE; u++) { if (u < nu) L.prod[en[u] >> 18] = vw[u] * L.tvec[(en[u] >> 9) & 0x1ffu]; }
     __syncthreads();
-    double *routR = repR + (size_t)(b % D) * ns, *routV = repV + (size_t)(b % D) * ns;
+    const unsigned ooR = orepR + (unsigned)(b % D) * nsb, ooV = orepV + (unsigned)(b % D) * nsb;
 #pragma unroll
     for (int u = 0; u < CW; u++) {
       if (u < ns2) {
@@ -1079,27 +1124,27 @@
           double tv = cv[u], tt = f1_segsum<8>(L.prod, cp0[u], cp1[u]);
           const int jo = a0 + c - cs0;
           if (jo >= 0 && jo < nown) { tv += L.uown[jo]; tt += L.puown[jo]; }
-          gst(routV + a0 + c, tv); gst(routR + a0 + c, tv - tt);
+          ast(8u * (a0 + c), ooV, tv); ast(8u * (a0 + c), ooR, tv - tt);
         } else if constexpr (MIX) {
           if (u == CW - 1 && c >= kFB && c - kFB < nfc) { const double tv = cv[u], tt = f1_segsum<8>(L.prod, cp0[u], cp1[u]); gst(spVw + fql, tv); gst(spR + fql, tv - tt); }
         }
       }
     }
-    for (int j = cov0 + tid; j < a0; j += kBlock) { gst(routV + j, 0.0); gst(routR + j, 0.0); }
-    for (int j = a0 + wl + tid; j < cov1; j += kBlock) { gst(routV + j, 0.0); gst(routR + j, 0.0); }
+    for (int j = cov0 + tid; j < a0; j += kBlock) { ast(8u * j, ooV, 0.0); ast(8u * j, ooR, 0.0); }
+    for (int j = a0 + wl + tid; j < cov1; j += kBlock) { ast(8u * j, ooV, 0.0); ast(8u * j, ooR, 0.0); }
     if (sl + slots < per) __syncthreads();
   }
 }
 template <int D, bool MIX, bool WT>
-__device__ __forceinline__ void f1_slot_ka(const Dev &d, F1Lds &L, F1Stream &S, const F1Rec &rec0, int used, int conv, int admm, int target, int rn_slot, int seq) {
-  double theta = d.theta, rn_last = 0.0, bn_last = 0.0;
+__device__ __forceinline__ void f1_slot_ka(const Dev &d, const F1Ctx &c, F1Lds &L, F1Stream &S, const F1Rec &rec0, int used, int conv, int admm, int target, int rn_slot, int seq) {
+  double theta = c.h.theta, rn_last = 0.0, bn_last = 0.0;
   if (!conv) { theta = cutoff_theta(d, rn_slot, L.red, rn_last, bn_last, admm); __syncthreads(); }
-  f1_ka_body<D, false, MIX, WT>(d, L, S, rec0, theta);
+  f1_ka_body<D, false, MIX, WT>(d, c, L, S, rec0, theta);
   if (blockIdx.x == 0) {
     if (!conv) {
       const double rn = rn_last, bn = bn_last;
-      conv = !(rn > fmax(gptr(d.scal)[S_TOL_REL] * bn, gptr(d.scal)[S_TOL_ABS])) ? 2 : 0;
-      if (!conv && threadIdx.x == 0 && rn > 0.1 * gptr(d.scal)[S_RN0]) gptr(d.flags)[F_STAT_STAG] += 1;
+      conv = !(rn > fmax(gptr(c.h.scal)[S_TOL_REL] * bn, gptr(c.h.scal)[S_TOL_ABS])) ? 2 : 0;
+      if (!conv && threadIdx.x == 0 && rn > 0.1 * gptr(c.h.scal)[S_RN0]) gptr(d.flags)[F_STAT_STAG] += 1;
     }
     if (threadIdx.x == 0) {
       gptr(d.flags)[F_STAT_SUM] += used; gptr(d.flags)[F_STAT_SUMSQ] += used * used; gptr(d.flags)[F_STAT_N] += 1;
@@ -1124,7 +1169,7 @@
   const int par = k & 1;
   f1_stream_first<!WT>(d.f1.stream, d.A.nblk, sbuf);
   const F1Fold fold = f1_fold_issue(gptr(d.part), par, mode);
-  f1_iteration<D, MIX, WT>(d, k, 1 << 30, 0, mode, lds, sbuf, f1_first_record(d.f1.blk, d.A.nblk), fold, par);
+  f1_iteration<D, MIX, WT>(d, f1_ctx_of(d), k, 1 << 30, 0, mode, lds, sbuf, f1_first_record(d.f1.blk, d.A.nblk), fold, par);
 }
 
 template <int D, bool MIX, bool WT>
@@ -1133,10 +1178,11 @@
   __shared__ F1Stream sbuf;
   f1_stream_first<!WT>(d.f1.stream, d.A.nblk, sbuf);
   const F1Rec rec0 = f1_first_record(d.f1.blk, d.A.nblk);
-  if (scatter_only) f1_ka_body<D, true, MIX, WT>(d, lds, sbuf, rec0, d.theta); else f1_ka_body<D, false, MIX, WT>(d, lds, sbuf, rec0, d.theta);
-}
-
-struct F1DevBlock { Dev d; };
+  const F1Ctx c = f1_ctx_of(d);
+  if (scatter_only) f1_ka_body<D, true, MIX, WT>(d, c, lds, sbuf, rec0, d.theta); else f1_ka_body<D, false, MIX, WT>(d, c, lds, sbuf, rec0, d.theta);
+}
+
+struct F1DevBlock { F1Head h; Dev d; };
 template <int D, bool MIX, bool WT>
 __global__ __launch_bounds__(kBlock) __attribute__((amdgpu_waves_per_eu(4, 4))) void k_slot1(const unsigned char *__restrict__ stream, const int *__restrict__ fblk, int nblk, int par,
                                                                                              const double *__restrict__ part, const int *__restrict__ slot, const F1DevBlock *__restrict__ blk) {
@@ -1150,22 +1196,23 @@
   const F1Fold fold = f1_fold_issue(gptr(part), par, 0);
   const F1Rec rec0 = f1_first_record(fblk, nblk);
   SlotState st = slot_read_scalar(R);
+  const F1Ctx c{f1_head_load(blk), stream, fblk, nblk, const_cast<double *>(part)};
   if (st.ph == P_KB) {
     if (st.admm >= st.target) { st.ph = P_IDLE; f1_stream_wait(); slot_write(W, st); return; }
-    f1_ka_body<D, true, MIX, WT>(d, lds, sbuf, rec0, 0.0);
+    f1_ka_body<D, true, MIX, WT>(d, c, lds, sbuf, rec0, 0.0);
     if (blockIdx.x == 0 && threadIdx.x == 0) { gptr(d.flags)[F_DONE] = 0; gptr(d.flags)[F_ITERS] = 0; }
     st.ph = P_F; st.k = 0;
   } else if (st.ph == P_F) {
-    if (f1_iteration<D, MIX, WT>(d, st.k, st.cap, st.admm & 1, 0, lds, sbuf, rec0, fold, par)) {
+    if (f1_iteration<D, MIX, WT>(d, c, st.k, st.cap, st.admm & 1, 0, lds, sbuf, rec0, fold, par)) {
       if (st.k >= st.cap) { st.ph = P_KA; st.used = st.k; st.conv = 0; }
       else st.k += 1;
     } else {
       __syncthreads();
-      f1_slot_ka<D, MIX, WT>(d, lds, sbuf, rec0, st.k - 1, 1, st.admm, st.target, 0, st.seq);
+      f1_slot_ka<D, MIX, WT>(d, c, lds, sbuf, rec0, st.k - 1, 1, st.admm, st.target, 0, st.seq);
       st.admm += 1; st.k = 0; st.ph = st.admm >= st.target ? P_IDLE : P_F;
     }
   } else if (st.ph == P_KA) {
-    f1_slot_ka<D, MIX, WT>(d, lds, sbuf, rec0, st.used, st.conv, st.admm, st.target, par ^ 1, st.seq);
+    f1_slot_ka<D, MIX, WT>(d, c, lds, sbuf, rec0, st.used, st.conv, st.admm, st.target, par ^ 1, st.seq);
     st.admm += 1; st.k = 0; st.ph = st.admm >= st.target ? P_IDLE : P_F;
   } else f1_stream_wait();
   slot_write(W, st);
@@ -1202,7 +1249,7 @@
   const Dev &d; int k, admm_par, probe, par; double *red; F1Scal *sc;
   using Tok = F1Fold;
   __device__ __forceinline__ Tok begin() const { return f1_fold_issue(d.part, par, probe); }
-  __device__ __forceinline__ bool finish(const Tok &t) const { return f1_fold_finish(d, k, admm_par, probe, t, red, *sc); }
+  __device__ __forceinline__ bool finish(const Tok &t) const { return f1_fold_finish(gptr(d.scal), gptr(d.part), gptr(d.res), k, admm_par, probe, t, red, *sc); }
 };
 template <class L>
 __device__ __forceinline__ bool kf_iteration(const Dev &d, const int k, const int cap, const int admm_par, const int probe, L &lds, const int par) {
@@ -1214,7 +1261,7 @@
   EKf e{recr, recw, d.p, d.xs, &sc};
   if (vec_only) {
     const F1Fold fold = f1_fold_issue(d.part, par, probe);
-    if (!f1_fold_finish(d, k, admm_par, probe, fold, lds.red, sc)) return false;
+    if (!f1_fold_finish(gptr(d.scal), gptr(d.part), gptr(d.res), k, admm_par, probe, fold, lds.red, sc)) return false;
     const DevCsr &M = d.kf.K;
     const int4 *desc = reinterpret_cast<const int4 *>(M.blkdesc);
     const int xcd = blockIdx.x & 7, slot0 = blockIdx.x >> 3, slots = gridDim.x >> 3, per = (M.nblk + 7) >> 3;
@@ -1313,6 +1360,7 @@
   F1DevBlock nb;
   std::memset(static_cast<void *>(&nb), 0, sizeof(nb));
   std::memcpy(static_cast<void *>(&nb.d), static_cast<const void *>(&d), sizeof(Dev));
+  nb.h = f1_head_of(d);
   if (std::memcmp(&nb, p.shadow_block, sizeof(nb)) == 0) return;
   HIP_CHECK(hipStreamSynchronize(st(d)));
   std::memcpy(p.shadow_block, &nb, sizeof(nb));
```

Result: no change. 11220 (median of 6 runs) (+0.5%).
